# Veason-silverbullet/DIGAT

Measured on AMD Instinct MI355X. Metric: MIND dev impressions scored/sec (AUC match not run), higher is better.
Workload: dtype f32; 1 GPU; MIND-small default: --graph_encoder=DIGAT neighbors=3 hops=2 (N=10, U=67), d=400, graph_depth=3, fp32 dev inference; projection=auto -> fp16x3, N=10, U=67, d=400, graph_depth=3, news_num=65238, parallelism=dp1 (row shards, no data-path collective), ranks_in_process_group=1

## Files before the change

digat_amd/_lib.py:

```python
from __future__ import annotations

import ctypes as C
import os
from typing import Optional

import torch

_HERE = os.path.dirname(os.path.abspath(__file__))
LIB_PATH = os.environ.get("DIGAT_HIP_LIB") or os.path.join(_HERE, "lib", "libdigat_hip.so")
DIGAT_MAX_DEPTH = 16
DIGAT_MAX_NODES = 128
GEMM_BF16X6, GEMM_F16X3 = 0, 1
GEMM_F16F8C = 2
PARAMS_GEMM_F16X3 = 64
PARAMS_BD_TILED = 128
PARAMS_PQ_FP8 = 256
PARAMS_SIDE_STREAM_OFF, PARAMS_SIDE_STREAM_ON = 512, 1024
PARAMS_NO_LIVE_ROWS = 2048
PARAMS_PROJ_F16F8C = 4096

_f = C.c_void_p


class LayerParams(C.Structure):
    _fields_ = [(k, _f) for k in ("W", "bW", "F1", "F2", "F3", "b3", "a", "wsplit", "f3_wsplit")]


class MsaParams(C.Structure):
    _fields_ = ([(k, C.c_int32) for k in ("word_embedding_dim", "head_num", "head_dim", "attention_dim")]
                + [(k, C.c_void_p) for k in ("word_embedding", "W_Q", "b_Q", "W_K", "W_V", "b_V", "A1", "b1", "a2",
                                             "qkv_wsplit", "a1_wsplit")])


class MhsaParams(C.Structure):
    _fields_ = ([(k, C.c_int32) for k in ("in_dim", "head_num", "head_dim", "attention_dim")]
                + [(k, C.c_void_p) for k in ("table", "W_Q", "b_Q", "W_K", "W_V", "b_V", "A1", "b1", "a2", "qkv_wsplit", "a1_wsplit")]
                + [("flags", C.c_int32), ("reserved", C.c_int32)])


MHSA_POOL_UNMASKED = 1


class CnnParams(C.Structure):
    _fields_ = ([(k, C.c_int32) for k in ("word_embedding_dim", "kernel_num", "taps", "attention_dim")]
                + [(k, C.c_void_p) for k in ("word_embedding", "W", "b", "A1", "b1", "a2", "w_split", "a1_wsplit")])


class SplitJob(C.Structure):
    _fields_ = [("w0", C.c_void_p), ("w1", C.c_void_p), ("w2", C.c_void_p), ("rows", C.c_int32), ("cols", C.c_int32), ("layout", C.c_int32),
                ("reserved", C.c_int32), ("image", C.c_void_p)]


class GatherJob(C.Structure):
    _fields_ = [("src", C.c_void_p), ("dst", C.c_void_p), ("row_bytes", C.c_int64), ("rows", C.c_int64),
                ("idx", C.c_void_p), ("idx2", C.c_void_p), ("inner", C.c_int64)]


class Params(C.Structure):
    _fields_ = ([("d", C.c_int32), ("depth", C.c_int32), ("category_num", C.c_int32), ("flags", C.c_int32)]
                + [(k, _f) for k in ("topic_node_embedding", "cand_K", "cand_Q", "cand_bQ",
                                     "news_graph_W", "news_graph_b", "user_news_K", "user_news_Q",
                                     "user_news_bQ", "featureAffine_W", "featureAffine_b",
                                     "userAtt_K", "userAtt_Q", "userAtt_bQ")]
                + [("news", LayerParams * DIGAT_MAX_DEPTH), ("user", LayerParams * DIGAT_MAX_DEPTH)]
                + [(k, _f) for k in ("cand_fold_W", "cand_fold_b", "user_news_fold_W", "user_news_fold_b",
                                     "userAtt_fold_W", "userAtt_fold_b", "featureAffine_wsplit", "cand_fold_wsplit", "gate_wsplit")]
                + [("ctx_wsplit", _f * (DIGAT_MAX_DEPTH + 1)), ("range_flag", _f), ("featureAffine_fsplit", _f)])


class DigatHipError(RuntimeError):
    pass


_lib: Optional[C.CDLL] = None

_SIGNATURES = {
    "digat_version": (C.c_int, []),
    "digat_error_string": (C.c_char_p, [C.c_int]),
    "digat_linear_f32": (C.c_int, [_f, C.c_int64, _f, _f, _f, C.c_int64, C.c_int, C.c_int, C.c_int, _f]),
    "digat_xattn_workspace_bytes": (C.c_size_t, [C.c_int] * 3),
    "digat_xattn_fwd": (C.c_int, [_f] * 12 + [C.c_int] * 3 + [_f, C.c_size_t, _f]),
    "digat_xattn_fwd_mode": (C.c_int, [_f] * 11 + [C.c_int] * 4 + [_f, C.c_size_t, _f]),
    "digat_xattn_fwd_lowprec": (C.c_int, [_f] * 11 + [C.c_int, _f] + [C.c_int] * 4 + [_f, C.c_size_t, _f]),
    "digat_xattn_pairwise_fwd": (C.c_int, [_f] * 8 + [C.c_int] * 3 + [_f]),
    "digat_news_ctx_workspace_bytes": (C.c_size_t, [C.c_int] * 3),
    "digat_news_ctx_fwd": (C.c_int, [_f] * 9 + [C.c_int] * 3 + [_f, C.c_size_t, _f]),
    "digat_user_ctx_workspace_bytes": (C.c_size_t, [C.c_int] * 5),
    "digat_user_ctx_fwd": (C.c_int, [_f] * 14 + [C.c_int] * 5 + [_f, C.c_size_t, _f]),
    "digat_user_ctx_grouped_workspace_bytes": (C.c_size_t, [C.c_int] * 6),
    "digat_user_ctx_fwd_grouped": (C.c_int, [_f] * 15 + [C.c_int] * 6 + [_f, C.c_size_t, _f]),
    "digat_user_nodes_build": (C.c_int, [_f] * 4 + [C.c_long, C.c_long] + [C.c_int] * 3 + [_f]),
    "digat_topic_pool_fwd": (C.c_int, [_f] * 4 + [C.c_int] * 5 + [_f]),
    "digat_encoder_workspace_bytes": (C.c_size_t, [C.c_int] * 6),
    "digat_encoder_fwd": (C.c_int, [C.POINTER(Params)] + [_f] * 10 + [C.c_int] * 3 + [_f, C.c_size_t, _f]),
    "digat_row_logits": (C.c_int, [_f] * 3 + [C.c_int] * 2 + [_f]),
    "digat_profile_pause": (C.c_int, [C.c_int]),
    "digat_set_train_precision": (C.c_int, [C.c_int]),
    "digat_gather_tables": (C.c_int, [C.POINTER(GatherJob), C.c_int, _f]),
    "digat_user_graph_build": (C.c_int, [_f, _f, C.c_long, C.c_int, C.c_int, _f, _f, _f, _f]),
    "digat_negative_sample": (C.c_int, [_f, _f, _f, C.c_long, C.c_int, C.c_uint32, C.c_uint32, _f, _f]),
    "digat_train_batch_ids": (C.c_int, [_f, C.c_long, _f, _f, C.c_long, C.c_int, _f, C.c_long, C.c_int, _f, C.c_long, C.c_int, _f, _f, _f, _f, _f]),
    "digat_profile_live_row_fraction": (C.c_double, []),
    "digat_rank_metrics": (C.c_int, [_f] * 3 + [C.c_int] + [_f] * 4),
    "digat_format_rank_file": (C.c_int64, [_f, _f, C.c_int64, _f, C.c_int64]),
    "digat_topk_segments_workspace_bytes": (C.c_size_t, [C.c_int64, C.c_int64, C.c_int]),
    "digat_topk_segments": (C.c_int, [_f, _f, C.c_int64, C.c_int64, _f, _f, C.c_int, C.c_int, _f, _f, _f, _f, C.c_size_t, _f]),
    "digat_dot_topk_workspace_bytes": (C.c_size_t, [C.c_int64, C.c_int64, C.c_int]),
    "digat_dot_topk": (C.c_int, [_f, _f, _f, C.c_int64, C.c_int64, C.c_int64, C.c_int, _f, C.c_int, C.c_int, _f, _f, _f, _f, C.c_size_t, _f]),
    "digat_dot_scores": (C.c_int, [_f, _f, _f, C.c_int64, C.c_int64, C.c_int64, C.c_int, _f, _f]),
    "digat_mmr_select_workspace_bytes": (C.c_size_t, [C.c_int64, C.c_int, C.c_int]),
    "digat_mmr_select": (C.c_int, [_f, _f, _f, C.c_int64, C.c_int, _f, C.c_int64, C.c_int, _f, C.c_int, C.c_float, C.c_float, C.c_int, _f, _f, _f,
                                   _f, C.c_size_t, _f]),
    "digat_gat_workspace_bytes": (C.c_size_t, [C.c_int] * 3),
    "digat_gat_fwd": (C.c_int, [_f] * 7 + [C.c_int] * 3 + [_f, C.c_size_t, _f]),
    "digat_gat_train_save_bytes": (C.c_size_t, [C.c_int] * 3),
    "digat_gat_train_workspace_bytes": (C.c_size_t, [C.c_int] * 3),
    "digat_gat_fwd_train": (C.c_int, [_f] * 7 + [C.c_float, C.c_uint32] + [C.c_int] * 3 + [_f, C.c_size_t, _f, C.c_size_t, _f]),
    "digat_gat_bwd": (C.c_int, [_f] * 7 + [C.c_float, _f, C.c_size_t] + [_f] * 5 + [C.c_int] * 3 + [_f, C.c_size_t, _f]),
    "digat_sag_cos_topk_workspace_bytes": (C.c_size_t, [C.c_int64, C.c_int64, C.c_int]),
    "digat_sag_cos_topk": (C.c_int, [_f, _f, C.c_int64, _f, _f, C.c_int64, C.c_int, C.c_int, _f, _f, _f, C.c_size_t, _f]),
    "digat_sag_similar_lists_workspace_bytes": (C.c_size_t, [C.c_int64, C.c_int64, C.c_int]),
    "digat_sag_similar_lists": (C.c_int, [_f, _f, C.c_int64, _f, _f, C.c_int64, C.c_int, C.c_int] + [_f] * 7 + [C.c_int64, _f, C.c_size_t, _f]),
    "digat_sag_news_graph": (C.c_int, [_f, _f, _f, C.c_int64, C.c_int, C.c_int, C.c_int, C.c_float] + [_f] * 5),
    "digat_msa_split_bytes": (C.c_size_t, [C.c_int] * 3),
    "digat_split_msa_weights": (C.c_int, [_f] * 3 + [C.c_int] * 2 + [_f, _f]),
    "digat_msa_workspace_bytes": (C.c_size_t, [C.c_int] * 6),
    "digat_msa_fwd": (C.c_int, [C.POINTER(MsaParams), _f, _f, _f, C.c_int, C.c_int, _f, C.c_size_t, _f]),
    "digat_msa_train_save_bytes": (C.c_size_t, [C.c_int] * 6),
    "digat_msa_train_workspace_bytes": (C.c_size_t, [C.c_int] * 6),
    "digat_msa_fwd_train": (C.c_int, [C.POINTER(MsaParams), _f, _f, _f, C.c_float, C.c_uint32, C.c_int, C.c_int, _f, C.c_size_t, _f,
                                      C.c_size_t, _f]),
    "digat_msa_bwd": (C.c_int, [C.POINTER(MsaParams), _f, _f, _f, C.c_float, _f, C.c_size_t, _f, C.c_int64] + [_f] * 8
                      + [C.c_int, C.c_int, _f, C.c_size_t, _f]),
    "digat_msa_row_grad_ld": (C.c_int64, [C.c_int] * 3),
    "digat_mhsa_workspace_bytes": (C.c_size_t, [C.c_int] * 6),
    "digat_mhsa_fwd": (C.c_int, [C.POINTER(MhsaParams), _f, _f, _f, C.c_int, C.c_int, _f, C.c_size_t, _f]),
    "digat_mhsa_train_save_bytes": (C.c_size_t, [C.c_int] * 6),
    "digat_mhsa_train_workspace_bytes": (C.c_size_t, [C.c_int] * 6),
    "digat_mhsa_fwd_train": (C.c_int, [C.POINTER(MhsaParams), _f, _f, _f, C.c_float, C.c_float, C.c_uint32, C.c_int, C.c_int, _f, C.c_size_t, _f,
                                       C.c_size_t, _f]),
    "digat_mhsa_bwd": (C.c_int, [C.POINTER(MhsaParams), _f, _f, _f, C.c_float, C.c_float, C.c_uint32, _f, C.c_size_t, _f, C.c_int64] + [_f] * 8
                       + [C.c_int, C.c_int, _f, C.c_size_t, _f]),
    "digat_mhsa_attention_fwd": (C.c_int, [_f, _f, _f, C.c_float, C.c_uint32] + [C.c_int] * 4 + [_f]),
    "digat_mhsa_attention_bwd": (C.c_int, [_f, _f, _f, _f, C.c_float, C.c_uint32] + [C.c_int] * 4 + [_f]),
    "digat_cnn_split_bytes": (C.c_size_t, [C.c_int] * 3),
    "digat_split_cnn_weights": (C.c_int, [_f] + [C.c_int] * 3 + [_f, _f]),
    "digat_cnn_merge_group3": (C.c_int, [_f] * 6 + [C.c_int] * 2 + [_f] * 3),
    "digat_cnn_workspace_bytes": (C.c_size_t, [C.c_int] * 6),
    "digat_cnn_fwd": (C.c_int, [C.POINTER(CnnParams), _f, _f, _f, C.c_int, C.c_int, _f, C.c_size_t, _f]),
    "digat_cnn_train_save_bytes": (C.c_size_t, [C.c_int] * 6),
    "digat_cnn_train_workspace_bytes": (C.c_size_t, [C.c_int] * 6),
    "digat_cnn_fwd_train": (C.c_int, [C.POINTER(CnnParams), _f, _f, _f, C.c_float, C.c_uint32, C.c_int, C.c_int, _f, C.c_size_t, _f,
                                      C.c_size_t, _f]),
    "digat_cnn_bwd": (C.c_int, [C.POINTER(CnnParams), _f, _f, _f, C.c_float, C.c_uint32, _f, C.c_size_t, _f, C.c_int64] + [_f] * 5
                      + [C.c_int, C.c_int, _f, C.c_size_t, _f]),
    "digat_embedding_bwd_workspace_bytes": (C.c_size_t, [C.c_int64, C.c_int]),
    "digat_embedding_bwd": (C.c_int, [_f, C.c_int64, _f, _f, C.c_int64, C.c_int, _f, _f, C.c_size_t, _f]),
    "digat_embedding_bwd_unsorted_workspace_bytes": (C.c_size_t, [C.c_int64, C.c_int, C.c_int64]),
    "digat_embedding_bwd_unsorted": (C.c_int, [_f, _f, C.c_int64, C.c_int64, _f, _f, C.c_int64, C.c_int64, C.c_int, C.c_int64, _f, _f, C.c_size_t,
                                               _f]),
    "digat_encoder_grouped_workspace_bytes": (C.c_size_t, [C.c_int] * 6),
    "digat_encoder_fwd_grouped": (C.c_int, [C.POINTER(Params)] + [_f] * 11 + [C.c_int] * 4 + [_f, C.c_size_t, _f]),
    "digat_encoder_fwd_grouped_cached": (C.c_int, [C.POINTER(Params)] + [_f] * 14 + [C.c_int64] + [_f] * 2 + [C.c_int] * 4 + [_f, C.c_size_t, _f]),
    "digat_news_context_queries": (C.c_int, [C.POINTER(Params), _f, _f, C.c_int, _f]),
    "digat_user_project0": (C.c_int, [C.POINTER(Params), _f, _f, C.c_int, _f]),
    "digat_news_project0": (C.c_int, [C.POINTER(Params), _f, _f, C.c_int, C.c_int, _f]),
    "digat_split_weights_bytes": (C.c_size_t, [C.c_int, C.c_int]),
    "digat_split_weights_bytes_format": (C.c_size_t, [C.c_int, C.c_int, C.c_int]),
    "digat_forget_split_image": (C.c_int, [_f]),
    "digat_split_proj_weights": (C.c_int, [_f, _f, _f, C.c_int, _f, C.c_int, _f]),
    "digat_split_weights": (C.c_int, [_f, C.c_int, C.c_int, _f, C.c_int, _f]),
    "digat_linear_f32x3": (C.c_int, [_f, C.c_int64, _f, _f, _f, C.c_int64, C.c_int, C.c_int, C.c_int, _f, C.c_int, _f]),
    "digat_fold_workspace_bytes": (C.c_size_t, [C.c_int]),
    "digat_fold_attention": (C.c_int, [_f] * 5 + [C.c_int, _f, C.c_size_t, _f]),
    "digat_linear_bwd_input": (C.c_int, [_f, C.c_int64, _f, _f, C.c_int64, C.c_int, C.c_int, C.c_int, C.c_int, _f]),
    "digat_linear_bwd_input_x3": (C.c_int, [_f, C.c_int64, _f, _f, C.c_int64, C.c_int, C.c_int, C.c_int, C.c_int, _f, _f]),
    "digat_linear_bwd_weight_workspace": (C.c_size_t, [C.c_int] * 3),
    "digat_linear_bwd_weight": (C.c_int, [_f, C.c_int64, _f, C.c_int64, _f, _f, C.c_int, C.c_int, C.c_int, C.c_int, _f,
                                          C.c_size_t, _f]),
    "digat_colsum": (C.c_int, [_f, C.c_int64, _f, C.c_int, C.c_int, C.c_int, _f]),
    "digat_dropout_fwd": (C.c_int, [_f, _f, _f, C.c_int64, C.c_float, C.c_uint32, _f]),
    "digat_dropout_bwd": (C.c_int, [_f, _f, _f, C.c_int64, C.c_float, _f]),
    "digat_gate_fwd": (C.c_int, [_f, _f, C.c_int64, _f, _f, C.c_int, C.c_int, _f]),
    "digat_gate_bwd": (C.c_int, [_f, _f, _f, C.c_int64, _f, _f, _f, _f, C.c_int, C.c_int, _f]),
    "digat_relu_res_fwd": (C.c_int, [_f, _f, _f, C.c_int64, _f]),
    "digat_relu_mask": (C.c_int, [_f, _f, _f, C.c_int64, _f]),
    "digat_attn_pool_fwd": (C.c_int, [_f, C.c_int64, _f, _f, _f, _f, C.c_int, C.c_int, C.c_int, _f]),
    "digat_attn_pool_bwd": (C.c_int, [_f, C.c_int64, _f, _f, _f, _f, _f, C.c_int64, _f, C.c_int, C.c_int, C.c_int,
                                      C.c_int, _f]),
    "digat_topic_pool_fwd_train": (C.c_int, [_f] * 5 + [C.c_int] * 5 + [_f]),
    "digat_topic_pool_bwd": (C.c_int, [_f] * 7 + [C.c_int] * 5 + [_f]),
    "digat_xattn_project": (C.c_int, [_f] * 9 + [C.c_int] * 3 + [_f]),
    "digat_xattn_project_x3": (C.c_int, [_f] * 9 + [C.c_int] * 3 + [_f, _f]),
    "digat_xattn_pairwise_fwd_train": (C.c_int, [_f] * 11 + [C.c_float, C.c_uint32, C.c_int, C.c_int, C.c_int, _f]),
    "digat_xattn_pairwise_bwd_workspace": (C.c_size_t, [C.c_int] * 3),
    "digat_xattn_pairwise_bwd": (C.c_int, [_f] * 11 + [C.c_float] + [_f] * 4 + [C.c_int] * 4 + [_f, C.c_size_t, _f]),
    "digat_sum_nodes": (C.c_int, [_f, _f, C.c_int, C.c_int, C.c_int, _f]),
    "digat_xattn_train_save_bytes": (C.c_size_t, [C.c_int] * 3),
    "digat_xattn_train_workspace_bytes": (C.c_size_t, [C.c_int] * 3),
    "digat_xattn_fwd_train": (C.c_int, [_f] * 11 + [C.c_float, C.c_uint32, C.c_float, C.c_uint32] + [C.c_int] * 3 + [_f, C.c_size_t, _f, C.c_size_t, _f, C.c_int,
                                        _f]),
    "digat_xattn_bwd": (C.c_int, [_f] * 10 + [C.c_float, C.c_float, _f, C.c_size_t] + [_f] * 9 + [C.c_int] * 3 + [_f, C.c_size_t, _f, C.c_int, _f]),
    "digat_opt_chunk": (C.c_int, []),
    "digat_clip_adam_step": (C.c_int, [_f, _f, _f, C.c_int, _f] + [C.c_float] * 5 + [C.c_int, _f]),
    "digat_row_logits_bwd": (C.c_int, [_f] * 5 + [C.c_int, C.c_int, _f]),
    "digat_click_loss": (C.c_int, [_f, C.c_int, C.c_int, _f, _f, _f]),
    "digat_split_job_bytes": (C.c_size_t, [C.c_int] * 4),
    "digat_split_jobs": (C.c_int, [C.POINTER(SplitJob), C.c_int, _f]),
    "digat_news_ctx_train_save_bytes": (C.c_size_t, [C.c_int] * 3),
    "digat_news_ctx_train_workspace_bytes": (C.c_size_t, [C.c_int] * 3),
    "digat_news_ctx_fwd_train": (C.c_int, [_f] * 8 + [C.c_float, C.c_uint32] + [C.c_int] * 3 + [_f, C.c_size_t, _f, C.c_size_t, _f, _f]),
    "digat_news_ctx_bwd": (C.c_int, [_f] * 6 + [C.c_float, _f, C.c_size_t] + [_f] * 6 + [C.c_int] * 4 + [_f, C.c_size_t, _f]),
    "digat_user_ctx_train_save_bytes": (C.c_size_t, [C.c_int] * 5),
    "digat_user_ctx_train_workspace_bytes": (C.c_size_t, [C.c_int] * 5),
    "digat_user_ctx_fwd_train": (C.c_int, [_f] * 13 + [C.c_float, C.c_uint32] + [C.c_int] * 5 + [_f, C.c_size_t, _f, C.c_size_t, _f, _f, _f]),
    "digat_user_ctx_bwd": (C.c_int, [_f] * 10 + [C.c_float, _f, C.c_size_t] + [_f] * 10 + [C.c_int] * 6 + [_f, C.c_size_t, _f, _f]),
    "digat_profile_start": (C.c_int, [C.c_int]),
    "digat_profile_stop": (C.c_int, [C.POINTER(C.c_double), C.POINTER(C.c_double), C.POINTER(C.c_int)]),
    "digat_profile_set_kinds": (C.c_int, [C.c_uint]),
    "digat_profile_gemm_bytes": (C.c_int, [C.POINTER(C.c_double)]),
    "digat_profile_marker": (C.c_int, [C.c_int, _f]),
    "digat_encoder_shared_workspace_bytes": (C.c_size_t, [C.c_int] * 6),
    "digat_encoder_fwd_shared": (C.c_int, [C.POINTER(Params)] + [_f] * 10 + [C.c_int] * 3 + [_f, C.c_size_t, _f]),
    "digat_user_row_runs": (C.c_int, [_f] * 4 + [C.c_int] * 5 + [_f] * 4 + [C.c_size_t, _f]),
    "digat_profile_xattn_parts": (C.c_int, [C.POINTER(C.c_double), C.POINTER(C.c_double), C.POINTER(C.c_int)]),
    "digat_split_ctx_fused_bytes": (C.c_size_t, [C.c_int]),
    "digat_split_ctx_fused_weights": (C.c_int, [_f, C.c_int, _f, _f]),
}
KERNEL_KINDS = ("proj", "linear", "xattn", "pool", "topic", "glue", "agg")
XATTN_PARTS = ("twin", "l0", "news", "other")
EXPORTED = tuple(_SIGNATURES)
ABI_VERSION = 4


def lib() -> C.CDLL:
    global _lib
    if _lib is None:
        if not os.path.exists(LIB_PATH):
            raise DigatHipError(
                f"{LIB_PATH} is missing: the HIP extension has not been built "
                "(run `python -m digat_amd.build` or __graft_entry__.build()). There is no CPU fallback.")
        handle = C.CDLL(LIB_PATH)
        handle.digat_version.restype, handle.digat_version.argtypes = C.c_int, []
        got = handle.digat_version()
        if got != ABI_VERSION:
            raise DigatHipError(f"{LIB_PATH} reports ABI version {got}, this loader's signature table is for version {ABI_VERSION}: "
                                "rebuild it from this tree (python -m digat_amd.build)")
        for name, (res, args) in _SIGNATURES.items():
            fn = getattr(handle, name)
            fn.restype, fn.argtypes = res, args
        _lib = handle
    return _lib


EXT_PATH = os.path.join(_HERE, "lib", "digat_torch_ext.so")
USE_TORCH_EXT = os.environ.get("DIGAT_TORCH_EXT", "1") != "0"
_ext = None


def ext():
    global _ext
    if not USE_TORCH_EXT or os.environ.get("DIGAT_HIP_LIB"):
        return None
    if _ext is None:
        if not os.path.exists(EXT_PATH):
            _ext = False
        else:
            import importlib.util
            lib()
            spec = importlib.util.spec_from_file_location("digat_torch_ext", EXT_PATH)
            mod = importlib.util.module_from_spec(spec)
            spec.loader.exec_module(mod)
            if mod.abi_version() != lib().digat_version():
                raise DigatHipError("digat_torch_ext.so and libdigat_hip.so disagree about the ABI version: rebuild (python -m digat_amd.build)")
            _ext = mod
    return _ext or None


def binding():
    X = ext()
    if X is not None:
        return X
    from . import _ctypes_binding
    return _ctypes_binding


def check(code: int, what: str) -> None:
    if code != 0:
        msg = lib().digat_error_string(code).decode()
        raise DigatHipError(f"{what} failed: [{code}] {msg}")


def addressof(struct) -> int:
    return C.addressof(struct)


def ptr(t: Optional[torch.Tensor]) -> Optional[int]:
    return None if t is None else t.data_ptr()


def stream_ptr() -> int:
    return torch.cuda.current_stream().cuda_stream


def require_device(*tensors: torch.Tensor) -> torch.device:
    dev = tensors[0].device
    if dev.type != "cuda":
        raise DigatHipError("digat_amd runs on the GPU only (got a %s tensor); there is no CPU path" % dev.type)
    for t in tensors:
        if t.device != dev:
            raise DigatHipError("all tensors must live on the same device")
    return dev


def f32(t: torch.Tensor) -> torch.Tensor:
    if t.dtype != torch.float32:
        raise DigatHipError(f"expected float32, got {t.dtype}")
    return t.contiguous()


def as_bytes(t: torch.Tensor) -> torch.Tensor:
    if t.dtype == torch.bool:
        return t.contiguous().view(torch.uint8)
    if t.dtype == torch.uint8:
        return t.contiguous()
# ... 44 lines not shown
```

digat_amd/csrc/digat_encoder.inc:

```
static size_t max_sz(size_t a, size_t b) { return a > b ? a : b; }

struct FoldCtxWs { float *T, *T2, *glob; };
struct EncoderWs {
    float *Xu[2], *Xn[2];
    char* xws; size_t xws_bytes;
    XattnWs xu;
    char* cws; size_t cws_bytes;
    FoldCtxWs fc;
    float *kq_t, *kq_u, *r_user[2], *r_news;
    char* xws_news; size_t xws_news_bytes;
    XattnWs xn;
    int *cnt, *off, *idx, *cnt2, *off2, *idx2, *entries, *flag, *hlast;
    uint8_t *flags1, *flags2;
    int *cnt_n, *off_n, *idx_n; uint8_t* flags_n;
    int *l0_gs, *l0_off; uint8_t* l0_lead; int* l0_idx;
    unsigned* tw_word; int* tw_list; uint8_t* tw_flags; int *tw_cnt, *tw_off;
    int *gl_off, *gl_idx;
    int* idx32;
    uint8_t *Au, *cm; int64_t* ci;
    uint8_t *fg, *tfg; unsigned* twg; uint8_t* bfg; int *cg, *eg, *hg, *bcg, *tcg;
    uint8_t *same, *is_leader, *lead; int* leader_of;
};
static bool encoder_carve(Arena& a, int B, int N, int H, int C, int d, int variant, EncoderWs& e) {
    const int U = H + C, C1 = C + 1, nmax = N > U ? N : U;
    const size_t b = (size_t)B, bd = b * d, bu = b * U;
    e = EncoderWs();
    for (float*& x : e.Xu) x = a.take<float>(bu * d);
    for (float*& x : e.Xn) x = a.take<float>(b * N * d);
    Arena xa = a.sub(digat_xattn_workspace_bytes(B, nmax, d));
    e.xws = xa.base; e.xws_bytes = xa.cap;
    e.xu = xattn_carve(xa, B, U, d);
    Arena ca = a.sub(max_sz(digat_news_ctx_workspace_bytes(B, N, d), digat_user_ctx_workspace_bytes(B, U, H, C1, d)));
    e.cws = ca.base; e.cws_bytes = ca.cap;
    e.fc = FoldCtxWs{ca.take<float>(b * C1 * d), ca.take<float>(b * C1 * d), ca.take<float>(bd)};
    e.kq_t = a.take<float>(bd); e.kq_u = a.take<float>(bd);
    e.r_user[0] = a.take<float>(bd); e.r_news = a.take<float>(bd); e.r_user[1] = a.take<float>(bd);
    Arena na = a.sub(digat_xattn_workspace_bytes(B, N, d));
    e.xws_news = na.base; e.xws_news_bytes = na.cap;
    e.xn = xattn_carve(na, B, N, d);
    e.cnt = a.take<int>(b); e.off = a.take<int>(b + 1); e.idx = a.take<int>(bu);
    e.cnt2 = a.take<int>(b); e.off2 = a.take<int>(b + 1); e.idx2 = a.take<int>(b * C1);
    e.entries = a.take<int>(b); e.flag = a.take<int>(64); e.hlast = a.take<int>(b);
    e.flags1 = a.take<uint8_t>(bu); e.flags2 = a.take<uint8_t>(b * C1);
    e.cnt_n = a.take<int>(b); e.off_n = a.take<int>(b + 1); e.idx_n = a.take<int>(b * N); e.flags_n = a.take<uint8_t>(b * N);
    e.l0_gs = a.take<int>(b + 64); e.l0_off = a.take<int>(b + 64); e.l0_lead = a.take<uint8_t>(b); e.l0_idx = a.take<int>(bu);
    e.tw_word = a.take<unsigned>(bu); e.tw_list = a.take<int>(bu); e.tw_flags = a.take<uint8_t>(bu);
    e.tw_cnt = a.take<int>(b + 64); e.tw_off = a.take<int>(b + 64);
    e.gl_off = a.take<int>(b + 64); e.gl_idx = a.take<int>(bu);
    e.idx32 = a.take<int>(b);
    if (variant == ENC_GROUPED) {
        const size_t g = b / 4 + 1;
        e.Au = a.take<uint8_t>(bu * U); e.cm = a.take<uint8_t>(b * C1); e.ci = a.take<int64_t>(b * H);
        e.fg = a.take<uint8_t>(g * U); e.tfg = a.take<uint8_t>(g * U); e.twg = a.take<unsigned>(g * U); e.bfg = a.take<uint8_t>(g * C1);
        for (int** x : {&e.cg, &e.eg, &e.hg, &e.bcg, &e.tcg}) *x = a.take<int>(g);
    } else if (variant == ENC_SHARED) {
        e.same = a.take<uint8_t>(b); e.is_leader = a.take<uint8_t>(b); e.lead = a.take<uint8_t>(b); e.leader_of = a.take<int>(b);
    }
    return a.ok && xa.ok && ca.ok && na.ok;
}
static size_t encoder_ws_bytes(int B, int N, int H, int C, int d, int variant) { Arena a; EncoderWs e; encoder_carve(a, B, N, H, C, d, variant, e); return a.used; }

struct EncoderCall {
    const digat_params* p;
    const float* Xn_in; const uint8_t *An, *Mn;
    const float* ue;
    const uint8_t *Au, *cat_mask; const int64_t* cat_idx;
    const float* c_n0; float *out_news, *out_user;
    int B, N, H;
    void* workspace; size_t workspace_bytes; hipStream_t st;
    int variant;
    const int* row_group; int G;
    const uint8_t *Au_g, *cm_g; const int64_t* ci_g;
    const float *news_hpq0, *hist_hpq0, *topic_hpq0, *ctxq0; const int64_t* news_index; int64_t news_rows;
    const uint8_t *run_leader, *run_lead;
    EncoderPlan plan;
    EncoderWs ws;
};
struct SideStream { hipStream_t s; hipEvent_t fork, join, early; int ok; };
constexpr int SPARSE_PER_NODE = 20;
static SideStream* side_stream(hipStream_t caller) {
    struct Entry { int dev; hipStream_t caller; SideStream side; int state; };
    static Entry tab[64];
    static int used = 0;
    static std::mutex mu;
    int dev = 0;
    if (hipGetDevice(&dev) != hipSuccess) return nullptr;
    std::lock_guard<std::mutex> lock(mu);
    for (int i = 0; i < used; ++i)
        if (tab[i].dev == dev && tab[i].caller == caller) return tab[i].state == 1 ? &tab[i].side : nullptr;
    if (used == 64) return nullptr;
    Entry& e = tab[used++];
    e.dev = dev; e.caller = caller;
    SideStream& x = e.side;
    const bool ok = hipStreamCreateWithFlags(&x.s, hipStreamNonBlocking) == hipSuccess &&
                    hipEventCreateWithFlags(&x.fork, hipEventDisableTiming) == hipSuccess &&
                    hipEventCreateWithFlags(&x.join, hipEventDisableTiming) == hipSuccess &&
                    hipEventCreateWithFlags(&x.early, hipEventDisableTiming) == hipSuccess;
    e.state = ok ? 1 : -1;
    return ok ? &x : nullptr;
}

static int grid_blocks(long total4, int cap) {
    const int blocks = (int)((total4 + 255) / 256);
    return blocks > cap ? cap : blocks;
}

static GemmArgs ctx_queries_args(const digat_params* p, const float* c_n, int M, int next_layer, float* kq_topic, float* kq_user, float* k3) {
    const GemmFormats f = gemm_formats(p);
    const int d = p->d;
    GemmArgs g = gemm_plain(c_n, d, p->user_news_fold_W, p->user_news_fold_b, kq_topic, d, M, d, d, 0);
    g.w[1] = p->userAtt_fold_W; g.bias[1] = p->userAtt_fold_b; g.y[1] = kq_user;
    g.nsegs = 2;
    if (next_layer < p->depth) {
        g.w[2] = p->user[next_layer].F3; g.bias[2] = p->user[next_layer].b3; g.y[2] = k3;
        g.nsegs = 3;
    }
    g.wsplit = (const unsigned short*)p->ctx_wsplit[next_layer]; g.format = f.fmt; g.range_flag = f.range_flag;
    g.m_dispatch = bd_dispatch(p->flags);
    return g;
}

static GemmArgs layer_proj3_args(const digat_params* p, const digat_layer_params& l, const float* X, int M, float* h, float* P, float* Q) {
    const GemmFormats f = gemm_formats(p);
    return proj3_args(X, M, p->d, l.W, l.bW, l.F1, l.F2, h, P, Q, l.wsplit, (p->flags & DIGAT_PROJ_PQ_X3) ? 1 : 0, f.lfmt, f.range_flag);
}

struct LiveArrays { uint8_t *flags, *tflags, *bflags; unsigned* twin; int *cnt, *entries, *hlast, *bcnt, *tcnt; };
struct LiveFlagsJob { const uint8_t *Au, *cat_mask; const int64_t* cat_idx; int rows; const uint8_t* rowmask; LiveArrays out; bool expand; };

struct LiveLists {
    const int *rowidx, *nrows;
    const int *bucket_idx, *nbuckets;
    const int* hist_last;
    uint8_t* flags;
    TwinLists tw;
};

struct FoldedPass {
    const EncoderCall& c; const EncoderPlan& pl;
    const float* const Xg0;
    SideStream* const side;
    const digat_params* const p; const EncoderWs& w; const hipStream_t st;
    const int B, N, H, G, d, C, L, U, C1;
    const GemmFormats f;
    float *const c_n, *const c_u; const float* const c_n_src;
    LiveLists pend{}, live{};
    const int* sparse_flag = nullptr;
    const int *news_rowidx = nullptr, *news_nrows = nullptr; const uint8_t* news_flags = nullptr;

    FoldedPass(const EncoderCall& call, const float* Xg0_, SideStream* side_)
        : c(call), pl(call.plan), Xg0(Xg0_), side(side_), p(call.p), w(call.ws), st(call.st), B(call.B), N(call.N), H(call.H), G(call.G),
          d(call.p->d), C(call.p->category_num), L(call.p->depth), U(call.H + call.p->category_num), C1(call.p->category_num + 1),
          f(gemm_formats(call.p)), c_n(call.out_news), c_u(call.out_user), c_n_src(call.plan.c_n0_in_place ? call.c_n0 : call.out_news) {}

    int context_queries(int next_layer, hipStream_t sq) const {
        return launch_gemm(ctx_queries_args(p, next_layer == 0 ? c_n_src : c_n, B, next_layer, w.kq_t, w.kq_u, w.r_user[next_layer & 1]), sq);
    }

    int user_context(const float* Xu_cur, const float* addend, hipStream_t sq, const int* xgroup, bool lists,
                     const float* kq_topic = nullptr, const float* kq_user = nullptr) const {
        if (!kq_topic) { kq_topic = w.kq_t; kq_user = w.kq_u; }
        const uint8_t* flags = lists ? live.flags : nullptr;
        const int* hist_last = flags ? live.hist_last : nullptr;
        if (pl.user_ctx_fused) {
            const CtxFusedArgs fa{Xu_cur, (long)U * d, xgroup, flags, U, hist_last, kq_topic, kq_user, c.cat_idx, c.cat_mask, addend, c_u,
                                  (const uint4*)p->featureAffine_fsplit, p->featureAffine_b, f.range_flag, B, H, C1, d, sqrtf((float)d)};
            return launch_user_ctx_fused(fa, sq);
        }
        float *T = w.fc.T, *T2 = w.fc.T2;
        int e = launch_topic(Xu_cur, (long)U * d, kq_topic, c.cat_idx, T, B, H, C1, d, sq, xgroup, flags, U, hist_last);
        if (e) return e;
        GemmArgs g = gemm_plain(T, d, p->featureAffine_W, p->featureAffine_b, T2, d, B * C1, d, d, 0);
        g.epi = EPI_RELU_RES; g.e0 = T; g.lde0 = d;
        g.wsplit = (const unsigned short*)p->featureAffine_wsplit;
        g.format = f.fmt; g.range_flag = f.range_flag;
        if (live.bucket_idx && gemm_takes_row_list(g)) { g.rowidx = live.bucket_idx; g.nrows_dev = live.nbuckets; }
        e = launch_gemm(g, sq);
        if (e) return e;
        return launch_pool(T2, (long)C1 * d, kq_user, c.cat_mask, addend, c_u, B, C1, d, sq);
    }

    int news_context(const float* Xn_cur, hipStream_t sq, bool first) const {
        const long ldx = (long)N * d;
        float *kq = w.kq_t, *glob = w.fc.glob;
        GemmArgs gq = gemm_plain(Xn_cur, ldx, p->cand_fold_W, p->cand_fold_b, kq, d, B, d, d, 0);
        gq.wsplit = (const unsigned short*)p->cand_fold_wsplit; gq.format = f.fmt; gq.range_flag = f.range_flag;
        gq.m_dispatch = pl.bd_disp;
        int e = launch_gemm(gq, sq);
        if (e) return e;
        e = launch_pool(Xn_cur, ldx, kq, c.Mn, nullptr, glob, B, N, d, sq);
        if (e) return e;
        GemmArgs g = gemm_plain(Xn_cur, ldx, p->news_graph_W, p->news_graph_b, c_n, d, B, d, 2 * d, 0);
        g.k0 = d; g.a1 = glob; g.lda1 = d;
        g.epi = EPI_GATE; g.e0 = Xn_cur; g.lde0 = ldx; g.e1 = glob; g.lde1 = d; g.e2 = first ? c_n_src : c_n; g.lde2 = d;
        g.wsplit = (const unsigned short*)p->gate_wsplit; g.format = f.fmt; g.range_flag = f.range_flag;
        g.m_dispatch = 1;
        return launch_gemm(g, sq);
    }

    int live_flags(const LiveFlagsJob& j, const LiveArrays& rows, hipStream_t sq) const {
        const bool want_entries = pl.sparse_mode == DIGAT_XATTN_AUTO, twins = pl.twins;
        const LiveArrays& o = j.out;
        hipLaunchKernelGGL(user_live_flags_kernel, dim3((j.rows + 3) / 4), dim3(256), (size_t)4 * ((U * U + 63) & ~63), sq, j.Au, j.cat_mask, j.cat_idx,
                           j.rows, U, H, C1, o.flags, o.cnt, want_entries ? o.entries : (int*)nullptr, o.hlast, o.bflags, o.bcnt,
                           twins ? o.twin : (unsigned*)nullptr, twins ? o.tflags : (uint8_t*)nullptr, twins ? o.tcnt : (int*)nullptr, j.rowmask);
        DIGAT_CHECK_LAUNCH();
        if (!j.expand) return DIGAT_OK;
        LiveExpand le;
        le.flags_g = o.flags; le.twin_g = twins ? o.twin : nullptr; le.tflags_g = o.tflags; le.bflags_g = o.bflags;
        le.cnt_g = o.cnt; le.entries_g = o.entries; le.hlast_g = o.hlast; le.bcnt_g = o.bcnt; le.tcnt_g = o.tcnt;
        le.flags = rows.flags; le.twin = twins ? rows.twin : nullptr; le.tflags = rows.tflags; le.bflags = rows.bflags;
        le.cnt = rows.cnt; le.entries = want_entries ? rows.entries : nullptr; le.hlast = rows.hlast; le.bcnt = rows.bcnt;
        le.tcnt = twins ? rows.tcnt : nullptr;
        hipLaunchKernelGGL(live_expand_kernel, dim3((B + 3) / 4), dim3(256), 0, sq, le, c.row_group, B, U, C1);
        DIGAT_CHECK_LAUNCH();
        return DIGAT_OK;
    }

    int adjacency_pass(hipStream_t sq) {
        LiveArrays rows;
        rows.flags = w.flags1; rows.tflags = w.tw_flags; rows.bflags = w.flags2; rows.twin = w.tw_word;
        rows.cnt = w.cnt; rows.entries = w.entries; rows.hlast = w.hlast; rows.bcnt = w.cnt2; rows.tcnt = w.tw_cnt;
        const uint8_t* const l0_lead = pl.shared ? c.run_lead : w.l0_lead;
        ProfScope prof(DIGAT_KERNEL_GLUE, (double)B * ((double)U * U + 2.0 * C1 + H * 8.0) + (double)B * (U + C1) * 6, sq);
        if (pl.l0_chunked && !pl.shared) {
            hipLaunchKernelGGL(sparse_l0_chunks_kernel, dim3(1), dim3(1024), 0, sq, c.row_group, B, G, SPARSE_L0_ROWS, w.l0_gs, w.l0_lead);
            DIGAT_CHECK_LAUNCH();
        }
        LiveFlagsJob j{c.Au, c.cat_mask, c.cat_idx, B, nullptr, rows, false};
        if (pl.shared) {
            j.rowmask = c.run_leader; j.expand = true;
        } else if (c.variant == ENC_GROUPED) {
            j.Au = c.Au_g; j.cat_mask = c.cm_g; j.cat_idx = c.ci_g; j.rows = G; j.expand = true;
            LiveArrays& o = j.out;
            o.flags = w.fg; o.tflags = w.tfg; o.bflags = w.bfg; o.twin = w.twg;
            o.cnt = w.cg; o.entries = w.eg; o.hlast = w.hg; o.bcnt = w.bcg; o.tcnt = w.tcg;
        }
        const int rc = live_flags(j, rows, sq);
        if (rc) return rc;
        if (pl.sparse_mode == DIGAT_XATTN_AUTO) {
            hipLaunchKernelGGL(sparse_decide_kernel, dim3(1), dim3(1024), 0, sq, (const int*)w.entries, B, U, SPARSE_PER_NODE, w.flag);
            DIGAT_CHECK_LAUNCH();
            sparse_flag = w.flag;
        }
        ScanPair sp{{w.cnt, w.cnt2}, {w.off, w.off2}, {nullptr, nullptr}};
        ListPair lp{{w.flags1, w.flags2}, {w.off, w.off2}, {U, C1, U, U, U, U}, {w.idx, w.idx2}, {nullptr, nullptr}};
        int jobs = 2;
        if (pl.l0_chunked) {
            sp.cnt[jobs] = w.cnt; sp.off[jobs] = w.l0_off; sp.rowmask[jobs] = l0_lead;
            lp.flags[jobs] = w.flags1; lp.off[jobs] = w.l0_off; lp.out[jobs] = w.l0_idx; lp.rowmask[jobs] = l0_lead;
            ++jobs;
        }
        if (pl.twins) {
            sp.cnt[jobs] = w.tw_cnt; sp.off[jobs] = w.tw_off;
            lp.flags[jobs] = w.tw_flags; lp.off[jobs] = w.tw_off; lp.out[jobs] = w.tw_list;
            lp.width[jobs] = U;
            ++jobs;
        }
        if (pl.shared) {
            sp.cnt[jobs] = w.cnt; sp.off[jobs] = w.gl_off; sp.rowmask[jobs] = c.run_leader;
            lp.flags[jobs] = w.flags1; lp.off[jobs] = w.gl_off; lp.out[jobs] = w.gl_idx; lp.rowmask[jobs] = c.run_leader;
            lp.width[jobs] = U;
            ++jobs;
        }
        hipLaunchKernelGGL(exclusive_scan2_kernel, dim3(jobs), dim3(1024), 0, sq, sp, B);
        DIGAT_CHECK_LAUNCH();
        hipLaunchKernelGGL(live_list2_kernel, dim3((B + 3) / 4, jobs), dim3(256), 0, sq, lp, B);
        DIGAT_CHECK_LAUNCH();
        pend = LiveLists{w.idx, w.off + B, w.idx2, w.off2 + B, w.hlast, w.flags1, {nullptr, nullptr, nullptr}};
        if (pl.twins) pend.tw = TwinLists{w.tw_word, w.tw_list, w.tw_off + B};
        return DIGAT_OK;
    }
    void publish() { live = pend; }

    int news_projection(int layer, const float* Xn_cur, hipStream_t sq) const {
        GemmArgs gp = layer_proj3_args(p, p->news[layer], Xn_cur, B * N, w.xn.h, w.xn.P, w.xn.Q);
        gp.m_dispatch = 1 << 30;
        if (news_rowidx && gemm_takes_row_list(gp)) { gp.rowidx = news_rowidx; gp.nrows_dev = news_nrows; }
        return launch_gemm(gp, sq, DIGAT_KERNEL_PROJ);
    }

    int group_projection(hipStream_t sq) const {
        const digat_layer_params& lu = p->user[0];
        if (pl.shared) {
            GemmArgs gs = layer_proj3_args(p, lu, w.Xu[0], B * U, w.xu.h, w.xu.P, w.xu.Q);
            gs.m_dispatch = B * U;
            if (pl.want_live && gemm_takes_row_list(gs)) { gs.rowidx = w.gl_idx; gs.nrows_dev = w.gl_off + B; }
            return launch_gemm(gs, sq, DIGAT_KERNEL_PROJ);
        }
        const size_t ndg = (size_t)G * U * d;
        float* Xg = pl.xu0_grouped ? const_cast<float*>(Xg0) : w.Xu[1];
        float* h0 = w.xu.h;
        float* P0 = h0 + ndg;
        float* Q0 = w.xu.Q;
        const int blocks = grid_blocks((long)ndg / 4, 2048);
        if (!pl.xu0_grouped) {
            hipLaunchKernelGGL(build_user_nodes_kernel, dim3(blocks), dim3(256), 0, sq, (const float4*)c.ue,
                               (const float4*)p->topic_node_embedding, (float4*)Xg, (long)G, H, C, d / 4, (const int*)nullptr);
            DIGAT_CHECK_LAUNCH();
        }
        if (pl.group_tables) {
            float* dst[3] = {h0, P0, Q0};
            UserNodes3 un3;
            for (int t = 0; t < 3; ++t) {
                un3.hist[t] = (const float4*)(c.hist_hpq0 + (size_t)t * G * H * d);
                un3.topic[t] = (const float4*)(c.topic_hpq0 + (size_t)t * C * d);
                un3.dst[t] = (float4*)dst[t];
            }
            hipLaunchKernelGGL(build_user_nodes3_kernel, dim3(blocks, 3), dim3(256), 0, sq, un3, (long)G, H, C, d / 4);
            DIGAT_CHECK_LAUNCH();
            return DIGAT_OK;
        }
        GemmArgs gg = layer_proj3_args(p, lu, Xg, G * U, h0, P0, Q0);
        gg.m_dispatch = B * U;
        return launch_gemm(gg, sq, DIGAT_KERNEL_PROJ);
    }

    int user_layer0_grouped(const float* r_user, bool projected) const {
        const digat_layer_params& lu = p->user[0];
        const size_t ndg = pl.shared ? (size_t)B * U * d : (size_t)G * U * d;
        float* h0 = w.xu.h;
        float* P0 = h0 + ndg;
        float* Q0 = w.xu.Q;
        int rc = projected ? DIGAT_OK : group_projection(st);
        if (rc) return rc;
        if (pl.l0_sparse) {
            const bool l0_live = pl.want_live && live.flags;
            SparseArgs sg{P0, Q0, h0, pl.xu0_grouped ? Xg0 : w.Xu[0], lu.a, c.Au, w.Xu[1], r_user, c.row_group, l0_live ? live.flags : nullptr,
// ... 354 lines not shown
```

digat_amd/csrc/digat_encoder_plan.h:

```cpp
#pragma once
#include <stddef.h>
#include <stdint.h>
#include "../../include/digat_hip.h"

enum { ENC_PLAIN, ENC_GROUPED, ENC_SHARED };

static inline bool eq8_row_fits_wave(int d) { return d / 4 <= 256; }
static inline bool eq8_multi_centre_fits(int d, int n) { return d / 4 <= 128 && n <= 128; }
static inline bool eq8_sparse_graph(int n) { return n > 16; }
static inline bool eq8_small_graph(int n) { return n <= 16; }

struct GemmFormats { int fmt, lfmt; unsigned* range_flag; };
static inline GemmFormats gemm_formats(int flags, void* range_flag) {
    const int fmt = (flags & DIGAT_PARAMS_GEMM_F16X3) ? 1 : 0;
    return GemmFormats{fmt, (flags & DIGAT_PARAMS_PROJ_F16F8C) ? DIGAT_GEMM_F16F8C : fmt, fmt ? (unsigned*)range_flag : nullptr};
}
static inline GemmFormats gemm_formats(const digat_params* p) { return gemm_formats(p->flags, p->range_flag); }
static inline int bd_dispatch(int flags) { return (flags & DIGAT_PARAMS_BD_TILED) ? (1 << 30) : 1; }

struct EncoderPlanIn {
    int flags, B, N, H, C, d, L, G, variant;
    bool folded;
    bool c_n0, news_hpq0, hist_hpq0, topic_hpq0, ctxq0, news_index; int64_t news_rows;
    bool fsplit;
    bool ctx_fused_fits;
};

struct EncoderPlan {
    int status;
    int status_after_carve;
    bool folded;
    bool shared;
    bool by_group;
    bool xu0_grouped;
    bool xu0_shared;
    bool c_n0_in_place;
    bool ctxq0;
    int sparse_mode;
    bool want_live, want_scan;
    bool l0_chunked, twins;
    bool l0_sparse, l0_dense;
    bool group_tables;
    int pq_x3, pq_mode;
    int fmt, lfmt, bd_disp;
    bool news_early;
    bool news_lists;
    int news_sparse_mode;
    bool news_cached0, news_indexed0;
    bool user_ctx_fused;
    int side_mode;
    bool side_wanted;
};

static inline EncoderPlan encoder_plan(const EncoderPlanIn& in) {
    EncoderPlan pl = {};
    const int flags = in.flags, B = in.B, N = in.N, H = in.H, C = in.C, d = in.d, L = in.L, U = H + C;
    const bool grouped = in.variant == ENC_GROUPED, folded = in.folded;
    pl.status = pl.status_after_carve = DIGAT_OK;
    pl.folded = folded;
    if (in.hist_hpq0 != in.topic_hpq0) { pl.status = DIGAT_ERR_ARG; return pl; }
    if (in.ctxq0 && !in.c_n0) { pl.status = DIGAT_ERR_ARG; return pl; }
    if (grouped && in.G <= 0) { pl.status = DIGAT_ERR_ARG; return pl; }
    if (B < 0 || N <= 0 || H < 0) { pl.status = DIGAT_ERR_ARG; return pl; }
    if (grouped && !folded) { pl.status = DIGAT_ERR_ARG; return pl; }
    if (d <= 0 || d % 4 || L < 0 || L > DIGAT_MAX_DEPTH || N > DIGAT_MAX_NODES || U > DIGAT_MAX_NODES || C < 0) { pl.status = DIGAT_ERR_SHAPE; return pl; }
    if (grouped && (size_t)4 * in.G > (size_t)B) { pl.status = DIGAT_ERR_SHAPE; return pl; }
    if (in.news_index && !(in.c_n0 && in.news_hpq0 && L > 0 && eq8_row_fits_wave(d) && in.news_rows > 0 && in.news_rows <= 0x7fffffffLL &&
                           (eq8_small_graph(N) || ((flags & DIGAT_NEWS_XATTN_SPARSE) && N <= DIGAT_MAX_NODES)) && folded))
        pl.status_after_carve = DIGAT_ERR_ARG;

    pl.shared = in.variant == ENC_SHARED && folded && L > 0 && (flags & 3) == DIGAT_XATTN_SPARSE && !(flags & DIGAT_PARAMS_NO_LIVE_ROWS) &&
                eq8_multi_centre_fits(d, U) && eq8_sparse_graph(U);
    pl.by_group = grouped || pl.shared;
    pl.xu0_grouped = grouped && folded && L > 0 && (flags & 3) == DIGAT_XATTN_SPARSE && eq8_row_fits_wave(d) && eq8_sparse_graph(U) && 3 * (long)in.G <= B;
    pl.c_n0_in_place = in.c_n0 && folded && L > 0;
    pl.ctxq0 = folded && in.ctxq0 && in.c_n0;
    const GemmFormats f = gemm_formats(flags, nullptr);
    pl.fmt = f.fmt; pl.lfmt = f.lfmt; pl.bd_disp = bd_dispatch(flags);
    pl.pq_x3 = (flags & DIGAT_PROJ_PQ_X3) ? 1 : 0;
    pl.pq_mode = ((flags & DIGAT_PQ_BF16) ? 1 : 0) | ((flags & DIGAT_PQ_X1) ? 2 : 0) | ((flags & DIGAT_PQ_FP8) ? 4 : 0);
    pl.sparse_mode = flags & 3;
    if (pl.sparse_mode == 3 || (pl.sparse_mode == DIGAT_XATTN_AUTO && L == 0)) pl.sparse_mode = DIGAT_XATTN_DENSE;
    pl.xu0_shared = pl.shared && pl.sparse_mode == DIGAT_XATTN_SPARSE;
    pl.want_live = L > 0 && !(flags & DIGAT_PARAMS_NO_LIVE_ROWS);
    pl.want_scan = pl.want_live || pl.sparse_mode == DIGAT_XATTN_AUTO;
    pl.l0_chunked = pl.by_group && (pl.xu0_grouped || pl.shared) && pl.want_live && pl.sparse_mode == DIGAT_XATTN_SPARSE && eq8_multi_centre_fits(d, U);
    pl.twins = pl.want_live && pl.sparse_mode == DIGAT_XATTN_SPARSE && eq8_multi_centre_fits(d, U) && L > 1;
    const bool group_l0 = folded && L > 0 && pl.by_group;
    pl.l0_sparse = group_l0 && pl.sparse_mode != DIGAT_XATTN_DENSE && eq8_row_fits_wave(d);
    pl.l0_dense = group_l0 && !(pl.sparse_mode == DIGAT_XATTN_SPARSE && eq8_row_fits_wave(d));
    pl.group_tables = group_l0 && !pl.shared && in.hist_hpq0 && in.topic_hpq0 && (long)B * U >= 2048;
    pl.news_early = L > 0 && eq8_small_graph(N) && eq8_row_fits_wave(d);
    const bool news_lists_on = L > 0 && eq8_row_fits_wave(d) && !(flags & DIGAT_PARAMS_NO_LIVE_ROWS);
    pl.news_lists = news_lists_on && ((!pl.news_early && (flags & DIGAT_NEWS_XATTN_SPARSE) && eq8_sparse_graph(N)) || (pl.news_early && L > 1 && B >= 2048));
    pl.news_sparse_mode = (flags & DIGAT_NEWS_XATTN_SPARSE) ? DIGAT_XATTN_SPARSE : DIGAT_XATTN_DENSE;
    pl.news_cached0 = folded && L > 0 && in.news_hpq0;
    pl.news_indexed0 = pl.news_cached0 && in.news_index;
    pl.user_ctx_fused = in.fsplit && pl.fmt == 1 && in.ctx_fused_fits;
    pl.side_mode = (flags & DIGAT_PARAMS_SIDE_STREAM_OFF) ? 0 : ((flags & DIGAT_PARAMS_SIDE_STREAM_ON) ? 1 : 2);
    pl.side_wanted = folded && !(pl.side_mode == 0 || (pl.side_mode == 2 && B >= 2048));
    return pl;
}
```

digat_amd/csrc/digat_gemm.inc:

```

#include "digat_gemm_plan.h"

template <int BM, int BN, int WAVES_M, int WAVES_N, int PF, int TAG>
__global__ void __launch_bounds__(256) gemm_f32_kernel(const GemmArgs g) {
    constexpr int BK4 = 8;
    constexpr int MT = BM / WAVES_M / 16;
    constexpr int NT = BN / WAVES_N / 16;
    static_assert(WAVES_M * WAVES_N == 4, "4 waves per workgroup");
    static_assert(BM % (WAVES_M * 16) == 0 && BN % (WAVES_N * 16) == 0, "wave tile");
    static_assert(BM % 8 == 0 && BN % 8 == 0, "xor swizzle needs 8-row groups");
    constexpr int A_PER_T = (BM * BK4 + 255) / 256;
    constexpr int B_PER_T = (BN * BK4 + 255) / 256;
    __shared__ float4 As[BK4 * BM];
    __shared__ float4 Bs[BK4 * BN];

    const int total = g.mtiles * g.ntiles;
    const int chunk = (total + 7) >> 3;
    const int tile = (int)(blockIdx.x & 7) * chunk + (int)(blockIdx.x >> 3);
    if (tile >= total) return;
    const int mtile = tile / g.ntiles, ntile = tile - mtile * g.ntiles;

    const int tid = threadIdx.x, lane = tid & 63, wave = tid >> 6;
    const int wm = wave / WAVES_N, wn = wave % WAVES_N;
    const int m0 = mtile * BM, n0 = ntile * BN;
// ... 164 lines not shown
}

typedef __bf16 bf16x8 __attribute__((ext_vector_type(8)));

struct Split3f { float a, b, c; };
__device__ __forceinline__ Split3f split3f(float v) {
    Split3f o;
    o.a = __builtin_bit_cast(float, __builtin_bit_cast(unsigned, v) & 0xffff0000u);
    const float r1 = v - o.a;
    o.b = __builtin_bit_cast(float, __builtin_bit_cast(unsigned, r1) & 0xffff0000u);
    o.c = r1 - o.b;
    return o;
}
__device__ __forceinline__ unsigned pack_bf16_rne(float lo, float hi) {
    unsigned a = __builtin_bit_cast(unsigned, lo), b = __builtin_bit_cast(unsigned, hi);
    a += 0x7fffu + ((a >> 16) & 1u);
    b += 0x7fffu + ((b >> 16) & 1u);
    return (a >> 16) | (b & 0xffff0000u);
}
__device__ __forceinline__ unsigned pack_hi16(float lo, float hi) {
    return __builtin_amdgcn_perm(__builtin_bit_cast(unsigned, hi), __builtin_bit_cast(unsigned, lo), 0x07060302u);
}
constexpr float F16_WEIGHT_SCALE = 1024.f;
constexpr float F16_ACT_SCALE = 16.f;
typedef _Float16 half8 __attribute__((ext_vector_type(8)));
typedef __fp16 fp16x2 __attribute__((ext_vector_type(2)));
__device__ __forceinline__ unsigned pack_half_rtz(float lo, float hi) { return __builtin_bit_cast(unsigned, __builtin_amdgcn_cvt_pkrtz(lo, hi)); }
__device__ __forceinline__ unsigned half_bits_rtz(float v) { return pack_half_rtz(v, 0.f) & 0xffffu; }
__device__ __forceinline__ float half_bits_to_float(unsigned bits) {
    const fp16x2 h = __builtin_bit_cast(fp16x2, bits);
    return (float)h[0];
}
struct Split3 { unsigned short a, b, c; };
__device__ __forceinline__ Split3 split3(float v) {
    const Split3f f = split3f(v);
    Split3 o;
    o.a = (unsigned short)(__builtin_bit_cast(unsigned, f.a) >> 16);
    o.b = (unsigned short)(__builtin_bit_cast(unsigned, f.b) >> 16);
    o.c = (unsigned short)(__builtin_bit_cast(unsigned, f.c) >> 16);
    return o;
}

constexpr int WS_SLOTS = 960;

__device__ __forceinline__ void split_weights_tiled_body(const float* w0, const float* w1, const float* w2,
                                                         int nseg, int nsegs, int K, unsigned short* out, int transposed, int planes) {
    const int KT = (K + 31) >> 5, Kp = KT * 32;
    const int Ntot = nseg * nsegs;
    const int strips = (Ntot + 79) / 80;
    const long total = (long)strips * 80 * Kp;
    for (long i = (long)blockIdx.x * 256 + threadIdx.x; i < total; i += (long)gridDim.x * 256) {
        const int n = (int)(i / Kp), k = (int)(i - (long)n * Kp);
        float v = 0.f;
        if (n < Ntot && k < K) {
            const int seg = n / nseg;
            const float* w = seg == 0 ? w0 : (seg == 1 ? w1 : w2);
            if (transposed == 2) {
                const int kseg = K / 3, ks = k / kseg;
                const float* wk = ks == 0 ? w0 : (ks == 1 ? w1 : w2);
                v = wk[(long)(k - ks * kseg) * nseg + n];
            } else
            v = transposed ? w[(long)k * nseg + n] : w[(long)(n - seg * nseg) * K + k];
        }
        const int strip = n / 80, r = n - strip * 80, kt = k >> 5, kq = (k >> 3) & 3, e = k & 7;
        const long base = ((long)strip * KT + kt) * (planes * 320) * 8;
        if (planes == 3) {
            const Split3 sp = split3(v);
            out[base + ((0 * 4 + kq) * 80 + r) * 8 + e] = sp.a;
            out[base + ((1 * 4 + kq) * 80 + r) * 8 + e] = sp.b;
            out[base + ((2 * 4 + kq) * 80 + r) * 8 + e] = sp.c;
        } else {
            const float vs = v * F16_WEIGHT_SCALE;
            const _Float16 h = (_Float16)vs;
            const _Float16 l = (_Float16)(vs - (float)h);
            const unsigned hi = __builtin_bit_cast(unsigned short, h), lo = __builtin_bit_cast(unsigned short, l);
            out[base + ((0 * 4 + kq) * 80 + r) * 8 + e] = (unsigned short)hi;
            out[base + ((1 * 4 + kq) * 80 + r) * 8 + e] = (unsigned short)lo;
        }
    }
}
__global__ void __launch_bounds__(256) split_weights_tiled_kernel(const float* w0, const float* w1, const float* w2,
                                                                  int nseg, int nsegs, int K, unsigned short* out, int transposed, int planes) {
    split_weights_tiled_body(w0, w1, w2, nseg, nsegs, K, out, transposed, planes);
}
constexpr int SPLIT_MAX_JOBS = 24;
struct SplitJobDev { const float *w0, *w1, *w2; unsigned short* out; int nseg, nsegs, K, transposed; };
struct SplitJobsDev { SplitJobDev j[SPLIT_MAX_JOBS]; };
__device__ __forceinline__ void split_weights_slots_body(const float* w0, const float* w1, const float* w2, int nseg, int nsegs, int K,
                                                         unsigned short* out, int transposed) {
    const int KT = (K + 31) >> 5;
    const int Ntot = nseg * nsegs;
    const int strips = (Ntot + 79) / 80;
    const int k8s = KT * 4;
    const long total = (long)strips * 80 * k8s;
    for (long i = (long)blockIdx.x * 256 + threadIdx.x; i < total; i += (long)gridDim.x * 256) {
        const int n = transposed ? (int)(i % (strips * 80)) : (int)(i / k8s);
        const int k8 = transposed ? (int)(i / (strips * 80)) : (int)(i - (long)n * k8s);
        const int k0 = k8 * 8;
        float v[8];
#pragma unroll
        for (int e = 0; e < 8; ++e) v[e] = 0.f;
        if (n < Ntot) {
            if (!transposed) {
                const int seg = n / nseg;
                const float* row = (seg == 0 ? w0 : (seg == 1 ? w1 : w2)) + (long)(n - seg * nseg) * K;
                if (k0 + 8 <= K && ((uintptr_t)(row + k0) & 15) == 0) {
                    const float4 a = *reinterpret_cast<const float4*>(row + k0), b = *reinterpret_cast<const float4*>(row + k0 + 4);
                    v[0] = a.x; v[1] = a.y; v[2] = a.z; v[3] = a.w; v[4] = b.x; v[5] = b.y; v[6] = b.z; v[7] = b.w;
                } else {
#pragma unroll
                    for (int e = 0; e < 8; ++e) if (k0 + e < K) v[e] = row[k0 + e];
                }
            } else if (transposed == 2) {
                const int kseg = K / 3;
#pragma unroll
                for (int e = 0; e < 8; ++e) {
                    const int k = k0 + e;
                    if (k < K) {
                        const int ks = k / kseg;
                        v[e] = (ks == 0 ? w0 : (ks == 1 ? w1 : w2))[(long)(k - ks * kseg) * nseg + n];
                    }
                }
            } else {
#pragma unroll
                for (int e = 0; e < 8; ++e) if (k0 + e < K) v[e] = w0[(long)(k0 + e) * nseg + n];
            }
        }
        const int strip = n / 80, r = n - strip * 80, kt = k8 >> 2, kq = k8 & 3;
        const long base = ((long)strip * KT + kt) * (3 * 320) * 8;
        unsigned pa[4], pb[4], pc[4];
#pragma unroll
        for (int h = 0; h < 4; ++h) {
            const Split3 s0 = split3(v[2 * h]), s1 = split3(v[2 * h + 1]);
            pa[h] = (unsigned)s0.a | ((unsigned)s1.a << 16);
            pb[h] = (unsigned)s0.b | ((unsigned)s1.b << 16);
            pc[h] = (unsigned)s0.c | ((unsigned)s1.c << 16);
        }
        *reinterpret_cast<uint4*>(out + base + ((0 * 4 + kq) * 80 + r) * 8) = make_uint4(pa[0], pa[1], pa[2], pa[3]);
        *reinterpret_cast<uint4*>(out + base + ((1 * 4 + kq) * 80 + r) * 8) = make_uint4(pb[0], pb[1], pb[2], pb[3]);
        *reinterpret_cast<uint4*>(out + base + ((2 * 4 + kq) * 80 + r) * 8) = make_uint4(pc[0], pc[1], pc[2], pc[3]);
    }
}
__global__ void __launch_bounds__(256) split_weights_jobs_kernel(const SplitJobsDev a) {
    const SplitJobDev& j = a.j[blockIdx.y];
    split_weights_slots_body(j.w0, j.w1, j.w2, j.nseg, j.nsegs, j.K, j.out, j.transposed);
}

#ifdef DIGAT_GEMM_TIMERS
__device__ unsigned long long g_gemm_timers[8];
#define GT_NOW() __builtin_amdgcn_s_memtime()
#else
#define GT_NOW() 0ull
#endif
template <int NSUB, bool F16, int MT, bool FULL>
__global__ void __launch_bounds__(256, MT == 1 ? 3 : 2) gemm_bf16x6s_kernel(const GemmArgs g) {
    static_assert(MT == 1 || MT == 2, "wave tiles of 16 or 32 rows");
    constexpr int NT = 5;
    constexpr int WROWS = 16 * MT, TROWS = 4 * WROWS;
    constexpr int APW = 2 * MT;
    constexpr int RING = 3;
    constexpr int ABUF = NSUB == 1 ? 2 : 1;
    constexpr int PL = F16 ? 2 : 3;
    constexpr int WS_SLOTS = PL * 320;
    constexpr int PIECES = WS_SLOTS / 64;
    constexpr int IMG_I = (PIECES + 3) / 4;
    __shared__ uint4 Bs[RING][WS_SLOTS];
    __shared__ uint4 As[ABUF][TROWS * 8];

    const int Mv = g.nrows_dev ? __builtin_amdgcn_readfirstlane(*g.nrows_dev) : g.M;
    if (g.exec_rows && blockIdx.x == 0 && threadIdx.x == 0) atomicAdd(g.exec_rows, (unsigned long long)Mv);
    const int total = ((Mv + TROWS - 1) / TROWS) * g.ntiles;
    const int chunk = (total + 7) >> 3;
    if ((int)(blockIdx.x >> 3) >= chunk) return;
    const int tile = (int)(blockIdx.x & 7) * chunk + (int)(blockIdx.x >> 3);
    if (tile >= total) return;
    const int mtile = tile / g.ntiles, ntile = tile - mtile * g.ntiles;

    const int tid = threadIdx.x, lane = tid & 63, wm = tid >> 6;
    const int kg = lane >> 4, lr = lane & 15;
    const int m0 = mtile * TROWS;
    const int strip0 = ntile * NSUB;
#ifdef DIGAT_GEMM_TIMERS
    const unsigned long long gt_enter = GT_NOW();
    unsigned long long gt_wait = 0, gt_bar = 0, gt_body = 0, gt_steps = 0, gt_last = 0;
#endif
    const int KT = (g.K + 31) >> 5;
    const int nsteps = KT * NSUB;
    const unsigned ldsB = (unsigned)(uintptr_t)(__attribute__((address_space(3))) unsigned char*)&Bs[0][0];
    const unsigned ldsA = (unsigned)(uintptr_t)(__attribute__((address_space(3))) unsigned char*)&As[0][0];
    const char* const wimg = reinterpret_cast<const char*>(g.wsplit);
    const unsigned wlane = (unsigned)lane * 16u;
    const int wu = __builtin_amdgcn_readfirstlane(wm);

    auto issue_b = [&](int step) {
        const int kt = step / NSUB, s = step - kt * NSUB;
        const int buf = step % RING;
        const char* src = wimg + ((long)(strip0 + s) * KT + kt) * (WS_SLOTS * 16);
#pragma unroll
        for (int k = 0; k < IMG_I; ++k) {
            int q = wu + 4 * k;
            q = q < PIECES ? q : PIECES - 1;
            lds_dma16_s(src + q * 1024, wlane, ldsB + (unsigned)((buf * WS_SLOTS + q * 64) * 16));
        }
    };
    const long arow0 = g.rowidx ? 0 : (long)(m0 < Mv ? m0 : Mv - 1);
    const char* const abase = reinterpret_cast<const char*>(g.a0 + arow0 * g.lda0);
    unsigned aoff[APW];
    int ac4[APW];
#pragma unroll
    for (int k = 0; k < APW; ++k) {
        const int sl = (wm + 4 * k) * 64 + lane;
        const int r = sl >> 3, c4 = (sl & 7) ^ ((r >> 1) & 7);
        int gm = m0 + r;
        gm = gm < Mv ? gm : Mv - 1;
        if (g.rowidx) gm = g.rowidx[gm];
        aoff[k] = (unsigned)((((long)gm - arow0) * g.lda0 + c4 * 4) * 4);
        ac4[k] = c4 * 4;
    }
    auto issue_a_piece = [&](int kt, int abuf, int k) {
        unsigned vo = aoff[k];
        long sk = (long)kt * 128;
        if (kt * 32 + 32 > g.K) { vo += kt * 32 + ac4[k] < g.K ? (unsigned)kt * 128u : 0u; sk = 0; }
        lds_dma16_s(abase + sk, vo, ldsA + (unsigned)((abuf * (TROWS * 8) + (wu + 4 * k) * 64) * 16));
    };
    auto issue_a = [&](int kt, int abuf) {
#pragma unroll
        for (int k = 0; k < APW; ++k) issue_a_piece(kt, abuf, k);
    };
    auto split_half = [&](const float4& v, unsigned (&o)[3][2]) {
        const Split3f s0 = split3f(v.x), s1 = split3f(v.y), s2 = split3f(v.z), s3 = split3f(v.w);
        o[0][0] = pack_hi16(s0.a, s1.a); o[0][1] = pack_hi16(s2.a, s3.a);
        o[1][0] = pack_hi16(s0.b, s1.b); o[1][1] = pack_hi16(s2.b, s3.b);
        o[2][0] = pack_hi16(s0.c, s1.c); o[2][1] = pack_hi16(s2.c, s3.c);
    };
    float amax = 0.f;
    auto split_mt = [&](int mt, int abuf, bf16x8 (&dst)[3][MT]) {
        const int r = wm * WROWS + mt * 16 + lr;
        const int sw = (r >> 1) & 7;
        const float4 v0 = __builtin_bit_cast(float4, As[abuf][r * 8 + ((kg * 2) ^ sw)]);
        const float4 v1 = __builtin_bit_cast(float4, As[abuf][r * 8 + ((kg * 2 + 1) ^ sw)]);
        if constexpr (F16) {
            constexpr float xs = F16_ACT_SCALE;
            const float raw[8] = {v0.x, v0.y, v0.z, v0.w, v1.x, v1.y, v1.z, v1.w};
            const float v[8] = {v0.x * xs, v0.y * xs, v0.z * xs, v0.w * xs, v1.x * xs, v1.y * xs, v1.z * xs, v1.w * xs};
            amax = fmaxf(fmaxf(amax, fabsf(v[0])), fabsf(v[1])); amax = fmaxf(fmaxf(amax, fabsf(v[2])), fabsf(v[3]));
            amax = fmaxf(fmaxf(amax, fabsf(v[4])), fabsf(v[5])); amax = fmaxf(fmaxf(amax, fabsf(v[6])), fabsf(v[7]));
            unsigned hi[4], lo[4];
#pragma unroll
            for (int e = 0; e < 4; ++e) {
                hi[e] = pack_half_rtz(v[2 * e], v[2 * e + 1]);
                const fp16x2 h = __builtin_bit_cast(fp16x2, hi[e]);
                const _Float16 l0 = (_Float16)__builtin_fmaf(raw[2 * e], xs, -(float)h[0]), l1 = (_Float16)__builtin_fmaf(raw[2 * e + 1], xs, -(float)h[1]);
                lo[e] = (unsigned)__builtin_bit_cast(unsigned short, l0) | ((unsigned)__builtin_bit_cast(unsigned short, l1) << 16);
            }
            dst[0][mt] = __builtin_bit_cast(bf16x8, make_uint4(hi[0], hi[1], hi[2], hi[3]));
            dst[1][mt] = __builtin_bit_cast(bf16x8, make_uint4(lo[0], lo[1], lo[2], lo[3]));
        } else {
            unsigned lo[3][2], hi[3][2];
            split_half(v0, lo);
            split_half(v1, hi);
#pragma unroll
            for (int p = 0; p < 3; ++p) dst[p][mt] = __builtin_bit_cast(bf16x8, make_uint4(lo[p][0], lo[p][1], hi[p][0], hi[p][1]));
        }
    };
    auto mma = [&](const bf16x8 w, const bf16x8 a, const v4f c) -> v4f {
        if constexpr (F16) return __builtin_amdgcn_mfma_f32_16x16x32_f16(__builtin_bit_cast(half8, w), __builtin_bit_cast(half8, a), c, 0, 0, 0);
        else return __builtin_amdgcn_mfma_f32_16x16x32_bf16(w, a, c, 0, 0, 0);
    };

    int lite[NSUB];
#pragma unroll
    for (int s = 0; s < NSUB; ++s) {
        const int seg = ((strip0 + s) * 80) / g.nseg;
        lite[s] = FULL ? 0 : __builtin_amdgcn_readfirstlane(((g.x1_segs >> seg) & 1) ? 2 : ((g.x3_segs >> seg) & 1));
    }
    v4f acc[NSUB][MT][NT];
#pragma unroll
    for (int s = 0; s < NSUB; ++s)
#pragma unroll
        for (int mt = 0; mt < MT; ++mt)
#pragma unroll
            for (int nt = 0; nt < NT; ++nt) acc[s][mt][nt] = (v4f){0.f, 0.f, 0.f, 0.f};

    bf16x8 af[3][MT], afn[3][MT];
    if constexpr (NSUB == 1) {
#pragma unroll
        for (int j = 0; j < ABUF; ++j) if (j < KT) issue_a(j, j);
#pragma unroll
        for (int j = 0; j < RING - 1; ++j) if (j < nsteps) issue_b(j);
    } else {
        issue_a(0, 0);
        issue_b(0);
        if (nsteps > 1) issue_b(1);
    }
    asm volatile("s_waitcnt vmcnt(0)" ::: "memory");
    __builtin_amdgcn_s_barrier();
#pragma unroll
    for (int mt = 0; mt < MT; ++mt) split_mt(mt, 0, af);

    for (int kt = 0; kt < KT; ++kt) {
        const bool more = kt + 1 < KT;
#pragma unroll
        for (int s = 0; s < NSUB; ++s) {
            const int step = kt * NSUB + s;
            const int buf = step % RING;
#ifdef DIGAT_GEMM_TIMERS
            const unsigned long long gt0 = GT_NOW();
            if (step > 0) gt_body += gt0 - gt_last;
#endif
            if constexpr (NSUB == 1) {
                constexpr int L = (RING - 1 < ABUF - 1 ? RING - 1 : ABUF - 1) - 1;
                constexpr int KEEP = (APW + IMG_I) * (L < 0 ? 0 : L) + ((ABUF - 1 < RING - 1) ? IMG_I : 0);
                static_assert(KEEP <= 63, "vmcnt is six bits");
                if (kt + (RING - 1 > ABUF ? RING - 1 : ABUF) < KT) wait_vmcnt_imm<KEEP>();
                else asm volatile("s_waitcnt vmcnt(0)" ::: "memory");
            } else if (step + 1 < nsteps) {
                if constexpr (IMG_I == 4) asm volatile("s_waitcnt vmcnt(4)" ::: "memory");
                else asm volatile("s_waitcnt vmcnt(3)" ::: "memory");
            } else asm volatile("s_waitcnt vmcnt(0)" ::: "memory");
#ifdef DIGAT_GEMM_TIMERS
            const unsigned long long gt1 = GT_NOW();
#endif
            __builtin_amdgcn_s_barrier();
#ifdef DIGAT_GEMM_TIMERS
            gt_last = GT_NOW();
            gt_wait += gt1 - gt0; gt_bar += gt_last - gt1; ++gt_steps;
#endif
            if (NSUB == 1) {
                if (kt + ABUF < KT) issue_a(kt + ABUF, kt % ABUF);
                if (step + RING - 1 < nsteps) issue_b(step + RING - 1);
            } else {
                if (s == 0 && more) issue_a(kt + 1, 0);
                if (step + 2 < nsteps) issue_b(step + 2);
            }
            const uint4* Bi = Bs[buf];
            const int lslot = kg * 80 + lr;
            bf16x8 bq[2][3];
#pragma unroll
            for (int p = 0; p < PL; ++p) bq[0][p] = __builtin_bit_cast(bf16x8, Bi[p * 320 + lslot]);
#pragma unroll
            for (int nt = 0; nt < NT; ++nt) {
                if (nt + 1 < NT) {
#pragma unroll
                    for (int p = 0; p < PL; ++p) bq[(nt + 1) & 1][p] = __builtin_bit_cast(bf16x8, Bi[p * 320 + lslot + (nt + 1) * 16]);
                }
                const bf16x8 b1 = bq[nt & 1][0], b2 = bq[nt & 1][1], b3 = bq[nt & 1][PL - 1];
                v4f c[MT];
#pragma unroll
                for (int mt = 0; mt < MT; ++mt) c[mt] = acc[s][mt][nt];
                if (!F16 && (FULL || !lite[s])) {
#pragma unroll
                    for (int mt = 0; mt < MT; ++mt) c[mt] = mma(b1, af[2][mt], c[mt]);
#pragma unroll
                    for (int mt = 0; mt < MT; ++mt) c[mt] = mma(b2, af[1][mt], c[mt]);
#pragma unroll
                    for (int mt = 0; mt < MT; ++mt) c[mt] = mma(b3, af[0][mt], c[mt]);
                }
                if (FULL || lite[s] < 2) {
#pragma unroll
                    for (int mt = 0; mt < MT; ++mt) c[mt] = mma(b1, af[1][mt], c[mt]);
#pragma unroll
                    for (int mt = 0; mt < MT; ++mt) c[mt] = mma(b2, af[0][mt], c[mt]);
                }
#pragma unroll
                for (int mt = 0; mt < MT; ++mt) c[mt] = mma(b1, af[0][mt], c[mt]);
#pragma unroll
                for (int mt = 0; mt < MT; ++mt) acc[s][mt][nt] = c[mt];
                if (NSUB > 1) {
                    if (s == 1 && nt == 0) split_mt(0, 0, afn);
                    if constexpr (MT > 1) { if (s == 1 && nt == 2) split_mt(1, 0, afn); }
                } else {
                    if (nt == 0) split_mt(0, (kt + 1) % ABUF, afn);
                    if constexpr (MT > 1) { if (nt == 2) split_mt(1, (kt + 1) % ABUF, afn); }
                }
            }
            if (NSUB == 1 || s == 1) {
#pragma unroll
                for (int i = 0; i < 56; ++i) {
                    __builtin_amdgcn_sched_group_barrier(0x008, 1, 0);
                    __builtin_amdgcn_sched_group_barrier(0x002, 2, 0);
                }
            }
        }
        if (more) {
#pragma unroll
            for (int p = 0; p < 3; ++p)
#pragma unroll
                for (int mt = 0; mt < MT; ++mt) af[p][mt] = afn[p][mt];
        }
    }

#ifdef DIGAT_GEMM_TIMERS
    const unsigned long long gt_loop_end = GT_NOW();
    gt_body += gt_loop_end - gt_last;
#endif
    if constexpr (F16) {
        if (g.range_flag && __builtin_amdgcn_ballot_w64(!(amax < 65504.f)) != 0 && lane == 0) atomicOr(g.range_flag, 1u);
    }
    int gmv[MT];
    bool rok[MT];
    {
        const int* const ri = (g.rowidx && !g.gather_only) ? g.rowidx : nullptr;
#pragma unroll
        for (int mt = 0; mt < MT; ++mt) {
            const int gv = m0 + wm * WROWS + mt * 16 + lr;
            rok[mt] = gv < Mv;
            const int gvc = rok[mt] ? gv : Mv - 1;
            gmv[mt] = ri ? ri[gvc] : gvc;
        }
    }
    const bool has_e0 = g.epi == EPI_RELU_RES || g.epi == EPI_ADD_E0;
#pragma unroll
    for (int s = 0; s < NSUB; ++s) {
        const int ncol0 = (strip0 + s) * 80;
        const int seg = ncol0 / g.nseg;
        const int nbase = ncol0 - seg * g.nseg + kg * 4;
        const float* const bp = g.bias[seg];
        const bool radd_here = g.radd && seg == g.radd_seg;
        const bool y16 = (g.bf16_segs >> seg) & 1;
        const bool y8 = (g.fp8_segs >> seg) & 1;
        float4 bv[NT];
        if (bp) {
#pragma unroll
            for (int nt = 0; nt < NT; ++nt) bv[nt] = *reinterpret_cast<const float4*>(bp + nbase + nt * 16);
        }
#pragma unroll
        for (int mt = 0; mt < MT; ++mt) {
            const int gm = gmv[mt];
            float* const yrow = g.y[seg] + (long)gm * g.ldy;
            float4 rv[NT], ev[NT];
            if (radd_here) {
                const float* rrow = g.radd + (long)(gm / g.rows_per_b) * g.nseg + nbase;
#pragma unroll
                for (int nt = 0; nt < NT; ++nt) rv[nt] = *reinterpret_cast<const float4*>(rrow + nt * 16);
            }
            if (y8) {
                float4 vv[NT];
                float amx = 0.f;
#pragma unroll
                for (int nt = 0; nt < NT; ++nt) {
                    const v4f a = acc[s][mt][nt];
                    float4 v = make_float4(a[0], a[1], a[2], a[3]);
                    if constexpr (F16) {
                        constexpr float u = 1.f / (F16_WEIGHT_SCALE * F16_ACT_SCALE);
                        v = make_float4(v.x * u, v.y * u, v.z * u, v.w * u);
                    }
                    if (bp) v = f4_add(v, bv[nt]);
                    if (radd_here) v = f4_add(rv[nt], v);
                    vv[nt] = v;
                    amx = fmaxf(fmaxf(amx, fmaxf(fabsf(v.x), fabsf(v.y))), fmaxf(fabsf(v.z), fabsf(v.w)));
                }
                amx = fmaxf(amx, __shfl_xor(amx, 16, 64));
                amx = fmaxf(amx, __shfl_xor(amx, 32, 64));
                const float scale = amx > 0.f ? amx * (1.f / 448.f) : 1.f;
                const float inv = 1.f / scale;
                unsigned char* const row8 = reinterpret_cast<unsigned char*>(g.y[seg]) + (long)gm * g.ldy8;
                if (rok[mt]) {
#pragma unroll
                    for (int nt = 0; nt < NT; ++nt) {
                        int w = 0;
                        w = __builtin_amdgcn_cvt_pk_fp8_f32(vv[nt].x * inv, vv[nt].y * inv, w, false);
                        w = __builtin_amdgcn_cvt_pk_fp8_f32(vv[nt].z * inv, vv[nt].w * inv, w, true);
                        *reinterpret_cast<int*>(row8 + nbase + nt * 16) = w;
                    }
                    if (kg == 0) *reinterpret_cast<float*>(row8 + g.nseg + 4 * ((ncol0 - seg * g.nseg) / 80)) = scale;
                }
                continue;
            }
            if (has_e0) {
                const float* erow = g.e0 + (long)gm * g.lde0 + nbase;
#pragma unroll
                for (int nt = 0; nt < NT; ++nt) ev[nt] = *reinterpret_cast<const float4*>(erow + nt * 16);
            } else if (g.epi == EPI_ACCUM) {
#pragma unroll
                for (int nt = 0; nt < NT; ++nt) ev[nt] = *reinterpret_cast<const float4*>(yrow + nbase + nt * 16);
            }
#pragma unroll
            for (int nt = 0; nt < NT; ++nt) {
                const int nn = nbase + nt * 16;
                const v4f a = acc[s][mt][nt];
                float4 v = make_float4(a[0], a[1], a[2], a[3]);
                if constexpr (F16) {
                    constexpr float u = 1.f / (F16_WEIGHT_SCALE * F16_ACT_SCALE);
                    v = make_float4(v.x * u, v.y * u, v.z * u, v.w * u);
                }
                if (bp) v = f4_add(v, bv[nt]);
                if (radd_here) v = f4_add(rv[nt], v);
                if (y16) {
                    if (rok[mt])
                        *reinterpret_cast<uint2*>(reinterpret_cast<unsigned short*>(g.y[seg]) + (long)gm * g.ldy + nn) =
                            make_uint2(pack_bf16_rne(v.x, v.y), pack_bf16_rne(v.z, v.w));
                    continue;
                }
                if (g.epi == EPI_RELU_RES) {
                    const float4 x = ev[nt];
                    v = make_float4(fmaxf(v.x, 0.f) + x.x, fmaxf(v.y, 0.f) + x.y, fmaxf(v.z, 0.f) + x.z, fmaxf(v.w, 0.f) + x.w);
                }
                if (g.epi == EPI_ACCUM || g.epi == EPI_ADD_E0) v = f4_add(ev[nt], v);
                if constexpr (!F16) {
                    if (g.dmask && rok[mt] && (g.dmask_cols == 0 || nn < g.dmask_cols)) {
                        const unsigned mk = *reinterpret_cast<const unsigned*>(g.dmask + (long)gm * g.lddm + nn);
                        v = make_float4((mk & 0xffu) ? v.x * g.dscale : 0.f, (mk & 0xff00u) ? v.y * g.dscale : 0.f,
                                        (mk & 0xff0000u) ? v.z * g.dscale : 0.f, (mk & 0xff000000u) ? v.w * g.dscale : 0.f);
                    }
                }
                if (rok[mt]) *reinterpret_cast<float4*>(yrow + nn) = v;
            }
        }
    }
#ifdef DIGAT_GEMM_TIMERS
    if (lane == 0 && (blockIdx.x & 15) < 8) {
        const unsigned long long gt_end = GT_NOW();
        atomicAdd(&g_gemm_timers[0], gt_wait); atomicAdd(&g_gemm_timers[1], gt_bar); atomicAdd(&g_gemm_timers[2], gt_body);
        atomicAdd(&g_gemm_timers[3], gt_steps); atomicAdd(&g_gemm_timers[5], gt_end - gt_loop_end);
        atomicAdd(&g_gemm_timers[6], 1ull); atomicAdd(&g_gemm_timers[7], gt_end - gt_enter);
    }
#endif
}

template <int MT, bool KTAIL, bool TW = false>
__global__ void __launch_bounds__(256) gemm_skinny_kernel(const GemmArgs g) {
    __shared__ float red[4][MT * 20][64];
    const int tile = blockIdx.x;
    const int mtile = tile / g.ntiles, ntile = tile - mtile * g.ntiles;
    const int tid = threadIdx.x, lane = tid & 63, wave = tid >> 6;
    const int lr = lane & 15, lq = lane >> 4;
    const int m0 = mtile * (MT * 16), n0 = ntile * 80;
    const int seg = n0 / g.nseg;
    const int nbase = n0 - seg * g.nseg;
    const float* const wseg = g.w[seg];
    const int nkb = (g.K + 15) >> 4;

    const float* arow[MT][2];
    bool aok[MT];
#pragma unroll
    for (int mt = 0; mt < MT; ++mt) {
        const int gm = m0 + mt * 16 + lr;
        aok[mt] = gm < g.M;
        arow[mt][0] = g.a0 + (long)(aok[mt] ? gm : 0) * g.lda0;
        arow[mt][1] = g.a1 ? g.a1 + (long)(aok[mt] ? gm : 0) * g.lda1 : arow[mt][0];
    }
    const float* brow[5];
    bool bok[5];
#pragma unroll
    for (int nt = 0; nt < 5; ++nt) {
        const int nn = nbase + nt * 16 + lr;
        bok[nt] = nn < g.nseg;
        brow[nt] = TW ? wseg + (bok[nt] ? nn : 0) : wseg + (long)(bok[nt] ? nn : 0) * g.K;
    }
    auto load_block = [&](int kb, float4* a, float4* b) {
        const int k = kb * 16 + 4 * lq;
        const int kc = (KTAIL && k >= g.K) ? g.K - 4 : k;
        const float mk = (KTAIL && k >= g.K) ? 0.f : 1.f;
#pragma unroll
        for (int mt = 0; mt < MT; ++mt) {
            const float* p = kc < g.k0 ? arow[mt][0] + kc : arow[mt][1] + (kc - g.k0);
            const float4 v = *reinterpret_cast<const float4*>(p);
            a[mt] = KTAIL ? make_float4(v.x * mk, v.y * mk, v.z * mk, v.w * mk) : v;
        }
#pragma unroll
        for (int nt = 0; nt < 5; ++nt) {
            float4 v;
            if constexpr (TW) {
                const float* c = brow[nt] + (long)kc * g.nseg;
                v = make_float4(c[0], c[g.nseg], c[2 * (long)g.nseg], c[3 * (long)g.nseg]);
            } else {
// ... 418 lines not shown
        const int w = (kg == 0 || kg == 3) ? mine : other;
        const int sh = kg < 2 ? 0 : 8;
        xsc = ((w >> sh) & 0xff) | (((w >> (16 + sh)) & 0xff) << 8);
    };

    v4f acc[NSUB][NT];
#pragma unroll
    for (int s = 0; s < NSUB; ++s)
#pragma unroll
        for (int nt = 0; nt < NT; ++nt) acc[s][nt] = (v4f){0.f, 0.f, 0.f, 0.f};

    load_x(0);
    issue_b(0);
    for (int kt = 0; kt < KT; ++kt) {
        const int krel = g.K - kt * 128;
        const int nks = krel >= 32 ? 4 : (krel + 7) >> 3;
#pragma unroll
        for (int s = 0; s < NSUB; ++s) {
            const int step = kt * NSUB + s;
            asm volatile("s_waitcnt vmcnt(0)" ::: "memory");
            __builtin_amdgcn_s_barrier();
            if (s == 0) split_x();
            if (step + 1 < nsteps) issue_b(step + 1);
            if (s == NSUB - 1 && kt + 1 < KT) load_x(kt + 1);
            const uint4* Bi = Bs[step & 1];
            const int lslot = kg * 80 + lr;
            const uint2 sch = *reinterpret_cast<const uint2*>(reinterpret_cast<const unsigned char*>(Bi) + 40960 + ((0 * 4 + kg) * 16 + lr) * 8);
            const uint2 scl = *reinterpret_cast<const uint2*>(reinterpret_cast<const unsigned char*>(Bi) + 40960 + ((1 * 4 + kg) * 16 + lr) * 8);
#pragma unroll
            for (int nt = 0; nt < NT; ++nt) {
                const int sl = lslot + nt * 16;
                const uint4 q1a = Bi[1280 + sl], q1b = Bi[1280 + 320 + sl];
                const uint4 q2a = Bi[1920 + sl], q2b = Bi[1920 + 320 + sl];
                const v8i wq1 = (v8i){(int)q1a.x, (int)q1a.y, (int)q1a.z, (int)q1a.w, (int)q1b.x, (int)q1b.y, (int)q1b.z, (int)q1b.w};
                const v8i wq2 = (v8i){(int)q2a.x, (int)q2a.y, (int)q2a.z, (int)q2a.w, (int)q2b.x, (int)q2b.y, (int)q2b.z, (int)q2b.w};
                const int sh = (int)(nt < 4 ? sch.x : sch.y), sl8 = (int)(nt < 4 ? scl.x : scl.y);
                v4f c = acc[s][nt];
                c = f8c_mma<0>(nt & 3, wq2, xq1, c, sl8, xsc);
                c = f8c_mma<1>(nt & 3, wq1, xq2, c, sh, xsc);
#pragma unroll
                for (int ks = 0; ks < 4; ++ks) {
                    if (ks < nks) {
                        const bf16x8 wh = __builtin_bit_cast(bf16x8, Bi[ks * 320 + sl]);
                        c = __builtin_amdgcn_mfma_f32_16x16x32_f16(__builtin_bit_cast(half8, wh), __builtin_bit_cast(half8, xh[ks]), c, 0, 0, 0);
                    }
                }
                acc[s][nt] = c;
            }
        }
    }

    if (g.range_flag && __builtin_amdgcn_ballot_w64(!(amax < 65504.f)) != 0 && lane == 0) atomicOr(g.range_flag, 1u);
    const int gv = m0 + wm * 16 + lr;
    const bool rok = gv < Mv;
    const int gvc = rok ? gv : Mv - 1;
    const int gm = (g.rowidx && !g.gather_only) ? g.rowidx[gvc] : gvc;
    const bool has_e0 = g.epi == EPI_RELU_RES || g.epi == EPI_ADD_E0;
    constexpr float u = 1.f / (F16_WEIGHT_SCALE * F16_ACT_SCALE);
#pragma unroll
    for (int s = 0; s < NSUB; ++s) {
        const int ncol0 = (strip0 + s) * 80;
        const int seg = ncol0 / g.nseg;
        const int nbase = ncol0 - seg * g.nseg + kg * 4;
        const float* const bp = g.bias[seg];
        const bool radd_here = g.radd && seg == g.radd_seg;
        float* const yrow = g.y[seg] + (long)gm * g.ldy;
        float4 bv[NT], rv[NT], ev[NT];
        if (bp) {
#pragma unroll
            for (int nt = 0; nt < NT; ++nt) bv[nt] = *reinterpret_cast<const float4*>(bp + nbase + nt * 16);
        }
        if (radd_here) {
            const float* rrow = g.radd + (long)(gm / g.rows_per_b) * g.nseg + nbase;
#pragma unroll
            for (int nt = 0; nt < NT; ++nt) rv[nt] = *reinterpret_cast<const float4*>(rrow + nt * 16);
        }
        if (has_e0) {
            const float* erow = g.e0 + (long)gm * g.lde0 + nbase;
#pragma unroll
            for (int nt = 0; nt < NT; ++nt) ev[nt] = *reinterpret_cast<const float4*>(erow + nt * 16);
        } else if (g.epi == EPI_ACCUM) {
#pragma unroll
            for (int nt = 0; nt < NT; ++nt) ev[nt] = *reinterpret_cast<const float4*>(yrow + nbase + nt * 16);
        }
#pragma unroll
        for (int nt = 0; nt < NT; ++nt) {
            const v4f a = acc[s][nt];
            float4 v = make_float4(a[0] * u, a[1] * u, a[2] * u, a[3] * u);
            if (bp) v = f4_add(v, bv[nt]);
            if (radd_here) v = f4_add(rv[nt], v);
            if (g.epi == EPI_RELU_RES) {
                const float4 x = ev[nt];
                v = make_float4(fmaxf(v.x, 0.f) + x.x, fmaxf(v.y, 0.f) + x.y, fmaxf(v.z, 0.f) + x.z, fmaxf(v.w, 0.f) + x.w);
            }
            if (g.epi == EPI_ACCUM || g.epi == EPI_ADD_E0) v = f4_add(ev[nt], v);
            if (rok) *reinterpret_cast<float4*>(yrow + nbase + nt * 16) = v;
        }
    }
}

static std::mutex g_wsplit_mu;
static std::unordered_map<const void*, int> g_wsplit_format;
static void wsplit_note(const void* image, int format) {
    std::lock_guard<std::mutex> lock(g_wsplit_mu);
    g_wsplit_format[image] = format;
}
static int wsplit_forget(const void* image) {
    std::lock_guard<std::mutex> lock(g_wsplit_mu);
    return g_wsplit_format.erase(image) ? 1 : 0;
}
static int wsplit_format_of(const void* image) {
    std::lock_guard<std::mutex> lock(g_wsplit_mu);
    const auto it = g_wsplit_format.find(image);
    return it == g_wsplit_format.end() ? -1 : it->second;
}
static double gemm_row_bytes(const GemmArgs& g) {
    double out = 0.0;
    for (int sgm = 0; sgm < g.nsegs; ++sgm)
        out += ((g.fp8_segs >> sgm) & 1) ? (double)g.nseg + 4.0 * (g.nseg / 80) : (((g.bf16_segs >> sgm) & 1) ? 2.0 * g.nseg : 4.0 * g.nseg);
    double in = 4.0 * g.K;
    if (g.epi == EPI_RELU_RES || g.epi == EPI_ADD_E0 || g.epi == EPI_ACCUM) in += 4.0 * g.nseg;
    if (g.epi == EPI_GATE) in += 4.0 * g.nseg * (g.e2 ? 3 : 2);
    if (g.radd) in += 4.0 * g.nseg / (g.rows_per_b > 0 ? g.rows_per_b : 1);
    return in + out;
}

static int launch_gemm(GemmArgs g, hipStream_t st, int kind = DIGAT_KERNEL_LINEAR) {
    if (g.M <= 0) return DIGAT_OK;
    const GemmPlan p = gemm_plan(g, kind);
    if (p.status) return p.status;
    if (p.kernel == GEMM_PER_SEGMENT) {
        for (int sgm = 0; sgm < g.nsegs; ++sgm) {
            GemmArgs one = g;
            one.w[0] = g.w[sgm]; one.bias[0] = g.bias[sgm]; one.y[0] = g.y[sgm]; one.nsegs = 1;
            if (sgm == g.radd_seg) one.radd_seg = 0; else one.radd = nullptr;
            const int rc = launch_gemm(one, st, kind);
            if (rc) return rc;
        }
        return DIGAT_OK;
    }
    if (p.image_format >= 0) {
        const int made_as = wsplit_format_of(g.wsplit);
        if (made_as >= 0 && made_as != p.image_format) return DIGAT_ERR_ARG;
    }
    const int Ntot = g.nseg * g.nsegs;
    const bool listed = g.rowidx != nullptr && !g.gather_only;
    if (listed && g_prof.enabled) {
        g.exec_rows = g_prof.rows_dev + kind;
        g_prof.flops_per_row[kind] = 2.0 * (double)Ntot * g.K; g_prof.rows_nominal[kind] += g.M;
        g_prof.bytes_per_row[kind] = gemm_row_bytes(g);
    }
    ProfScope prof(kind, listed ? 0.0 : 2.0 * g.M * (double)Ntot * g.K, st, listed ? 0.0 : (double)g.M * gemm_row_bytes(g));
    g.mtiles = p.mtiles; g.ntiles = p.ntiles;
    switch (p.kernel) {
#define DIGAT_GEMM_LAUNCH(id, ...) case GEMM_##id: hipLaunchKernelGGL((__VA_ARGS__), dim3(p.grid), dim3(p.block), 0, st, g); break;
        DIGAT_GEMM_KERNELS(DIGAT_GEMM_LAUNCH)
#undef DIGAT_GEMM_LAUNCH
        default: return DIGAT_ERR_ARG;
    }
    DIGAT_CHECK_LAUNCH();
    return DIGAT_OK;
}

static GemmArgs gemm_plain(const float* x, long ldx, const float* w, const float* b, float* y, long ldy,
                           int M, int N, int K, int transW) {
    GemmArgs g;
    memset(&g, 0, sizeof(g));
    g.a0 = x; g.lda0 = ldx; g.k0 = K; g.a1 = nullptr; g.lda1 = 0;
    g.w[0] = w; g.bias[0] = b; g.y[0] = y; g.ldy = ldy;
    g.nseg = N; g.nsegs = 1; g.M = M; g.K = K; g.transW = transW; g.epi = EPI_NONE;
    return g;
}
```

digat_amd/csrc/digat_gemm_plan.h:

```cpp
#pragma once
#include <stdint.h>
#include "../../include/digat_hip.h"

enum { EPI_NONE = 0, EPI_RELU_RES = 1, EPI_GATE = 2, EPI_ACCUM = 3,
       EPI_ADD_E0 = 4 };

struct GemmArgs {
    const float* a0; long lda0; int k0;
    const float* a1; long lda1;
    const float* w[3]; const float* bias[3]; float* y[3]; long ldy;
    int nseg, nsegs, M, K, transW;
    int epi;
    const float* e0; long lde0; const float* e1; long lde1; const float* e2; long lde2;
    int mtiles, ntiles;
    const unsigned short* wsplit;
    const float* radd; int radd_seg, rows_per_b;
    unsigned long long* exec_rows;
    const int* rowidx; const int* nrows_dev;
    int gather_only;
    int m_dispatch;
    int x3_segs;
    int x1_segs;
    int bf16_segs;
    int fp8_segs; long ldy8;
    int format;
    unsigned* range_flag;
    const uint8_t* dmask; long lddm; float dscale;
    int dmask_cols;
};

#define DIGAT_GEMM_KERNELS(X)                                        \
    X(F16F8C_3, gemm_f16f8c_kernel<3>)                               \
    X(F16F8C_1, gemm_f16f8c_kernel<1>)                               \
    X(SKINNY_TW_2, gemm_skinny_kernel<2, false, true>)               \
    X(SKINNY_TW_1, gemm_skinny_kernel<1, false, true>)               \
    X(SKINNY_SPLIT_F16_2, gemm_skinny_split_kernel<2, true>)         \
    X(SKINNY_SPLIT_F16_1, gemm_skinny_split_kernel<1, true>)         \
    X(SKINNY_SPLIT_BF16_2, gemm_skinny_split_kernel<2, false>)       \
    X(SKINNY_SPLIT_BF16_1, gemm_skinny_split_kernel<1, false>)       \
    X(SKINNY_2_KTAIL, gemm_skinny_kernel<2, true, false>)            \
    X(SKINNY_2, gemm_skinny_kernel<2, false, false>)                 \
    X(SKINNY_1_KTAIL, gemm_skinny_kernel<1, true, false>)            \
    X(SKINNY_1, gemm_skinny_kernel<1, false, false>)                 \
    X(STRIP_3_F16_64, gemm_bf16x6s_kernel<3, true, 1, false>)        \
    X(STRIP_1_F16_64, gemm_bf16x6s_kernel<1, true, 1, false>)        \
    X(STRIP_3_BF16_64, gemm_bf16x6s_kernel<3, false, 1, false>)      \
    X(STRIP_1_BF16_64, gemm_bf16x6s_kernel<1, false, 1, false>)      \
    X(STRIP_3_F16_FULL, gemm_bf16x6s_kernel<3, true, 2, true>)       \
    X(STRIP_3_F16, gemm_bf16x6s_kernel<3, true, 2, false>)           \
    X(STRIP_3_BF16, gemm_bf16x6s_kernel<3, false, 2, false>)         \
    X(STRIP_1_F16, gemm_bf16x6s_kernel<1, true, 2, false>)           \
    X(STRIP_1_BF16, gemm_bf16x6s_kernel<1, false, 2, false>)         \
    X(F32_128_PROJ, gemm_f32_kernel<128, 80, 4, 1, 1, 1>)            \
    X(F32_128, gemm_f32_kernel<128, 80, 4, 1, 1, 0>)                 \
    X(F32_64, gemm_f32_kernel<64, 80, 4, 1, 2, 0>)                   \
    X(F32_32, gemm_f32_kernel<32, 64, 1, 4, 2, 0>)

enum GemmKernel {
    GEMM_NONE,
    GEMM_PER_SEGMENT,
#define DIGAT_GEMM_ENUM(id, ...) GEMM_##id,
    DIGAT_GEMM_KERNELS(DIGAT_GEMM_ENUM)
#undef DIGAT_GEMM_ENUM
};

static inline const char* gemm_kernel_name(int kernel) {
#define DIGAT_GEMM_NAME(id, ...) if (kernel == GEMM_##id) return #__VA_ARGS__;
    DIGAT_GEMM_KERNELS(DIGAT_GEMM_NAME)
#undef DIGAT_GEMM_NAME
    return kernel == GEMM_PER_SEGMENT ? "per segment" : "none";
}

struct GemmPlan {
    int status;
    int kernel;
    int mtiles, ntiles;
    unsigned grid, block;
    int image_format;
};

static inline bool gemm_kernel_takes_row_list(int kernel) {
    return kernel == GEMM_F16F8C_3 || kernel == GEMM_F16F8C_1 || (kernel >= GEMM_STRIP_3_F16_64 && kernel <= GEMM_STRIP_1_BF16);
}

static inline GemmPlan gemm_plan(const GemmArgs& g, int kind = DIGAT_KERNEL_LINEAR) {
    GemmPlan p = {DIGAT_OK, GEMM_NONE, 0, 0, 0, 256, -1};
    const int Ntot = g.nseg * g.nsegs;
    const int Md = g.m_dispatch > 0 ? g.m_dispatch : g.M;
    const auto tiles = [&](int kernel, int mtiles, int ntiles, bool round8) {
        p.kernel = kernel; p.mtiles = mtiles; p.ntiles = ntiles;
        p.grid = round8 ? (unsigned)(((mtiles * ntiles + 7) / 8) * 8) : (unsigned)(mtiles * ntiles);
        if (g.rowidx && !gemm_kernel_takes_row_list(kernel)) p.status = DIGAT_ERR_ARG;
        return p;
    };

    if (g.format == DIGAT_GEMM_F16F8C && g.wsplit) {
        const bool ok = g.nseg % 80 == 0 && g.K % 4 == 0 && g.k0 == g.K && !g.a1 && !g.transW && g.lda0 % 4 == 0 &&
                        ((uintptr_t)g.a0 & 15) == 0 && g.ldy % 4 == 0 && g.lde0 % 4 == 0 &&
                        (g.epi == EPI_NONE || g.epi == EPI_RELU_RES || g.epi == EPI_ACCUM || g.epi == EPI_ADD_E0) &&
                        !g.x1_segs && !g.x3_segs && !g.bf16_segs && !g.fp8_segs && !g.dmask;
        if (!ok) { p.status = DIGAT_ERR_ARG; return p; }
        const int strips = Ntot / 80;
        p.image_format = DIGAT_GEMM_F16F8C;
        p.block = 512;
        return strips % 3 == 0 ? tiles(GEMM_F16F8C_3, (g.M + 127) / 128, strips / 3, true)
                               : tiles(GEMM_F16F8C_1, (g.M + 127) / 128, strips, true);
    }
    if (Md < 2048 && g.nseg % 80 == 0 && g.transW && g.nsegs == 1 && g.K % 16 == 0 && g.k0 == g.K && !g.radd && !g.a1) {
        const int ntiles = Ntot / 80;
        if (((g.M + 31) / 32) * ntiles >= 480 || g.K >= 800) return tiles(GEMM_SKINNY_TW_2, (g.M + 31) / 32, ntiles, false);
        return tiles(GEMM_SKINNY_TW_1, (g.M + 15) / 16, ntiles, false);
    }
    if (Md < 2048 && g.wsplit && g.nseg % 80 == 0 && !g.transW && g.K % 8 == 0 && g.k0 % 8 == 0 && !g.radd && !g.rowidx &&
        g.ldy % 4 == 0 && g.lda0 % 4 == 0 && (!g.a1 || g.lda1 % 4 == 0) && g.lde0 % 4 == 0 && g.lde1 % 4 == 0 && g.lde2 % 4 == 0 &&
        (g.epi == EPI_NONE || g.epi == EPI_RELU_RES || g.epi == EPI_GATE || g.epi == EPI_ACCUM)) {
        if (g.format != DIGAT_GEMM_BF16X6 && g.format != DIGAT_GEMM_F16X3) p.status = DIGAT_ERR_ARG;
        p.image_format = g.format;
        const int ntiles = Ntot / 80;
        const bool mt2 = ((g.M + 31) / 32) * ntiles >= 320;
        const bool f16 = g.format == DIGAT_GEMM_F16X3;
        return tiles(mt2 ? (f16 ? GEMM_SKINNY_SPLIT_F16_2 : GEMM_SKINNY_SPLIT_BF16_2) : (f16 ? GEMM_SKINNY_SPLIT_F16_1 : GEMM_SKINNY_SPLIT_BF16_1),
                     mt2 ? (g.M + 31) / 32 : (g.M + 15) / 16, ntiles, false);
    }
    if (Md < 2048 && g.nseg % 80 == 0 && !g.transW && g.K % 4 == 0 && g.k0 % 16 == 0 && !g.radd) {
        const int ntiles = Ntot / 80;
        const bool ktail = (g.K & 15) != 0;
        if (((g.M + 31) / 32) * ntiles >= 480 || g.K >= 800)
            return tiles(ktail ? GEMM_SKINNY_2_KTAIL : GEMM_SKINNY_2, (g.M + 31) / 32, ntiles, false);
        return tiles(ktail ? GEMM_SKINNY_1_KTAIL : GEMM_SKINNY_1, (g.M + 15) / 16, ntiles, false);
    }
    const int cfg = Md >= 2048 ? 0 : ((g.nsegs > 1 && g.nseg % 80 == 0) ? 1 : 2);
    const int bn = cfg == 2 ? 64 : 80;
    if (g.nsegs > 1 && g.nseg % bn != 0) return tiles(GEMM_PER_SEGMENT, 0, 0, false);
    if (g.wsplit && cfg == 0 && g.nseg % 80 == 0 && g.K % 4 == 0 && g.K >= 32 && g.ldy % 4 == 0 && g.lde0 % 4 == 0 &&
        (g.epi == EPI_NONE || g.epi == EPI_RELU_RES || g.epi == EPI_ACCUM || g.epi == EPI_ADD_E0) && g.k0 == g.K && !g.transW) {
        if (g.format != DIGAT_GEMM_BF16X6 && g.format != DIGAT_GEMM_F16X3) p.status = DIGAT_ERR_ARG;
        else if (g.rowidx && (unsigned long long)g.M * (unsigned long long)g.lda0 * 4ull >= (1ull << 32)) p.status = DIGAT_ERR_SHAPE;
        p.image_format = g.format;
        const bool f16 = g.format == DIGAT_GEMM_F16X3;
        const int strips = Ntot / 80;
        const bool three = strips % 3 == 0;
        const int ntiles = three ? strips / 3 : strips;
        if (((g.M + 127) / 128) * ntiles < 400 && (f16 || !g.rowidx)) {
            const int k = f16 ? (three ? GEMM_STRIP_3_F16_64 : GEMM_STRIP_1_F16_64) : (three ? GEMM_STRIP_3_BF16_64 : GEMM_STRIP_1_BF16_64);
            return tiles(k, (g.M + 63) / 64, ntiles, true);
        }
        const int k = three ? (f16 ? (!g.x1_segs && !g.x3_segs ? GEMM_STRIP_3_F16_FULL : GEMM_STRIP_3_F16) : GEMM_STRIP_3_BF16)
                            : (f16 ? GEMM_STRIP_1_F16 : GEMM_STRIP_1_BF16);
        return tiles(k, (g.M + 127) / 128, ntiles, true);
    }
    const int bm = cfg == 0 ? 128 : (cfg == 1 ? 64 : 32);
    const int k = cfg == 0 ? (kind == DIGAT_KERNEL_PROJ ? GEMM_F32_128_PROJ : GEMM_F32_128) : (cfg == 1 ? GEMM_F32_64 : GEMM_F32_32);
    return tiles(k, (g.M + bm - 1) / bm, (Ntot + bn - 1) / bn, true);
}

static inline bool gemm_takes_row_list(const GemmArgs& g) { return gemm_kernel_takes_row_list(gemm_plan(g).kernel); }
```

digat_amd/csrc/digat_kernels.hip:

```cpp
#include <hip/hip_runtime.h>
#include <stdint.h>
#include <string.h>
#include <stdlib.h>
#include <atomic>
#include <initializer_list>
#include <mutex>
#include <unordered_map>
#include <utility>

#include "../../include/digat_hip.h"
#include "digat_encoder_plan.h"

typedef float v4f __attribute__((ext_vector_type(4)));

#define DIGAT_CHECK_LAUNCH()                                   \
    do {                                                       \
        if (hipGetLastError() != hipSuccess) return DIGAT_ERR_LAUNCH; \
    } while (0)

static inline size_t align_up(size_t v, size_t a) { return (v + a - 1) / a * a; }
struct Arena {
    char* base; size_t cap, used; bool ok;
    Arena() : base(nullptr), cap(SIZE_MAX), used(0), ok(true) {}
    Arena(void* p, size_t n) : base((char*)p), cap(n), used(0), ok(p != nullptr) {}
// ... 313 lines not shown
static thread_local const void* tl_premade_image = nullptr;
struct PremadeImage {
    const void* prev;
    explicit PremadeImage(const void* image) : prev(tl_premade_image) { tl_premade_image = image; }
    ~PremadeImage() { tl_premade_image = prev; }
};
static int launch_split(const float* w0, const float* w1, const float* w2, int nseg, int nsegs, int K, void* wsplit, hipStream_t st,
                        int transposed = 0, int format = 0) {
    if (format != 0 && format != 1 && format != DIGAT_GEMM_F16F8C) return DIGAT_ERR_ARG;
    if (wsplit && wsplit == tl_premade_image) return format == 0 ? DIGAT_OK : DIGAT_ERR_ARG;
    if (format == DIGAT_GEMM_F16F8C) {
        if (transposed) return DIGAT_ERR_ARG;
        const long total = (long)((nseg * nsegs + 79) / 80) * ((K + 127) / 128) * 320;
        int blocks = (int)((total + 255) / 256);
        if (blocks > 2048) blocks = 2048;
        wsplit_note(wsplit, format);
        hipLaunchKernelGGL(split_weights_f8c_kernel, dim3(blocks), dim3(256), 0, st, w0, w1, w2, nseg, nsegs, K, (unsigned char*)wsplit);
        DIGAT_CHECK_LAUNCH();
        return DIGAT_OK;
    }
    const long total = (long)nseg * nsegs * K;
    int blocks = (int)((total + 255) / 256);
    if (blocks > 2048) blocks = 2048;
    wsplit_note(wsplit, format);
    hipLaunchKernelGGL(split_weights_tiled_kernel, dim3(blocks), dim3(256), 0, st, w0, w1, w2, nseg, nsegs, K, (unsigned short*)wsplit, transposed,
                       format == 1 ? 2 : 3);
    DIGAT_CHECK_LAUNCH();
    return DIGAT_OK;
}

size_t digat_split_job_bytes(int rows, int cols, int layout, int matrices) {
    if (rows <= 0 || cols <= 0 || (matrices != 1 && matrices != 3)) return 0;
    if (layout == 0) return digat_split_weights_bytes(rows * matrices, cols);
    if (layout == 1) return matrices == 1 ? digat_split_weights_bytes(cols, rows) : digat_split_weights_bytes(cols, 3 * rows);
    return 0;
}
int digat_split_jobs(const digat_split_job* jobs, int njobs, void* stream) {
    if (!jobs || njobs < 0 || njobs > SPLIT_MAX_JOBS) return DIGAT_ERR_ARG;
    if (njobs == 0) return DIGAT_OK;
    SplitJobsDev all;
    memset(&all, 0, sizeof(all));
    long most = 0;
    for (int k = 0; k < njobs; ++k) {
        const digat_split_job& j = jobs[k];
        const bool three = j.w1 != nullptr || j.w2 != nullptr;
        if (!j.w0 || !j.image || j.rows <= 0 || j.cols <= 0 || (three && (!j.w1 || !j.w2)) || (j.layout != 0 && j.layout != 1)) return DIGAT_ERR_ARG;
        SplitJobDev& o = all.j[k];
        o.w0 = j.w0; o.w1 = three ? j.w1 : j.w0; o.w2 = three ? j.w2 : j.w0; o.out = (unsigned short*)j.image;
        if (j.layout == 0) { o.nseg = j.rows; o.nsegs = three ? 3 : 1; o.K = j.cols; o.transposed = 0; }
        else { o.nseg = j.cols; o.nsegs = 1; o.K = three ? 3 * j.rows : j.rows; o.transposed = three ? 2 : 1; }
        const long total = (long)((o.nseg * o.nsegs + 79) / 80) * 80 * ((o.K + 31) / 32) * 4;
        if (total > most) most = total;
        wsplit_note(j.image, 0);
    }
    long bx = (most + 255) / 256;
    if (bx > 2048) bx = 2048;
    hipLaunchKernelGGL(split_weights_jobs_kernel, dim3((unsigned)bx, (unsigned)njobs), dim3(256), 0, (hipStream_t)stream, all);
    DIGAT_CHECK_LAUNCH();
    return DIGAT_OK;
}

int digat_forget_split_image(const void* wsplit) { return wsplit && wsplit_forget(wsplit) ? DIGAT_OK : DIGAT_ERR_ARG; }

int digat_gather_tables(const digat_gather_job* jobs, int njobs, void* stream) {
    if (!jobs || njobs < 0 || njobs > GATHER_MAX_JOBS) return DIGAT_ERR_ARG;
    if (njobs == 0) return DIGAT_OK;
    GatherTableJobs all;
    memset(&all, 0, sizeof(all));
    long most = 0;
    for (int k = 0; k < njobs; ++k) {
        const digat_gather_job& j = jobs[k];
        if (j.rows < 0 || j.row_bytes <= 0 || (j.rows > 0 && (!j.src || !j.dst || !j.idx)) || (j.idx2 && j.inner <= 0)) return DIGAT_ERR_ARG;
        all.job[k] = j;
        if (!j.idx2) all.job[k].inner = 1;
        const long units = (j.row_bytes & 15) == 0 ? j.rows * (j.row_bytes >> 4) : j.rows * j.row_bytes;
        if (units > most) most = units;
    }
    if (most == 0) return DIGAT_OK;
    long bx = (most + 255) / 256;
    if (bx > 1024) bx = 1024;
    hipLaunchKernelGGL(gather_tables_kernel, dim3((unsigned)bx, (unsigned)njobs), dim3(256), 0, (hipStream_t)stream, all);
    DIGAT_CHECK_LAUNCH();
    return DIGAT_OK;
}

int digat_user_row_runs(const float* ue, const uint8_t* Au, const uint8_t* cat_mask, const int64_t* cat_idx, int B, int H, int U, int C1, int d,
                        int32_t* row_group, int64_t* leaders, int32_t* n_runs, void* workspace, size_t workspace_bytes, void* stream) {
    if (!ue || !Au || !cat_mask || !cat_idx || !row_group || !leaders || !n_runs || !workspace || B <= 0 || H < 0 || U <= 0 || C1 <= 0 || d <= 0)
        return DIGAT_ERR_ARG;
    if (d % 4 || ((long)H * d) % 4) return DIGAT_ERR_SHAPE;
    if (workspace_bytes < (size_t)B) return DIGAT_ERR_WORKSPACE;
    hipStream_t st = (hipStream_t)stream;
    uint8_t* same = (uint8_t*)workspace;
    ProfScope prof(DIGAT_KERNEL_GLUE, (double)B * ((double)H * d * 4 + (double)U * U + C1 + 8.0 * H), st);
    hipLaunchKernelGGL(user_rows_same_kernel, dim3(B), dim3(256), 0, st, (const uint4*)ue, Au, cat_mask, cat_idx, B, (long)H * d / 4, U * U, C1, H, same);
    DIGAT_CHECK_LAUNCH();
    hipLaunchKernelGGL(user_row_runs_kernel, dim3(1), dim3(1024), 0, st, (const uint8_t*)same, B, row_group, leaders, n_runs);
    DIGAT_CHECK_LAUNCH();
    return DIGAT_OK;
}

int digat_split_proj_weights(const float* W, const float* F1, const float* F2, int d, void* wsplit, int format, void* stream) {
    if (!W || !F1 || !F2 || !wsplit || d <= 0) return DIGAT_ERR_ARG;
    return launch_split(W, F1, F2, d, 3, d, wsplit, (hipStream_t)stream, 0, format);
}

size_t digat_split_ctx_fused_bytes(int d) { return d > 0 ? ctxfused_image_bytes(d) : 0; }
int digat_split_ctx_fused_weights(const float* W, int d, void* image, void* stream) {
    if (!W || !image || d <= 0) return DIGAT_ERR_ARG;
    if (d % 8) return DIGAT_ERR_SHAPE;
    const long total = (long)(ctxfused_image_bytes(d) / 16);
    hipLaunchKernelGGL(split_weights_ctxfused_kernel, dim3((unsigned)((total + 255) / 256)), dim3(256), 0, (hipStream_t)stream, W, d, (uint4*)image);
    DIGAT_CHECK_LAUNCH();
    return DIGAT_OK;
}

int digat_split_weights(const float* W, int N, int K, void* wsplit, int format, void* stream) {
    if (!W || !wsplit || N <= 0 || K <= 0) return DIGAT_ERR_ARG;
    return launch_split(W, W, W, N, 1, K, wsplit, (hipStream_t)stream, 0, format);
}

#ifdef DIGAT_CF_TIMERS
extern "C" int digat_debug_cf_timers(double* out16) {
    unsigned long long h[16];
    if (hipDeviceSynchronize() != hipSuccess || hipMemcpyFromSymbol(h, HIP_SYMBOL(g_cf_timers), sizeof(h)) != hipSuccess) return DIGAT_ERR_LAUNCH;
    for (int k = 0; k < 16; ++k) { out16[k] = (double)h[k]; h[k] = 0; }
    return hipMemcpyToSymbol(HIP_SYMBOL(g_cf_timers), h, sizeof(h)) == hipSuccess ? DIGAT_OK : DIGAT_ERR_LAUNCH;
}
#endif
#ifdef DIGAT_GEMM_TIMERS
int digat_debug_gemm_timers(double* out8) {
    unsigned long long h[8];
    if (hipDeviceSynchronize() != hipSuccess || hipMemcpyFromSymbol(h, HIP_SYMBOL(g_gemm_timers), sizeof(h)) != hipSuccess) return DIGAT_ERR_LAUNCH;
    for (int k = 0; k < 8; ++k) { out8[k] = (double)h[k]; h[k] = 0; }
    return hipMemcpyToSymbol(HIP_SYMBOL(g_gemm_timers), h, sizeof(h)) == hipSuccess ? DIGAT_OK : DIGAT_ERR_LAUNCH;
}
#endif

static std::atomic<int> g_train_bf16{0};
int digat_set_train_precision(int bf16) { return g_train_bf16.exchange(bf16 ? 1 : 0); }

int digat_linear_f32x3(const float* x, int64_t ldx, const float* w, const float* b, float* y, int64_t ldy,
                       int M, int N, int K, void* wsplit, int format, void* stream) {
    if (!x || !w || !y || !wsplit || M < 0 || N <= 0 || K <= 0) return DIGAT_ERR_ARG;
    if (K % 8 || ldx % 4 || N % 80) return DIGAT_ERR_SHAPE;
    const int rcs = launch_split(w, w, w, N, 1, K, wsplit, (hipStream_t)stream, 0, format);
    if (rcs) return rcs;
    GemmArgs g = gemm_plain(x, ldx, w, b, y, ldy, M, N, K, 0);
    g.wsplit = (const unsigned short*)wsplit; g.format = format;
    if (g_train_bf16 && format != DIGAT_GEMM_F16F8C) g.x1_segs = 7;
    return launch_gemm(g, (hipStream_t)stream, DIGAT_KERNEL_PROJ);
}

struct NewsCtxWs { float *qv, *kq, *glob; };
static NewsCtxWs news_ctx_carve(Arena& a, int B, int d) {
    const size_t bd = (size_t)B * d;
    return NewsCtxWs{a.take<float>(bd), a.take<float>(bd), a.take<float>(bd)};
}
size_t digat_news_ctx_workspace_bytes(int B, int N, int d) { (void)N; Arena a; news_ctx_carve(a, B, d); return a.used; }

int digat_news_ctx_fwd(const float* X, const uint8_t* mask, const float* Kc, const float* Qc, const float* bQc,
                       const float* Wg, const float* bg, const float* addend, float* out, int B, int N, int d,
                       void* workspace, size_t workspace_bytes, void* stream) {
    if (!X || !mask || !Kc || !Qc || !Wg || !out || !workspace || B < 0 || N <= 0 || d <= 0) return DIGAT_ERR_ARG;
    if (d % 4 || N > DIGAT_MAX_NODES) return DIGAT_ERR_SHAPE;
    Arena ar(workspace, workspace_bytes);
    const NewsCtxWs w = news_ctx_carve(ar, B, d);
    if (!ar.ok) return DIGAT_ERR_WORKSPACE;
    if (B == 0) return DIGAT_OK;
    hipStream_t st = (hipStream_t)stream;
    float *qv = w.qv, *kq = w.kq, *glob = w.glob;
    const long ldx = (long)N * d;
    int rc;
    rc = launch_gemm(gemm_plain(X, ldx, Qc, bQc, qv, d, B, d, d, 0), st);
    if (rc) return rc;
    rc = launch_gemm(gemm_plain(qv, d, Kc, nullptr, kq, d, B, d, d, 1), st);
    if (rc) return rc;
    rc = launch_pool(X, ldx, kq, mask, nullptr, glob, B, N, d, st);
    if (rc) return rc;
    GemmArgs g = gemm_plain(X, ldx, Wg, bg, out, d, B, d, 2 * d, 0);
    g.k0 = d; g.a1 = glob; g.lda1 = d;
    g.epi = EPI_GATE; g.e0 = X; g.lde0 = ldx; g.e1 = glob; g.lde1 = d; g.e2 = addend; g.lde2 = d;
    return launch_gemm(g, st);
}

struct UserCtxWs { float *qv, *kq, *T, *T2; };
static UserCtxWs user_ctx_carve(Arena& a, int B, int C1, int d) {
    const size_t bd = (size_t)B * d, bcd = (size_t)B * C1 * d;
    return UserCtxWs{a.take<float>(bd), a.take<float>(bd), a.take<float>(bcd), a.take<float>(bcd)};
}
size_t digat_user_ctx_workspace_bytes(int B, int U, int H, int C1, int d) { (void)U; (void)H; Arena a; user_ctx_carve(a, B, C1, d); return a.used; }

int digat_topic_pool_fwd(const float* Xu, const float* kq, const int64_t* cat_idx, float* out,
                         int B, int U, int H, int C1, int d, void* stream) {
    if (!Xu || !kq || !cat_idx || !out || B < 0 || H < 0 || U < H || C1 <= 0 || d <= 0) return DIGAT_ERR_ARG;
    return launch_topic(Xu, (long)U * d, kq, cat_idx, out, B, H, C1, d, (hipStream_t)stream);
}

static int user_ctx_run(const float* Xu, const uint8_t* cat_mask, const int64_t* cat_idx, const int* group, const float* c_n,
                        const float* Ku, const float* Qu, const float* bQu, const float* Fa, const float* bFa,
                        const float* Kua, const float* Qua, const float* bQua, const float* addend, float* out,
                        int B, int U, int H, int C1, int d, const UserCtxWs& w, hipStream_t st) {
    float *qv = w.qv, *kq = w.kq, *T = w.T, *T2 = w.T2;
    int rc;
    rc = launch_gemm(gemm_plain(c_n, d, Qu, bQu, qv, d, B, d, d, 0), st);
    if (rc) return rc;
    rc = launch_gemm(gemm_plain(qv, d, Ku, nullptr, kq, d, B, d, d, 1), st);
    if (rc) return rc;
    rc = launch_topic(Xu, (long)U * d, kq, cat_idx, T, B, H, C1, d, st, group);
    if (rc) return rc;
    GemmArgs g = gemm_plain(T, d, Fa, bFa, T2, d, B * C1, d, d, 0);
    g.epi = EPI_RELU_RES; g.e0 = T; g.lde0 = d;
    rc = launch_gemm(g, st);
    if (rc) return rc;
    rc = launch_gemm(gemm_plain(c_n, d, Qua, bQua, qv, d, B, d, d, 0), st);
    if (rc) return rc;
    rc = launch_gemm(gemm_plain(qv, d, Kua, nullptr, kq, d, B, d, d, 1), st);
    if (rc) return rc;
    return launch_pool(T2, (long)C1 * d, kq, cat_mask, addend, out, B, C1, d, st);
}

int digat_user_ctx_fwd(const float* Xu, const uint8_t* cat_mask, const int64_t* cat_idx, const float* c_n,
                       const float* Ku, const float* Qu, const float* bQu, const float* Fa, const float* bFa,
                       const float* Kua, const float* Qua, const float* bQua, const float* addend, float* out,
                       int B, int U, int H, int C1, int d, void* workspace, size_t workspace_bytes, void* stream) {
    if (!Xu || !cat_mask || !cat_idx || !c_n || !Ku || !Qu || !Fa || !Kua || !Qua || !out || !workspace)
        return DIGAT_ERR_ARG;
    if (B < 0 || H < 0 || U < H || C1 <= 0 || d <= 0) return DIGAT_ERR_ARG;
    if (d % 4 || C1 > DIGAT_MAX_NODES || H > TOPIC_MAX_H) return DIGAT_ERR_SHAPE;
    Arena ar(workspace, workspace_bytes);
    const UserCtxWs w = user_ctx_carve(ar, B, C1, d);
    if (!ar.ok) return DIGAT_ERR_WORKSPACE;
    if (B == 0) return DIGAT_OK;
    return user_ctx_run(Xu, cat_mask, cat_idx, nullptr, c_n, Ku, Qu, bQu, Fa, bFa, Kua, Qua, bQua, addend, out, B, U, H, C1, d, w,
                        (hipStream_t)stream);
}

__global__ void __launch_bounds__(256) transpose_kernel(const float* __restrict__ in, float* __restrict__ out, int d) {
    __shared__ float tile[32][33];
    const int bx = blockIdx.x * 32, by = blockIdx.y * 32;
    for (int r = threadIdx.y; r < 32; r += 8) {
        const int y = by + r, x = bx + threadIdx.x;
        if (y < d && x < d) tile[r][threadIdx.x] = in[(long)y * d + x];
    }
    __syncthreads();
    for (int r = threadIdx.y; r < 32; r += 8) {
        const int y = bx + r, x = by + threadIdx.x;
        if (y < d && x < d) out[(long)y * d + x] = tile[threadIdx.x][r];
    }
}

size_t digat_fold_workspace_bytes(int d) { return 2 * align_up((size_t)d * d * 4, 256); }

int digat_fold_attention(const float* K, const float* Q, const float* bQ, float* Wf, float* bf, int d,
                         void* workspace, size_t workspace_bytes, void* stream) {
    if (!K || !Q || !Wf || !bf || !workspace || d <= 0) return DIGAT_ERR_ARG;
    if (d % 4) return DIGAT_ERR_SHAPE;
    if (workspace_bytes < digat_fold_workspace_bytes(d)) return DIGAT_ERR_WORKSPACE;
    hipStream_t st = (hipStream_t)stream;
    float* Kt = (float*)workspace;
    float* Qt = (float*)((char*)workspace + align_up((size_t)d * d * 4, 256));
    const dim3 grid((d + 31) / 32, (d + 31) / 32), block(32, 8);
    hipLaunchKernelGGL(transpose_kernel, grid, block, 0, st, K, Kt, d);
    hipLaunchKernelGGL(transpose_kernel, grid, block, 0, st, Q, Qt, d);
    DIGAT_CHECK_LAUNCH();
    int rc = launch_gemm(gemm_plain(Kt, d, Qt, nullptr, Wf, d, d, d, d, 0), st);
    if (rc) return rc;
    if (bQ) return launch_gemm(gemm_plain(bQ, d, Kt, nullptr, bf, d, 1, d, d, 0), st);
    return hipMemsetAsync(bf, 0, (size_t)d * 4, st) == hipSuccess ? DIGAT_OK : DIGAT_ERR_LAUNCH;
}

#include "digat_encoder.inc"

static double g_prof_last_live_fraction = -1.0;
double digat_profile_live_row_fraction(void) { return g_prof_last_live_fraction; }
static double g_prof_last_gemm_bytes[DIGAT_KERNEL_KINDS] = {0.0};
static double g_prof_last_part_ms[XATTN_PARTS] = {0.0}, g_prof_last_part_bytes[XATTN_PARTS] = {0.0};
static int g_prof_last_part_launches[XATTN_PARTS] = {0};
int digat_profile_xattn_parts(double* ms, double* bytes, int* launches) {
    for (int p = 0; p < XATTN_PARTS; ++p) {
        if (ms) ms[p] = g_prof_last_part_ms[p];
        if (bytes) bytes[p] = g_prof_last_part_bytes[p];
        if (launches) launches[p] = g_prof_last_part_launches[p];
    }
    return DIGAT_OK;
}
int digat_profile_gemm_bytes(double* bytes_per_kind) {
    if (!bytes_per_kind) return DIGAT_ERR_ARG;
    for (int k = 0; k < DIGAT_KERNEL_KINDS; ++k) bytes_per_kind[k] = g_prof_last_gemm_bytes[k];
    return DIGAT_OK;
}

int digat_profile_pause(int paused) {
    if (!g_prof.ev) return DIGAT_ERR_ARG;
    g_prof.enabled = paused ? 0 : 1;
    return DIGAT_OK;
}

__global__ void digat_region_marker_kernel(int id, int* sink) { if (sink && id < 0) *sink = id; }
int digat_profile_marker(int id, void* stream) {
    hipLaunchKernelGGL(digat_region_marker_kernel, dim3(1), dim3(1), 0, (hipStream_t)stream, id, (int*)nullptr);
    DIGAT_CHECK_LAUNCH();
    return DIGAT_OK;
}

int digat_profile_set_kinds(unsigned mask) {
// ... 99 lines not shown
```

digat_amd/graphEncoders.py:

```python
from __future__ import annotations

import contextlib
import math
import threading

import torch
import torch.nn as nn

from . import _lib
from .layers import ScaledDotProductAttention

_TLS = threading.local()


def derive_user_graph(user_graph, user_category_mask, user_category_indices, category_num: int):
    if user_graph is not None:
        return user_graph, user_category_mask
    if user_category_mask is not None:
        raise ValueError("user_graph=None derives the category mask too: pass user_category_mask=None")
    from .util import user_graphs_from_indices
    return user_graphs_from_indices(user_category_indices, category_num)


class GraphEncoder(nn.Module):
    def __init__(self, config, news_embedding_dim: int):
        super().__init__()
        self.news_graph_size = config.news_graph_size
        self.user_graph_size = config.max_history_num + config.category_num
        self.max_history_num = config.max_history_num
        self.category_num = config.category_num + 1
        self.news_embedding_dim = news_embedding_dim
        self.graph_depth = config.graph_depth
        self.dropout_rate = float(config.dropout_rate)
        self.attention_scalar = math.sqrt(float(self.news_embedding_dim))
        self.topic_node_embedding = nn.Parameter(torch.zeros([config.category_num, self.news_embedding_dim]))

    def initialize(self):
        nn.init.zeros_(self.topic_node_embedding)

    def forward(self, news_graph_embeddings, news_graph, news_graph_mask, user_news_embedding, user_graph,
                user_category_mask, user_category_indices):
        raise Exception('Function forward must be implemented at sub-class')

    def inference(self, news_graph_embeddings, news_graph, news_graph_mask, user_news_embedding, user_graph,
                  user_category_mask, user_category_indices, news_graph_context):
        raise Exception('Function inference must be implemented at sub-class')


class DIGAT(GraphEncoder):
    def __init__(self, config, news_embedding_dim: int):
        super().__init__(config, news_embedding_dim)
        d, L = self.news_embedding_dim, self.graph_depth
        if d % 4 != 0:
            raise ValueError("digat_amd needs news_embedding_dim % 4 == 0 (float4 rows)")
        if L > _lib.DIGAT_MAX_DEPTH or max(self.news_graph_size, self.user_graph_size) > _lib.DIGAT_MAX_NODES:
            raise ValueError("graph_depth <= %d and graph sizes <= %d are supported"
                             % (_lib.DIGAT_MAX_DEPTH, _lib.DIGAT_MAX_NODES))
        self.candidate_attention = ScaledDotProductAttention(d, d, d)
        self.news_graph_W = nn.Linear(d * 2, d, bias=True)
        self.user_news_K = nn.Linear(d, d, bias=False)
        self.user_news_Q = nn.Linear(d, d, bias=True)
        self.featureAffine = nn.Linear(d, d, bias=True)
        self.userAttention = ScaledDotProductAttention(d, d, d)
        for g in ("news", "user"):
            setattr(self, f"{g}_graph_attention_W", nn.ModuleList([nn.Linear(d, d, bias=True) for _ in range(L)]))
            setattr(self, f"{g}_graph_attention_ffn1", nn.ModuleList([nn.Linear(d, d, bias=False) for _ in range(L)]))
            setattr(self, f"{g}_graph_attention_ffn2", nn.ModuleList([nn.Linear(d, d, bias=False) for _ in range(L)]))
            setattr(self, f"{g}_graph_attention_ffn3", nn.ModuleList([nn.Linear(d, d, bias=True) for _ in range(L)]))
            setattr(self, f"{g}_graph_attention_a", nn.ModuleList([nn.Linear(d, 1, bias=False) for _ in range(L)]))
        self._param_block = None
        self.projection_mode = "auto"
        self._resolved_pm = None
        self._range_flag = None
        self.range_fallback = False
        self.corpus_activation_max = None
        self.pass_rows = 4096
        self.user_xattn_mode = "auto"
        self.news_xattn_mode = "auto"
        self.corpus_xattn_hint = {}
        self.side_stream = "auto"
        self.live_rows = True
        self.fused_user_context = False

    def initialize(self):
        super().initialize()
        relu_gain = nn.init.calculate_gain('relu')
        leaky_gain = nn.init.calculate_gain('leaky_relu', 0.2)
        for g in ("news", "user"):
            for i in range(self.graph_depth):
                nn.init.xavier_uniform_(getattr(self, f"{g}_graph_attention_W")[i].weight)
                nn.init.zeros_(getattr(self, f"{g}_graph_attention_W")[i].bias)
                nn.init.xavier_uniform_(getattr(self, f"{g}_graph_attention_a")[i].weight, gain=leaky_gain)
                for f in ("ffn1", "ffn2", "ffn3"):
                    nn.init.xavier_uniform_(getattr(self, f"{g}_graph_attention_{f}")[i].weight, gain=relu_gain)
                nn.init.zeros_(getattr(self, f"{g}_graph_attention_ffn3")[i].bias)
        self.candidate_attention.initialize()
        nn.init.xavier_uniform_(self.news_graph_W.weight)
        nn.init.zeros_(self.news_graph_W.bias)
        nn.init.xavier_uniform_(self.user_news_K.weight)
        nn.init.xavier_uniform_(self.user_news_Q.weight)
        nn.init.zeros_(self.user_news_Q.bias)
        nn.init.xavier_uniform_(self.featureAffine.weight, gain=relu_gain)
        nn.init.zeros_(self.featureAffine.bias)
        self.userAttention.initialize()

    @contextlib.contextmanager
    def launch_options(self, side_stream=None, live_rows=None, shared_users=None):
        table = _TLS.__dict__.setdefault("opts", {})
        prev = table.get(id(self))
        cur = dict(prev or {})
        if side_stream is not None:
            if side_stream not in ("auto", "on", "off"):
                raise ValueError("side_stream must be 'auto', 'on' or 'off'")
            cur["side_stream"] = side_stream
        if live_rows is not None:
            cur["live_rows"] = bool(live_rows)
        if shared_users is not None:
            cur["detect_shared_users"] = bool(shared_users)
        table[id(self)] = cur
        try:
            yield self
        finally:
            if prev is None:
                table.pop(id(self), None)
            else:
                table[id(self)] = prev

    def _launch_option(self, name):
        return _TLS.__dict__.get("opts", {}).get(id(self), {}).get(name, getattr(self, name))

    def resolved_xattn_mode(self, g: str) -> str:
        mode = getattr(self, f"{g}_xattn_mode", "auto")
        return self.corpus_xattn_hint.get(g, "auto") if mode == "auto" else mode

    def _apply(self, fn, *args, **kwargs):
        self._param_block = None
        return super()._apply(fn, *args, **kwargs)

    def _params(self) -> "_lib.Params":
        pm = self.resolved_projection_mode()
        fmt = self.gemm_format()
        ptrs = tuple(p.data_ptr() for p in self.parameters())
        if self._param_block is not None and self._param_block[0] == ptrs and self._param_block[2] == self._fold_key():
            return self._call_block(self._param_block[1])
        for p in self.parameters():
            if p.device.type != "cuda" or p.dtype != torch.float32 or not p.is_contiguous():
                raise _lib.DigatHipError("DIGAT parameters must be contiguous float32 CUDA tensors "
                                         "(call model.cuda()); there is no CPU path")
        P = _lib.Params()
        P.d, P.depth, P.category_num = self.news_embedding_dim, self.graph_depth, self.category_num - 1
        P.flags = self._flags()
        P.topic_node_embedding = self.topic_node_embedding.data_ptr()
        P.cand_K = self.candidate_attention.K.weight.data_ptr()
        P.cand_Q = self.candidate_attention.Q.weight.data_ptr()
        P.cand_bQ = self.candidate_attention.Q.bias.data_ptr()
        P.news_graph_W = self.news_graph_W.weight.data_ptr()
        P.news_graph_b = self.news_graph_W.bias.data_ptr()
        P.user_news_K = self.user_news_K.weight.data_ptr()
        P.user_news_Q = self.user_news_Q.weight.data_ptr()
        P.user_news_bQ = self.user_news_Q.bias.data_ptr()
        P.featureAffine_W = self.featureAffine.weight.data_ptr()
        P.featureAffine_b = self.featureAffine.bias.data_ptr()
        P.userAtt_K = self.userAttention.K.weight.data_ptr()
        P.userAtt_Q = self.userAttention.Q.weight.data_ptr()
        P.userAtt_bQ = self.userAttention.Q.bias.data_ptr()
        for g, arr in (("news", P.news), ("user", P.user)):
            for i in range(self.graph_depth):
                lp = arr[i]
                W = getattr(self, f"{g}_graph_attention_W")[i]
                lp.W, lp.bW = W.weight.data_ptr(), W.bias.data_ptr()
                lp.F1 = getattr(self, f"{g}_graph_attention_ffn1")[i].weight.data_ptr()
                lp.F2 = getattr(self, f"{g}_graph_attention_ffn2")[i].weight.data_ptr()
                F3 = getattr(self, f"{g}_graph_attention_ffn3")[i]
                lp.F3, lp.b3 = F3.weight.data_ptr(), F3.bias.data_ptr()
                lp.a = getattr(self, f"{g}_graph_attention_a")[i].weight.data_ptr()
        P._splits = []
        if pm in ("bf16x6", "bf16x6-pq3", "pq-bf16", "pq-bf16-x1", "pq-fp8", "fp16x3", "fp16-fp8c") and self.news_embedding_dim % 80 == 0:
            L_ = _lib.lib()
            d = self.news_embedding_dim
            lfmt = _lib.GEMM_F16F8C if pm == "fp16-fp8c" else fmt
            nbytes = L_.digat_split_weights_bytes_format(3 * d, d, lfmt)
            for g, arr in (("news", P.news), ("user", P.user)):
                for i in range(self.graph_depth):
                    buf = _lib.split_buffer(nbytes, self.topic_node_embedding.device)
                    _lib.check(L_.digat_split_proj_weights(
                        getattr(self, f"{g}_graph_attention_W")[i].weight.data_ptr(),
                        getattr(self, f"{g}_graph_attention_ffn1")[i].weight.data_ptr(),
                        getattr(self, f"{g}_graph_attention_ffn2")[i].weight.data_ptr(), d, buf.data_ptr(), lfmt,
                        _lib.stream_ptr()), "digat_split_proj_weights")
                    arr[i].wsplit = buf.data_ptr()
                    P._splits.append(buf)
            buf = _lib.split_buffer(L_.digat_split_weights_bytes(d, d), self.topic_node_embedding.device)
            _lib.check(L_.digat_split_weights(self.featureAffine.weight.data_ptr(), d, d, buf.data_ptr(), fmt, _lib.stream_ptr()),
                       "digat_split_weights")
            P.featureAffine_wsplit = buf.data_ptr()
            P._splits.append(buf)
            if fmt == _lib.GEMM_F16X3:
                P.range_flag = self.range_flag().data_ptr()
        P._folds = None
        if not self.training:
            P._folds = self._fold_attention()
            (P.cand_fold_W, P.cand_fold_b, P.user_news_fold_W, P.user_news_fold_b,
             P.userAtt_fold_W, P.userAtt_fold_b) = (t.data_ptr() for t in P._folds)
            if P._splits:
                L_, d, dev = _lib.lib(), self.news_embedding_dim, self.topic_node_embedding.device

                def image(rows, K, fn, *args):
                    buf = _lib.split_buffer(L_.digat_split_weights_bytes(rows, K), dev)
                    _lib.check(fn(*args, buf.data_ptr(), fmt, _lib.stream_ptr()), "split")
                    P._splits.append(buf)
                    return buf.data_ptr()
                for i in range(self.graph_depth):
                    P.news[i].f3_wsplit = image(d, d, L_.digat_split_weights, self.news_graph_attention_ffn3[i].weight.data_ptr(), d, d)
                P.cand_fold_wsplit = image(d, d, L_.digat_split_weights, P.cand_fold_W, d, d)
                P.gate_wsplit = image(d, 2 * d, L_.digat_split_weights, self.news_graph_W.weight.data_ptr(), d, 2 * d)
                for l in range(self.graph_depth + 1):
                    third = self.user_graph_attention_ffn3[l].weight.data_ptr() if l < self.graph_depth else P.userAtt_fold_W
                    P.ctx_wsplit[l] = image(3 * d, d, L_.digat_split_proj_weights, P.user_news_fold_W, P.userAtt_fold_W, third, d)
                if fmt == _lib.GEMM_F16X3 and self.fused_user_context:
                    buf = _lib.split_buffer(L_.digat_split_ctx_fused_bytes(d), dev)
                    _lib.check(L_.digat_split_ctx_fused_weights(self.featureAffine.weight.data_ptr(), d, buf.data_ptr(), _lib.stream_ptr()),
                               "digat_split_ctx_fused_weights")
                    P._splits.append(buf)
                    P.featureAffine_fsplit = buf.data_ptr()
        self._param_block = (ptrs, P, self._fold_key())
        return self._call_block(P)

    def _call_block(self, P):
        Q = _lib.Params.from_buffer_copy(P)
        Q.flags = self._flags()
        return Q

    def resolved_projection_mode(self) -> str:
        return self._auto_base() if self.projection_mode == "auto" else self.projection_mode

    def gemm_format(self) -> int:
        pm = self.projection_mode
        if pm in ("fp16x3", "fp16-fp8c") or (pm in ("auto", "pq-bf16", "pq-fp8") and self._auto_base() == "fp16x3"):
            return _lib.GEMM_F16X3
        return _lib.GEMM_BF16X6

    def _auto_base(self) -> str:
        if self.news_embedding_dim % 80 != 0:
            return "bf16x6"
        ws = [m.weight for g in ("news", "user") for f in ("W", "ffn1", "ffn2") for m in getattr(self, f"{g}_graph_attention_{f}")]
        ws.append(self.featureAffine.weight)
        key = tuple((w.data_ptr(), w._version) for w in ws + [self.topic_node_embedding])
        key += (self.corpus_activation_max, self.range_fallback)
        if self._resolved_pm is None or self._resolved_pm[0] != key:
            amax = self.corpus_activation_max
            ok = amax is not None and not self.range_fallback
            if ok:
                wmax = float(torch.stack([w.detach().abs().max() for w in ws]).max())
                tmax = float(self.topic_node_embedding.detach().abs().max())
                ok = wmax < 32.0 and amax < 256.0 and tmax < 256.0
            self._resolved_pm = (key, "fp16x3" if ok else "bf16x6")
        return self._resolved_pm[1]

    def range_flag(self) -> torch.Tensor:
        dev = self.topic_node_embedding.device
        if self._range_flag is None or self._range_flag.device != dev:
            self._range_flag = torch.zeros(1, dtype=torch.int32, device=dev)
        return self._range_flag

    def range_overflowed(self, reset: bool = True) -> bool:
        if self._range_flag is None:
            return False
        hit = bool(int(self._range_flag.item()))
        if reset and hit:
            self._range_flag.zero_()
        return hit

    def _flags(self) -> int:
        pm = self.projection_mode
        return ({"auto": 0, "dense": 1, "sparse": 2}[self.resolved_xattn_mode("user")]
                | (4 if pm in ("bf16x6-pq3", "pq-bf16", "pq-fp8") else 0)
                | (8 if self.resolved_xattn_mode("news") == "sparse" else 0)
                | (16 if pm in ("pq-bf16", "pq-bf16-x1") else 0)
                | (32 if pm == "pq-bf16-x1" else 0)
                | (256 if pm == "pq-fp8" else 0)
                | (_lib.PARAMS_GEMM_F16X3 if self.gemm_format() == _lib.GEMM_F16X3 else 0)
                | (_lib.PARAMS_PROJ_F16F8C if pm == "fp16-fp8c" else 0)
                | (_lib.PARAMS_BD_TILED if self.pass_rows >= 2048 else 0)
                | {"auto": 0, "off": _lib.PARAMS_SIDE_STREAM_OFF, "on": _lib.PARAMS_SIDE_STREAM_ON}[self._launch_option("side_stream")]
                | (0 if self._launch_option("live_rows") else _lib.PARAMS_NO_LIVE_ROWS))

    def _fold_sources(self):
        ca, ua = self.candidate_attention, self.userAttention
        return ((ca.K.weight, ca.Q.weight, ca.Q.bias), (self.user_news_K.weight, self.user_news_Q.weight,
                                                        self.user_news_Q.bias), (ua.K.weight, ua.Q.weight, ua.Q.bias))

    def _fold_key(self):
        key = (self.training, self.resolved_projection_mode(), self.gemm_format()) + tuple(t._version for trio in self._fold_sources() for t in trio)
        for g in ("news", "user"):
            for f in ("W", "ffn1", "ffn2"):
                key += tuple(m.weight._version for m in getattr(self, f"{g}_graph_attention_{f}"))
        return key + (self.featureAffine.weight._version, bool(self.fused_user_context))

    def _fold_attention(self):
        L = _lib.lib()
        d = self.news_embedding_dim
        dev = self.topic_node_embedding.device
        nbytes = L.digat_fold_workspace_bytes(d)
        ws = _lib.workspace(nbytes, dev, "fold")
        out = []
        for K, Q, b in self._fold_sources():
            Wf = torch.empty((d, d), dtype=torch.float32, device=dev)
            bf = torch.empty((d,), dtype=torch.float32, device=dev)
            _lib.check(L.digat_fold_attention(K.data_ptr(), Q.data_ptr(), b.data_ptr(), Wf.data_ptr(), bf.data_ptr(), d,
                                              ws.data_ptr(), nbytes, _lib.stream_ptr()), "digat_fold_attention")
            out += [Wf, bf]
        return out

    def _eval_only(self, what: str):
        if self.training and self.dropout_rate > 0 and torch.is_grad_enabled():
            raise NotImplementedError(
                f"{what}: the HIP path implements eval-mode semantics (dropout = identity); "
                "call model.eval() / torch.no_grad(), or train through digat_amd.training")

    def compute_news_graph_context(self, news_graph_embeddings, news_graph_mask):
        X = _lib.f32(news_graph_embeddings)
        dev = _lib.require_device(X, news_graph_mask)
        B, N, d = X.shape
        mask = _lib.as_bytes(news_graph_mask)
        out = torch.empty((B, d), dtype=torch.float32, device=dev)
        if B == 0:
            return out
        L = _lib.lib()
        nbytes = L.digat_news_ctx_workspace_bytes(B, N, d)
        ws = _lib.workspace(nbytes, dev, "ctx")
        ca, g = self.candidate_attention, self.news_graph_W
        _lib.check(L.digat_news_ctx_fwd(X.data_ptr(), mask.data_ptr(), ca.K.weight.data_ptr(), ca.Q.weight.data_ptr(),
                                        ca.Q.bias.data_ptr(), g.weight.data_ptr(), g.bias.data_ptr(), None,
                                        out.data_ptr(), B, N, d, ws.data_ptr(), nbytes, _lib.stream_ptr()),
                   "digat_news_ctx_fwd")
        return out

    def compute_user_graph_context(self, user_graph_embeddings, user_category_mask, user_category_indices,
                                   news_graph_context):
        Xu = _lib.f32(user_graph_embeddings)
        c_n = _lib.f32(news_graph_context)
        dev = _lib.require_device(Xu, user_category_mask, user_category_indices, c_n)
        B, U, d = Xu.shape
        H, C1 = self.max_history_num, self.category_num
        mask = _lib.as_bytes(user_category_mask)
        idx = user_category_indices.to(torch.int64).contiguous()
        out = torch.empty((B, d), dtype=torch.float32, device=dev)
        if B == 0:
            return out
        L = _lib.lib()
        nbytes = L.digat_user_ctx_workspace_bytes(B, U, H, C1, d)
        ws = _lib.workspace(nbytes, dev, "ctx")
        ua = self.userAttention
        _lib.check(L.digat_user_ctx_fwd(Xu.data_ptr(), mask.data_ptr(), idx.data_ptr(), c_n.data_ptr(),
                                        self.user_news_K.weight.data_ptr(), self.user_news_Q.weight.data_ptr(),
                                        self.user_news_Q.bias.data_ptr(), self.featureAffine.weight.data_ptr(),
                                        self.featureAffine.bias.data_ptr(), ua.K.weight.data_ptr(),
                                        ua.Q.weight.data_ptr(), ua.Q.bias.data_ptr(), None, out.data_ptr(),
                                        B, U, H, C1, d, ws.data_ptr(), nbytes, _lib.stream_ptr()),
                   "digat_user_ctx_fwd")
        return out

    def _xattn(self, g: str, index: int, X, A, ctx, return_alpha: bool = False):
        X, ctx = _lib.f32(X), _lib.f32(ctx)
        dev = _lib.require_device(X, A, ctx)
        B, n, d = X.shape
        adj = _lib.as_bytes(A)
        out = torch.empty_like(X)
        alpha = torch.empty((B, n, n), dtype=torch.float32, device=dev) if return_alpha else None
        if B == 0:
            return (out, alpha) if return_alpha else out
        L = _lib.lib()
        nbytes = L.digat_xattn_workspace_bytes(B, n, d)
        ws = _lib.workspace(nbytes, dev, "xattn")
        W = getattr(self, f"{g}_graph_attention_W")[index]
        F3 = getattr(self, f"{g}_graph_attention_ffn3")[index]
        mode = self.resolved_xattn_mode(g)
        if mode == "sparse" and not return_alpha and n > 16 and d <= 1024:
            _lib.check(L.digat_xattn_fwd_mode(X.data_ptr(), adj.data_ptr(), ctx.data_ptr(), W.weight.data_ptr(), W.bias.data_ptr(),
                                              getattr(self, f"{g}_graph_attention_ffn1")[index].weight.data_ptr(),
                                              getattr(self, f"{g}_graph_attention_ffn2")[index].weight.data_ptr(),
                                              F3.weight.data_ptr(), F3.bias.data_ptr(),
                                              getattr(self, f"{g}_graph_attention_a")[index].weight.data_ptr(),
                                              out.data_ptr(), B, n, d, 2, ws.data_ptr(), nbytes, _lib.stream_ptr()),
                       "digat_xattn_fwd_mode")
            return out
        _lib.check(L.digat_xattn_fwd(X.data_ptr(), adj.data_ptr(), ctx.data_ptr(), W.weight.data_ptr(),
                                     W.bias.data_ptr(),
                                     getattr(self, f"{g}_graph_attention_ffn1")[index].weight.data_ptr(),
                                     getattr(self, f"{g}_graph_attention_ffn2")[index].weight.data_ptr(),
                                     F3.weight.data_ptr(), F3.bias.data_ptr(),
                                     getattr(self, f"{g}_graph_attention_a")[index].weight.data_ptr(),
                                     out.data_ptr(), _lib.ptr(alpha), B, n, d, ws.data_ptr(), nbytes,
                                     _lib.stream_ptr()), "digat_xattn_fwd")
        return (out, alpha) if return_alpha else out

    def compute_news_graph_embeddings(self, index, news_graph_embeddings, news_graph, user_graph_context):
        self._eval_only("compute_news_graph_embeddings")
        return self._xattn("news", index, news_graph_embeddings, news_graph, user_graph_context)

    def compute_user_graph_embeddings(self, index, user_graph_embeddings, user_graph, news_graph_context):
        self._eval_only("compute_user_graph_embeddings")
        return self._xattn("user", index, user_graph_embeddings, user_graph, news_graph_context)

    def _encode(self, news_graph_embeddings, news_graph, news_graph_mask, user_news_embedding, user_graph,
                user_category_mask, user_category_indices, news_graph_context, shared: bool = False):
        Xn, ue = _lib.f32(news_graph_embeddings), _lib.f32(user_news_embedding)
        dev = _lib.require_device(Xn, news_graph, news_graph_mask, ue, user_graph, user_category_mask,
                                  user_category_indices)
        B, N, d = Xn.shape
        H, C = self.max_history_num, self.category_num - 1
        if ue.shape != (B, H, d) or user_graph.shape[1] != H + C or N != self.news_graph_size:
            raise _lib.DigatHipError("input shapes do not match the encoder's configuration")
        An, Mn = _lib.as_bytes(news_graph), _lib.as_bytes(news_graph_mask)
        Au, cm = _lib.as_bytes(user_graph), _lib.as_bytes(user_category_mask)
        ci = user_category_indices.to(torch.int64).contiguous()
        c0 = None if news_graph_context is None else _lib.f32(news_graph_context)
        out_n = torch.empty((B, d), dtype=torch.float32, device=dev)
        out_u = torch.empty((B, d), dtype=torch.float32, device=dev)
        if B == 0:
            return out_n, out_u
        L = _lib.lib()
        nbytes = (L.digat_encoder_shared_workspace_bytes if shared else L.digat_encoder_workspace_bytes)(B, N, H, C, d, self.graph_depth)
        ws = _lib.workspace(nbytes, dev, "encoder")
        P = self._params()
        _lib.binding().encoder_fwd(_lib.addressof(P), bool(shared), Xn, An, Mn, ue, Au, cm, ci, c0, out_n, out_u, ws)
        return out_n, out_u

    def project_news_layer0(self, news_graph_embeddings):
        X = _lib.f32(news_graph_embeddings)
        dev = _lib.require_device(X)
        M, N, d = X.shape
        out = torch.empty((3, M, N, d), dtype=torch.float32, device=dev)
        if M:
            _lib.check(_lib.lib().digat_news_project0(self._params(), X.data_ptr(), out.data_ptr(), M, N, _lib.stream_ptr()),
                       "digat_news_project0")
        return out

# ... 514 lines not shown
```

include/digat_hip.h:

```cpp
#ifndef DIGAT_HIP_H
#define DIGAT_HIP_H

#include <stddef.h>
#include <stdint.h>

#ifdef __cplusplus
extern "C" {
#endif

#define DIGAT_ABI_VERSION 4
#define DIGAT_MAX_NODES 128
#define DIGAT_MAX_DEPTH 16

enum {
    DIGAT_OK = 0,
    DIGAT_ERR_ARG = 1,
    DIGAT_ERR_SHAPE = 2,
    DIGAT_ERR_WORKSPACE = 3,
    DIGAT_ERR_LAUNCH = 4
};

int digat_version(void);
const char* digat_error_string(int code);

int digat_linear_f32(const float* x, int64_t ldx, const float* w, const float* b, float* y, int64_t ldy,
                     int M, int N, int K, void* stream);

size_t digat_split_weights_bytes(int rows, int K);
int digat_forget_split_image(const void* wsplit);
int digat_split_proj_weights(const float* W, const float* F1, const float* F2, int d, void* wsplit, int format, void* stream);
int digat_split_weights(const float* W, int N, int K, void* wsplit, int format, void* stream);
int digat_linear_f32x3(const float* x, int64_t ldx, const float* w, const float* b, float* y, int64_t ldy,
                       int M, int N, int K, void* wsplit, int format, void* stream);

size_t digat_xattn_workspace_bytes(int B, int n, int d);
int digat_xattn_fwd(const float* X, const uint8_t* A, const float* ctx,
                    const float* W, const float* bW, const float* F1, const float* F2,
                    const float* F3, const float* b3, const float* a,
                    float* out, float* alpha_out, int B, int n, int d,
                    void* workspace, size_t workspace_bytes, void* stream);
int digat_xattn_fwd_mode(const float* X, const uint8_t* A, const float* ctx,
                         const float* W, const float* bW, const float* F1, const float* F2,
                         const float* F3, const float* b3, const float* a,
                         float* out, int B, int n, int d, int mode,
                         void* workspace, size_t workspace_bytes, void* stream);

int digat_xattn_fwd_lowprec(const float* X, const uint8_t* A, const float* ctx,
                            const float* W, const float* bW, const float* F1, const float* F2,
                            const float* F3, const float* b3, const float* a, const void* wsplit, int format,
                            float* out, int B, int n, int d, int pq,
                            void* workspace, size_t workspace_bytes, void* stream);

int digat_xattn_pairwise_fwd(const float* Pr, const float* Q, const float* h, const float* X,
                             const float* a, const uint8_t* A,
                             float* out, float* alpha, int B, int n, int d, void* stream);

size_t digat_news_ctx_workspace_bytes(int B, int N, int d);
int digat_news_ctx_fwd(const float* X, const uint8_t* mask,
                       const float* Kc, const float* Qc, const float* bQc,
                       const float* Wg, const float* bg,
                       const float* addend, float* out, int B, int N, int d,
                       void* workspace, size_t workspace_bytes, void* stream);

size_t digat_user_ctx_workspace_bytes(int B, int U, int H, int C1, int d);
int digat_user_ctx_fwd(const float* Xu, const uint8_t* cat_mask, const int64_t* cat_idx, const float* c_n,
                       const float* Ku, const float* Qu, const float* bQu,
                       const float* Fa, const float* bFa,
                       const float* Kua, const float* Qua, const float* bQua,
                       const float* addend, float* out, int B, int U, int H, int C1, int d,
                       void* workspace, size_t workspace_bytes, void* stream);

size_t digat_user_ctx_grouped_workspace_bytes(int B, int G, int U, int H, int C1, int d);
int digat_user_ctx_fwd_grouped(const float* Xu, const uint8_t* cat_mask, const int64_t* cat_idx, const int32_t* row_group,
                               const float* c_n,
                               const float* Ku, const float* Qu, const float* bQu,
                               const float* Fa, const float* bFa,
                               const float* Kua, const float* Qua, const float* bQua,
                               const float* addend, float* out, int B, int G, int U, int H, int C1, int d,
                               void* workspace, size_t workspace_bytes, void* stream);

int digat_user_nodes_build(const float* ue, const float* topic, const int32_t* row_group, float* Xu, long rows, long G, int H,
                           int C, int d, void* stream);

int digat_topic_pool_fwd(const float* Xu, const float* kq, const int64_t* cat_idx, float* out,
                         int B, int U, int H, int C1, int d, void* stream);

enum { DIGAT_XATTN_AUTO = 0, DIGAT_XATTN_DENSE = 1, DIGAT_XATTN_SPARSE = 2 };
enum { DIGAT_PROJ_PQ_X3 = 4 };
enum { DIGAT_NEWS_XATTN_SPARSE = 8 };
enum { DIGAT_PQ_BF16 = 16, DIGAT_PQ_X1 = 32 };
enum { DIGAT_PQ_FP8 = 256 };
enum { DIGAT_PARAMS_GEMM_F16X3 = 64 };
enum { DIGAT_PARAMS_BD_TILED = 128 };

typedef struct digat_layer_params {
    const float *W, *bW;
    const float *F1;
    const float *F2;
    const float *F3, *b3;
    const float *a;
    const void  *wsplit;
    const void  *f3_wsplit;
} digat_layer_params;

typedef struct digat_params {
    int32_t d;
    int32_t depth;
    int32_t category_num;
    int32_t flags;
    const float *topic_node_embedding;
    const float *cand_K, *cand_Q, *cand_bQ;
    const float *news_graph_W, *news_graph_b;
    const float *user_news_K, *user_news_Q, *user_news_bQ;
    const float *featureAffine_W, *featureAffine_b;
    const float *userAtt_K, *userAtt_Q, *userAtt_bQ;
    digat_layer_params news[DIGAT_MAX_DEPTH];
    digat_layer_params user[DIGAT_MAX_DEPTH];
    const float *cand_fold_W, *cand_fold_b;
    const float *user_news_fold_W, *user_news_fold_b;
    const float *userAtt_fold_W, *userAtt_fold_b;
    const void  *featureAffine_wsplit;
    const void  *cand_fold_wsplit, *gate_wsplit;
    const void  *ctx_wsplit[DIGAT_MAX_DEPTH + 1];
    uint32_t    *range_flag;
    const void  *featureAffine_fsplit;
} digat_params;

size_t digat_split_ctx_fused_bytes(int d);
int digat_split_ctx_fused_weights(const float* W, int d, void* image, void* stream);

size_t digat_fold_workspace_bytes(int d);
int digat_fold_attention(const float* K, const float* Q, const float* bQ, float* Wf, float* bf, int d,
                         void* workspace, size_t workspace_bytes, void* stream);

size_t digat_encoder_workspace_bytes(int B, int N, int H, int C, int d, int depth);
int digat_encoder_fwd(const digat_params* params,
                      const float* news_graph_embeddings, const uint8_t* news_graph,
                      const uint8_t* news_graph_mask, const float* user_news_embedding,
                      const uint8_t* user_graph, const uint8_t* user_category_mask,
                      const int64_t* user_category_indices, const float* news_graph_context,
                      float* out_news_context, float* out_user_context,
                      int B, int N, int H,
                      void* workspace, size_t workspace_bytes, void* stream);

enum { DIGAT_PARAMS_SIDE_STREAM_OFF = 512, DIGAT_PARAMS_SIDE_STREAM_ON = 1024, DIGAT_PARAMS_NO_LIVE_ROWS = 2048 };
enum { DIGAT_PARAMS_PROJ_F16F8C = 4096 };

size_t digat_encoder_grouped_workspace_bytes(int B, int N, int H, int C, int d, int depth);
int digat_encoder_fwd_grouped(const digat_params* params,
                              const float* news_graph_embeddings, const uint8_t* news_graph,
                              const uint8_t* news_graph_mask, const float* user_news_embedding_groups,
                              const uint8_t* user_graph_groups, const uint8_t* user_category_mask_groups,
                              const int64_t* user_category_indices_groups, const int32_t* row_group,
                              const float* news_graph_context, float* out_news_context, float* out_user_context,
                              int B, int G, int N, int H, void* workspace, size_t workspace_bytes, void* stream);

int digat_news_project0(const digat_params* params, const float* Xn, float* hpq, int M, int N, void* stream);
int digat_user_project0(const digat_params* params, const float* X, float* hpq, int M, void* stream);
int digat_news_context_queries(const digat_params* params, const float* c_n, float* out, int M, void* stream);
int digat_encoder_fwd_grouped_cached(const digat_params* params,
                                     const float* news_graph_embeddings, const uint8_t* news_graph, const uint8_t* news_graph_mask,
                                     const float* user_news_embedding_g, const uint8_t* user_graph_g,
                                     const uint8_t* user_category_mask_g, const int64_t* user_category_indices_g,
                                     const int32_t* row_group, const float* news_graph_context, const float* news_hpq0,
                                     const float* hist_hpq0, const float* topic_hpq0, const float* ctxq0,
                                     const int64_t* news_index, int64_t news_rows,
                                     float* out_news, float* out_user, int B, int G, int N, int H,
                                     void* workspace, size_t workspace_bytes, void* stream);

int digat_row_logits(const float* news_ctx, const float* user_ctx, float* logits, int B, int d, void* stream);

int digat_linear_bwd_input(const float* dy, int64_t lddy, const float* w, float* dx, int64_t lddx,
                           int M, int N, int K, int accumulate, void* stream);
int digat_linear_bwd_input_x3(const float* dy, int64_t lddy, const float* w, float* dx, int64_t lddx,
                              int M, int N, int K, int accumulate, void* wsplit, void* stream);
size_t digat_linear_bwd_weight_workspace(int M, int No, int Ni);
int digat_linear_bwd_weight(const float* dy, int64_t lddy, const float* x, int64_t ldx, float* dW, float* db,
                            int M, int No, int Ni, int accumulate, void* workspace, size_t workspace_bytes,
                            void* stream);
int digat_colsum(const float* x, int64_t ldx, float* out, int M, int N, int accumulate, void* stream);
int digat_dropout_fwd(const float* x, float* y, uint8_t* mask, int64_t n, float p, uint32_t seed, void* stream);
int digat_dropout_bwd(const float* dy, const uint8_t* mask, float* dx, int64_t n, float p, void* stream);
int digat_gate_fwd(const float* z, const float* l, int64_t ldl, const float* g, float* out, int B, int d, void* stream);
int digat_gate_bwd(const float* dout, const float* z, const float* l, int64_t ldl, const float* g,
                   float* dz, float* dl, float* dg, int B, int d, void* stream);
int digat_relu_res_fwd(const float* y, const float* t, float* out, int64_t n, void* stream);
int digat_relu_mask(const float* dout, const float* y, float* dy, int64_t n, void* stream);
int digat_attn_pool_fwd(const float* feat, int64_t ld_b, const float* kq, const uint8_t* mask, float* out,
                        float* alpha_out, int B, int n, int d, void* stream);
int digat_attn_pool_bwd(const float* feat, int64_t ld_b, const float* kq, const uint8_t* mask, const float* alpha,
                        const float* dout, float* dfeat, int64_t ldd_b, float* dkq, int B, int n, int d,
                        int accumulate_dfeat, void* stream);
int digat_topic_pool_fwd_train(const float* Xu, const float* kq, const int64_t* cat_idx, float* out, float* alpha_out,
                               int B, int U, int H, int C1, int d, void* stream);
int digat_topic_pool_bwd(const float* Xu, const float* kq, const int64_t* cat_idx, const float* alpha, const float* dT,
                         float* dXu, float* dkq, int B, int U, int H, int C1, int d, void* stream);
int digat_xattn_project(const float* X, const float* r, const float* W, const float* bW, const float* F1,
                        const float* F2, float* h, float* Pr, float* Q, int B, int n, int d, void* stream);
int digat_xattn_project_x3(const float* X, const float* r, const float* W, const float* bW, const float* F1, const float* F2,
                           float* h, float* Pr, float* Q, int B, int n, int d, void* wsplit, void* stream);
int digat_xattn_pairwise_fwd_train(const float* Pr, const float* Q, const float* h, const float* X, const float* a,
                                   const uint8_t* A, float* out, float* alpha, float* s_pre, float* alpha_drop,
                                   uint8_t* amask, float p, uint32_t seed, int B, int n, int d, void* stream);
size_t digat_xattn_pairwise_bwd_workspace(int B, int n, int d);
int digat_xattn_pairwise_bwd(const float* dOut, const float* out, const float* Xres, const float* Pr, const float* Q,
                             const float* h, const float* a, const uint8_t* A, const float* alpha, const float* s_pre,
                             const uint8_t* amask, float p, float* dPr, float* dQ, float* dh, float* da,
                             int accumulate_da, int B, int n, int d, void* workspace, size_t workspace_bytes,
                             void* stream);
int digat_sum_nodes(const float* dP, float* dr, int B, int n, int d, void* stream);

int digat_set_train_precision(int bf16);

enum { DIGAT_GEMM_BF16X6 = 0, DIGAT_GEMM_F16X3 = 1 };
enum { DIGAT_GEMM_F16F8C = 2 };
size_t digat_split_weights_bytes_format(int rows, int K, int format);

int digat_row_logits_bwd(const float* dlogits, const float* news_ctx, const float* user_ctx, float* dnews, float* duser, int B, int d,
                         void* stream);
int digat_click_loss(const float* logits, int B, int K, float* loss, float* dlogits, void* stream);

typedef struct digat_opt_tensor { float* p; const float* g; float* m; float* v; int64_t n; float weight_decay; int32_t pad; } digat_opt_tensor;
int digat_opt_chunk(void);
int digat_clip_adam_step(const void* tensors, const int32_t* chunk_tensor, const int64_t* chunk_off, int nchunks, float* scratch, float max_norm,
                         float lr, float beta1, float beta2, float eps, int step, void* stream);

typedef struct digat_split_job {
    const float *w0, *w1, *w2;
    int32_t rows, cols, layout, reserved;
    void* image;
} digat_split_job;
size_t digat_split_job_bytes(int rows, int cols, int layout, int matrices);
int digat_split_jobs(const digat_split_job* jobs, int njobs, void* stream);

size_t digat_xattn_train_save_bytes(int B, int n, int d);
size_t digat_xattn_train_workspace_bytes(int B, int n, int d);
enum { DIGAT_TRAIN_XATTN_AUTO = 0, DIGAT_TRAIN_XATTN_SPARSE = 1, DIGAT_TRAIN_XATTN_DENSE = 2 };
int digat_xattn_fwd_train(const float* X, const uint8_t* A, const float* ctx, const float* W, const float* bW, const float* F1,
                          const float* F2, const float* F3, const float* b3, const float* a, float* out, float p_alpha,
                          uint32_t seed, float p_in, uint32_t seed_in, int B, int n, int d, void* save, size_t save_bytes, void* workspace,
                          size_t workspace_bytes, const void* proj_image, int xattn_mode, void* stream);
int digat_xattn_bwd(const float* dOut, const float* out, const float* X, const uint8_t* A, const float* ctx, const float* W,
                    const float* F1, const float* F2, const float* F3, const float* a, float p_alpha, float p_in, const void* save,
                    size_t save_bytes, float* dX, float* dctx, float* dW, float* dbW, float* dF1, float* dF2, float* dF3,
                    float* db3, float* da, int B, int n, int d, void* workspace, size_t workspace_bytes, const void* bwd_image,
                    int xattn_mode, void* stream);
size_t digat_news_ctx_train_save_bytes(int B, int N, int d);
size_t digat_news_ctx_train_workspace_bytes(int B, int N, int d);
int digat_news_ctx_fwd_train(const float* X, const uint8_t* mask, const float* Kc, const float* Qc, const float* bQc,
                             const float* Wg, const float* bg, float* out, float p_gate, uint32_t seed, int B, int N, int d,
                             void* save, size_t save_bytes, void* workspace, size_t workspace_bytes,
                             const float* prev , void* stream);
int digat_news_ctx_bwd(const float* dout, const float* X, const uint8_t* mask, const float* Kc, const float* Qc, const float* Wg,
                       float p_gate, const void* save, size_t save_bytes, float* dX, float* dKc, float* dQc, float* dbQc,
                       float* dWg, float* dbg, int B, int N, int d, int accumulate_params, void* workspace, size_t workspace_bytes,
                       void* stream);
size_t digat_user_ctx_train_save_bytes(int B, int U, int H, int C1, int d);
size_t digat_user_ctx_train_workspace_bytes(int B, int U, int H, int C1, int d);
int digat_user_ctx_fwd_train(const float* Xu, const uint8_t* cat_mask, const int64_t* cat_idx, const float* c_n, const float* Ku,
                             const float* Qu, const float* bQu, const float* Fa, const float* bFa, const float* Kua,
                             const float* Qua, const float* bQua, float* out, float p_topic, uint32_t seed, int B, int U, int H,
                             int C1, int d, void* save, size_t save_bytes, void* workspace, size_t workspace_bytes,
                             const void* fa_image ,
                             const float* prev , void* stream);
int digat_user_ctx_bwd(const float* dout, const float* Xu, const uint8_t* cat_mask, const int64_t* cat_idx, const float* c_n,
                       const float* Ku, const float* Qu, const float* Fa, const float* Kua, const float* Qua, float p_topic,
                       const void* save, size_t save_bytes, float* dXu, float* dc_n, float* dKu, float* dQu, float* dbQu,
                       float* dFa, float* dbFa, float* dKua, float* dQua, float* dbQua, int B, int U, int H, int C1, int d,
                       int accumulate_params ,
                       void* workspace, size_t workspace_bytes, const void* fa_bwd_image , void* stream);

int digat_rank_metrics(const float* scores, const uint8_t* labels, const int64_t* impression_start, int num_impressions,
                       int32_t* ranks, double* per_impression, double* mean4, void* stream);

int64_t digat_format_rank_file(const int64_t* ranks, const int64_t* starts, int64_t impressions, char* out, int64_t cap);

#define DIGAT_TOPK_CHUNK 16384
size_t digat_topk_segments_workspace_bytes(int64_t rows, int64_t segments, int k);
int digat_topk_segments(const float* scores, const int64_t* seg_start, int64_t rows, int64_t segments, const int64_t* ids,
                        const int64_t* skip, int skip_len, int k, float* out_scores, int64_t* out_ids, int32_t* out_count,
                        void* workspace, size_t workspace_bytes, void* stream);

#define DIGAT_DOT_TOPK_CHUNK 2048
#define DIGAT_DOT_TOPK_USERS 64
#define DIGAT_DOT_TOPK_SUB 64
size_t digat_dot_topk_workspace_bytes(int64_t users, int64_t pool, int k);
int digat_dot_topk(const float* users, const float* news, const int64_t* pool, int64_t G, int64_t N, int64_t P, int d, const int64_t* skip,
                   int skip_len, int k, float* out_scores, int64_t* out_ids, int32_t* out_count, void* workspace, size_t workspace_bytes,
                   void* stream);
int digat_dot_scores(const float* users, const float* news, const int64_t* pool, int64_t G, int64_t N, int64_t P, int d, float* out,
                     void* stream);

size_t digat_mmr_select_workspace_bytes(int64_t users, int m, int k);
int digat_mmr_select(const int64_t* ids, const float* scores, const int32_t* count, int64_t G, int M, const float* vectors, int64_t N, int d,
                     const int32_t* category, int max_per_category, float lam, float mu, int k, int64_t* out_ids, float* out_scores,
                     int32_t* out_count, void* workspace, size_t workspace_bytes, void* stream);

size_t digat_gat_workspace_bytes(int B, int n, int d);
int digat_gat_fwd(const float* X, const uint8_t* A, const float* W, const float* bW, const float* a1, const float* a2,
// ... 154 lines not shown
```

Measured before the change: 38310 impressions/s.

## Add ragged three-strip GEMM tiles for strip counts not divisible by three

Adds a ragged variant of the strip GEMM kernel that uses three-strip tiles with a shorter final tile when the strip count is not a multiple of three, so A-tile loads are reused across more output columns. For d=400 there are five 80-column strips, which previously ran as single-strip tiles. Full tiles are scheduled before the short tail tiles by default (long-first), with a row-major option and an off switch. The featureAffine GEMM in the encoder enables it by default. It also adds a new standalone linear-rows entry point. The cost is extra kernel instantiations and runtime branching on the strip count inside the K loop.

```diff
diff --git a/digat_amd/_lib.py b/digat_amd/_lib.py
--- a/digat_amd/_lib.py
+++ b/digat_amd/_lib.py
@@ -18,6 +18,7 @@
 PARAMS_SIDE_STREAM_OFF, PARAMS_SIDE_STREAM_ON = 512, 1024
 PARAMS_NO_LIVE_ROWS = 2048
 PARAMS_PROJ_F16F8C = 4096
+PARAMS_RAGGED_OFF, PARAMS_RAGGED_ROWMAJOR = 8192, 16384
 
 _f = C.c_void_p
 
@@ -171,6 +172,8 @@
     "digat_split_proj_weights": (C.c_int, [_f, _f, _f, C.c_int, _f, C.c_int, _f]),
     "digat_split_weights": (C.c_int, [_f, C.c_int, C.c_int, _f, C.c_int, _f]),
     "digat_linear_f32x3": (C.c_int, [_f, C.c_int64, _f, _f, _f, C.c_int64, C.c_int, C.c_int, C.c_int, _f, C.c_int, _f]),
+    "digat_linear_rows_f32x3": (C.c_int, [_f, C.c_int64] + [_f] * 6 + [C.c_int64] + [C.c_int] * 3 + [_f, C.c_int, _f, _f, _f, C.c_int64, _f]
+                                + [C.c_int] * 3 + [_f]),
     "digat_fold_workspace_bytes": (C.c_size_t, [C.c_int]),
     "digat_fold_attention": (C.c_int, [_f] * 5 + [C.c_int, _f, C.c_size_t, _f]),
     "digat_linear_bwd_input": (C.c_int, [_f, C.c_int64, _f, _f, C.c_int64, C.c_int, C.c_int, C.c_int, C.c_int, _f]),
diff --git a/digat_amd/csrc/digat_encoder.inc b/digat_amd/csrc/digat_encoder.inc
--- a/digat_amd/csrc/digat_encoder.inc
+++ b/digat_amd/csrc/digat_encoder.inc
@@ -143,6 +143,7 @@
     const digat_params* const p; const EncoderWs& w; const hipStream_t st;
     const int B, N, H, G, d, C, L, U, C1;
     const GemmFormats f;
+    const int ragged;
     float *const c_n, *const c_u; const float* const c_n_src;
     LiveLists pend{}, live{};
     const int* sparse_flag = nullptr;
@@ -151,7 +152,7 @@
     FoldedPass(const EncoderCall& call, const float* Xg0_, SideStream* side_)
         : c(call), pl(call.plan), Xg0(Xg0_), side(side_), p(call.p), w(call.ws), st(call.st), B(call.B), N(call.N), H(call.H), G(call.G),
           d(call.p->d), C(call.p->category_num), L(call.p->depth), U(call.H + call.p->category_num), C1(call.p->category_num + 1),
-          f(gemm_formats(call.p)), c_n(call.out_news), c_u(call.out_user), c_n_src(call.plan.c_n0_in_place ? call.c_n0 : call.out_news) {}
+          f(gemm_formats(call.p)), ragged(encoder_ragged(call.p->flags)), c_n(call.out_news), c_u(call.out_user), c_n_src(call.plan.c_n0_in_place ? call.c_n0 : call.out_news) {}
 
     int context_queries(int next_layer, hipStream_t sq) const {
         return launch_gemm(ctx_queries_args(p, next_layer == 0 ? c_n_src : c_n, B, next_layer, w.kq_t, w.kq_u, w.r_user[next_layer & 1]), sq);
@@ -174,6 +175,7 @@
         g.epi = EPI_RELU_RES; g.e0 = T; g.lde0 = d;
         g.wsplit = (const unsigned short*)p->featureAffine_wsplit;
         g.format = f.fmt; g.range_flag = f.range_flag;
+        g.ragged = ragged;
         if (live.bucket_idx && gemm_takes_row_list(g)) { g.rowidx = live.bucket_idx; g.nrows_dev = live.nbuckets; }
         e = launch_gemm(g, sq);
         if (e) return e;
diff --git a/digat_amd/csrc/digat_encoder_plan.h b/digat_amd/csrc/digat_encoder_plan.h
--- a/digat_amd/csrc/digat_encoder_plan.h
+++ b/digat_amd/csrc/digat_encoder_plan.h
@@ -101,3 +101,5 @@
     pl.side_wanted = folded && !(pl.side_mode == 0 || (pl.side_mode == 2 && B >= 2048));
     return pl;
 }
+
+static inline int encoder_ragged(int flags) { return (flags & DIGAT_PARAMS_RAGGED_OFF) ? 0 : ((flags & DIGAT_PARAMS_RAGGED_ROWMAJOR) ? 2 : 1); }
diff --git a/digat_amd/csrc/digat_gemm.inc b/digat_amd/csrc/digat_gemm.inc
--- a/digat_amd/csrc/digat_gemm.inc
+++ b/digat_amd/csrc/digat_gemm.inc
@@ -340,14 +340,15 @@
 #else
 #define GT_NOW() 0ull
 #endif
-template <int NSUB, bool F16, int MT, bool FULL>
+template <int NSUB, bool F16, int MT, bool FULL, bool RAG = false>
 __global__ void __launch_bounds__(256, MT == 1 ? 3 : 2) gemm_bf16x6s_kernel(const GemmArgs g) {
     static_assert(MT == 1 || MT == 2, "wave tiles of 16 or 32 rows");
+    static_assert(!RAG || (NSUB == 3 && MT == 2), "ragged tiles: 128 rows x up to three strips");
     constexpr int NT = 5;
     constexpr int WROWS = 16 * MT, TROWS = 4 * WROWS;
     constexpr int APW = 2 * MT;
     constexpr int RING = 3;
-    constexpr int ABUF = NSUB == 1 ? 2 : 1;
+    constexpr int ABUF = NSUB == 1 || RAG ? 2 : 1;
     constexpr int PL = F16 ? 2 : 3;
     constexpr int WS_SLOTS = PL * 320;
     constexpr int PIECES = WS_SLOTS / 64;
@@ -357,12 +358,29 @@
 
     const int Mv = g.nrows_dev ? __builtin_amdgcn_readfirstlane(*g.nrows_dev) : g.M;
     if (g.exec_rows && blockIdx.x == 0 && threadIdx.x == 0) atomicAdd(g.exec_rows, (unsigned long long)Mv);
-    const int total = ((Mv + TROWS - 1) / TROWS) * g.ntiles;
-    const int chunk = (total + 7) >> 3;
-    if ((int)(blockIdx.x >> 3) >= chunk) return;
-    const int tile = (int)(blockIdx.x & 7) * chunk + (int)(blockIdx.x >> 3);
-    if (tile >= total) return;
-    const int mtile = tile / g.ntiles, ntile = tile - mtile * g.ntiles;
+    int mtile, ntile;
+    if (!RAG || g.ragged == DIGAT_GEMM_RAGGED_ROWMAJOR) {
+        const int total = ((Mv + TROWS - 1) / TROWS) * g.ntiles;
+        const int chunk = (total + 7) >> 3;
+        if ((int)(blockIdx.x >> 3) >= chunk) return;
+        const int tile = (int)(blockIdx.x & 7) * chunk + (int)(blockIdx.x >> 3);
+        if (tile >= total) return;
+        mtile = tile / g.ntiles; ntile = tile - mtile * g.ntiles;
+    } else {
+        const int mlive = (Mv + TROWS - 1) / TROWS, nfw = g.ntiles - 1;
+        const int nfull = mlive * nfw, cf = (nfull + 7) >> 3, cs = (mlive + 7) >> 3;
+        const int xcd = (int)(blockIdx.x & 7), j = (int)(blockIdx.x >> 3);
+        if (j < cf) {
+            const int t = xcd * cf + j;
+            if (t >= nfull) return;
+            mtile = t / nfw; ntile = t - mtile * nfw;
+        } else {
+            const int t = xcd * cs + (j - cf);
+            if (j - cf >= cs || t >= mlive) return;
+            mtile = t; ntile = nfw;
+        }
+    }
+    const int ns = RAG ? __builtin_amdgcn_readfirstlane(g.strips - NSUB * ntile < NSUB ? g.strips - NSUB * ntile : NSUB) : NSUB;
 
     const int tid = threadIdx.x, lane = tid & 63, wm = tid >> 6;
     const int kg = lane >> 4, lr = lane & 15;
@@ -373,16 +391,14 @@
     unsigned long long gt_wait = 0, gt_bar = 0, gt_body = 0, gt_steps = 0, gt_last = 0;
 #endif
     const int KT = (g.K + 31) >> 5;
-    const int nsteps = KT * NSUB;
+    const int nsteps = KT * ns;
     const unsigned ldsB = (unsigned)(uintptr_t)(__attribute__((address_space(3))) unsigned char*)&Bs[0][0];
     const unsigned ldsA = (unsigned)(uintptr_t)(__attribute__((address_space(3))) unsigned char*)&As[0][0];
     const char* const wimg = reinterpret_cast<const char*>(g.wsplit);
     const unsigned wlane = (unsigned)lane * 16u;
     const int wu = __builtin_amdgcn_readfirstlane(wm);
 
-    auto issue_b = [&](int step) {
-        const int kt = step / NSUB, s = step - kt * NSUB;
-        const int buf = step % RING;
+    auto issue_b_at = [&](int kt, int s, int buf) {
         const char* src = wimg + ((long)(strip0 + s) * KT + kt) * (WS_SLOTS * 16);
 #pragma unroll
         for (int k = 0; k < IMG_I; ++k) {
@@ -390,6 +406,16 @@
             q = q < PIECES ? q : PIECES - 1;
             lds_dma16_s(src + q * 1024, wlane, ldsB + (unsigned)((buf * WS_SLOTS + q * 64) * 16));
         }
+    };
+    auto issue_b = [&](int step) {
+        const int kt = step / NSUB;
+        issue_b_at(kt, step - kt * NSUB, step % RING);
+    };
+    int nb_kt = 0, nb_s = 0, nb_buf = 0;
+    auto issue_b_next = [&]() {
+        issue_b_at(nb_kt, nb_s, nb_buf);
+        if (++nb_s == ns) { nb_s = 0; ++nb_kt; }
+        nb_buf = nb_buf == RING - 1 ? 0 : nb_buf + 1;
     };
     const long arow0 = g.rowidx ? 0 : (long)(m0 < Mv ? m0 : Mv - 1);
     const char* const abase = reinterpret_cast<const char*>(g.a0 + arow0 * g.lda0);
@@ -476,6 +502,11 @@
         for (int j = 0; j < ABUF; ++j) if (j < KT) issue_a(j, j);
 #pragma unroll
         for (int j = 0; j < RING - 1; ++j) if (j < nsteps) issue_b(j);
+    } else if constexpr (RAG) {
+        issue_a(0, 0);
+        if (ns == 1 && KT > 1) issue_a(1, 1);
+        issue_b_next();
+        if (nsteps > 1) issue_b_next();
     } else {
         issue_a(0, 0);
         issue_b(0);
@@ -486,97 +517,114 @@
 #pragma unroll
     for (int mt = 0; mt < MT; ++mt) split_mt(mt, 0, af);
 
-    for (int kt = 0; kt < KT; ++kt) {
-        const bool more = kt + 1 < KT;
-#pragma unroll
-        for (int s = 0; s < NSUB; ++s) {
-            const int step = kt * NSUB + s;
-            const int buf = step % RING;
+    auto k_loop = [&](auto one_strip) __attribute__((always_inline)) {
+        constexpr bool ONE = decltype(one_strip)::value;
+        constexpr int SMAX = ONE ? 1 : NSUB;
+        int step_r = 0, buf_r = 0;
+        for (int kt = 0; kt < KT; ++kt) {
+            const bool more = kt + 1 < KT;
+            const int sbuf = RAG ? ((more ? kt + 1 : kt) & 1) : 0;
+#pragma unroll
+            for (int s = 0; s < SMAX; ++s) {
+                if constexpr (RAG && !ONE) { if (s == 2 && ns == 2) break; }
+                const bool split_here = ONE ? s == 0 : s == 1;
+                const int step = RAG ? step_r : kt * NSUB + s;
+                const int buf = RAG ? buf_r : step % RING;
 #ifdef DIGAT_GEMM_TIMERS
-            const unsigned long long gt0 = GT_NOW();
-            if (step > 0) gt_body += gt0 - gt_last;
+                const unsigned long long gt0 = GT_NOW();
+                if (step > 0) gt_body += gt0 - gt_last;
 #endif
-            if constexpr (NSUB == 1) {
-                constexpr int L = (RING - 1 < ABUF - 1 ? RING - 1 : ABUF - 1) - 1;
-                constexpr int KEEP = (APW + IMG_I) * (L < 0 ? 0 : L) + ((ABUF - 1 < RING - 1) ? IMG_I : 0);
-                static_assert(KEEP <= 63, "vmcnt is six bits");
-                if (kt + (RING - 1 > ABUF ? RING - 1 : ABUF) < KT) wait_vmcnt_imm<KEEP>();
-                else asm volatile("s_waitcnt vmcnt(0)" ::: "memory");
-            } else if (step + 1 < nsteps) {
-                if constexpr (IMG_I == 4) asm volatile("s_waitcnt vmcnt(4)" ::: "memory");
-                else asm volatile("s_waitcnt vmcnt(3)" ::: "memory");
-            } else asm volatile("s_waitcnt vmcnt(0)" ::: "memory");
+                if constexpr (NSUB == 1) {
+                    constexpr int L = (RING - 1 < ABUF - 1 ? RING - 1 : ABUF - 1) - 1;
+                    constexpr int KEEP = (APW + IMG_I) * (L < 0 ? 0 : L) + ((ABUF - 1 < RING - 1) ? IMG_I : 0);
+                    static_assert(KEEP <= 63, "vmcnt is six bits");
+                    if (kt + (RING - 1 > ABUF ? RING - 1 : ABUF) < KT) wait_vmcnt_imm<KEEP>();
+                    else asm volatile("s_waitcnt vmcnt(0)" ::: "memory");
+                } else if (step + 1 < nsteps) {
+                    if constexpr (IMG_I == 4) asm volatile("s_waitcnt vmcnt(4)" ::: "memory");
+                    else asm volatile("s_waitcnt vmcnt(3)" ::: "memory");
+                } else asm volatile("s_waitcnt vmcnt(0)" ::: "memory");
 #ifdef DIGAT_GEMM_TIMERS
-            const unsigned long long gt1 = GT_NOW();
+                const unsigned long long gt1 = GT_NOW();
 #endif
-            __builtin_amdgcn_s_barrier();
+                __builtin_amdgcn_s_barrier();
 #ifdef DIGAT_GEMM_TIMERS
-            gt_last = GT_NOW();
-            gt_wait += gt1 - gt0; gt_bar += gt_last - gt1; ++gt_steps;
+                gt_last = GT_NOW();
+                gt_wait += gt1 - gt0; gt_bar += gt_last - gt1; ++gt_steps;
 #endif
-            if (NSUB == 1) {
-                if (kt + ABUF < KT) issue_a(kt + ABUF, kt % ABUF);
-                if (step + RING - 1 < nsteps) issue_b(step + RING - 1);
-            } else {
-                if (s == 0 && more) issue_a(kt + 1, 0);
-                if (step + 2 < nsteps) issue_b(step + 2);
-            }
-            const uint4* Bi = Bs[buf];
-            const int lslot = kg * 80 + lr;
-            bf16x8 bq[2][3];
-#pragma unroll
-            for (int p = 0; p < PL; ++p) bq[0][p] = __builtin_bit_cast(bf16x8, Bi[p * 320 + lslot]);
-#pragma unroll
-            for (int nt = 0; nt < NT; ++nt) {
-                if (nt + 1 < NT) {
-#pragma unroll
-                    for (int p = 0; p < PL; ++p) bq[(nt + 1) & 1][p] = __builtin_bit_cast(bf16x8, Bi[p * 320 + lslot + (nt + 1) * 16]);
-                }
-                const bf16x8 b1 = bq[nt & 1][0], b2 = bq[nt & 1][1], b3 = bq[nt & 1][PL - 1];
-                v4f c[MT];
-#pragma unroll
-                for (int mt = 0; mt < MT; ++mt) c[mt] = acc[s][mt][nt];
-                if (!F16 && (FULL || !lite[s])) {
-#pragma unroll
-                    for (int mt = 0; mt < MT; ++mt) c[mt] = mma(b1, af[2][mt], c[mt]);
-#pragma unroll
-                    for (int mt = 0; mt < MT; ++mt) c[mt] = mma(b2, af[1][mt], c[mt]);
-#pragma unroll
-                    for (int mt = 0; mt < MT; ++mt) c[mt] = mma(b3, af[0][mt], c[mt]);
-                }
-                if (FULL || lite[s] < 2) {
-#pragma unroll
-                    for (int mt = 0; mt < MT; ++mt) c[mt] = mma(b1, af[1][mt], c[mt]);
-#pragma unroll
-                    for (int mt = 0; mt < MT; ++mt) c[mt] = mma(b2, af[0][mt], c[mt]);
-                }
-#pragma unroll
-                for (int mt = 0; mt < MT; ++mt) c[mt] = mma(b1, af[0][mt], c[mt]);
-#pragma unroll
-                for (int mt = 0; mt < MT; ++mt) acc[s][mt][nt] = c[mt];
-                if (NSUB > 1) {
-                    if (s == 1 && nt == 0) split_mt(0, 0, afn);
-                    if constexpr (MT > 1) { if (s == 1 && nt == 2) split_mt(1, 0, afn); }
+                if (NSUB == 1) {
+                    if (kt + ABUF < KT) issue_a(kt + ABUF, kt % ABUF);
+                    if (step + RING - 1 < nsteps) issue_b(step + RING - 1);
+                } else if constexpr (RAG) {
+                    if constexpr (ONE) { if (kt + 2 < KT) issue_a(kt + 2, kt & 1); }
+                    else if (s == 0 && more) issue_a(kt + 1, (kt + 1) & 1);
+                    if (step + 2 < nsteps) issue_b_next();
                 } else {
-                    if (nt == 0) split_mt(0, (kt + 1) % ABUF, afn);
-                    if constexpr (MT > 1) { if (nt == 2) split_mt(1, (kt + 1) % ABUF, afn); }
-                }
-            }
-            if (NSUB == 1 || s == 1) {
-#pragma unroll
-                for (int i = 0; i < 56; ++i) {
-                    __builtin_amdgcn_sched_group_barrier(0x008, 1, 0);
-                    __builtin_amdgcn_sched_group_barrier(0x002, 2, 0);
-                }
-            }
-        }
-        if (more) {
-#pragma unroll
-            for (int p = 0; p < 3; ++p)
-#pragma unroll
-                for (int mt = 0; mt < MT; ++mt) af[p][mt] = afn[p][mt];
-        }
-    }
+                    if (s == 0 && more) issue_a(kt + 1, 0);
+                    if (step + 2 < nsteps) issue_b(step + 2);
+                }
+                const uint4* Bi = Bs[buf];
+                const int lslot = kg * 80 + lr;
+                bf16x8 bq[2][3];
+#pragma unroll
+                for (int p = 0; p < PL; ++p) bq[0][p] = __builtin_bit_cast(bf16x8, Bi[p * 320 + lslot]);
+#pragma unroll
+                for (int nt = 0; nt < NT; ++nt) {
+                    if (nt + 1 < NT) {
+#pragma unroll
+                        for (int p = 0; p < PL; ++p) bq[(nt + 1) & 1][p] = __builtin_bit_cast(bf16x8, Bi[p * 320 + lslot + (nt + 1) * 16]);
+                    }
+                    const bf16x8 b1 = bq[nt & 1][0], b2 = bq[nt & 1][1], b3 = bq[nt & 1][PL - 1];
+                    v4f c[MT];
+#pragma unroll
+                    for (int mt = 0; mt < MT; ++mt) c[mt] = acc[s][mt][nt];
+                    if (!F16 && (FULL || !lite[s])) {
+#pragma unroll
+                        for (int mt = 0; mt < MT; ++mt) c[mt] = mma(b1, af[2][mt], c[mt]);
+#pragma unroll
+                        for (int mt = 0; mt < MT; ++mt) c[mt] = mma(b2, af[1][mt], c[mt]);
+#pragma unroll
+                        for (int mt = 0; mt < MT; ++mt) c[mt] = mma(b3, af[0][mt], c[mt]);
+                    }
+                    if (FULL || lite[s] < 2) {
+#pragma unroll
+                        for (int mt = 0; mt < MT; ++mt) c[mt] = mma(b1, af[1][mt], c[mt]);
+#pragma unroll
+                        for (int mt = 0; mt < MT; ++mt) c[mt] = mma(b2, af[0][mt], c[mt]);
+                    }
+#pragma unroll
+                    for (int mt = 0; mt < MT; ++mt) c[mt] = mma(b1, af[0][mt], c[mt]);
+#pragma unroll
+                    for (int mt = 0; mt < MT; ++mt) acc[s][mt][nt] = c[mt];
+                    if (NSUB > 1) {
+                        if (split_here && nt == 0) split_mt(0, sbuf, afn);
+                        if constexpr (MT > 1) { if (split_here && nt == 2) split_mt(1, sbuf, afn); }
+                    } else {
+                        if (nt == 0) split_mt(0, (kt + 1) % ABUF, afn);
+                        if constexpr (MT > 1) { if (nt == 2) split_mt(1, (kt + 1) % ABUF, afn); }
+                    }
+                }
+                if (NSUB == 1 || split_here) {
+#pragma unroll
+                    for (int i = 0; i < 56; ++i) {
+                        __builtin_amdgcn_sched_group_barrier(0x008, 1, 0);
+                        __builtin_amdgcn_sched_group_barrier(0x002, 2, 0);
+                    }
+                }
+                if constexpr (RAG) { ++step_r; buf_r = buf_r == RING - 1 ? 0 : buf_r + 1; }
+            }
+            if (more) {
+#pragma unroll
+                for (int p = 0; p < 3; ++p)
+#pragma unroll
+                    for (int mt = 0; mt < MT; ++mt) af[p][mt] = afn[p][mt];
+            }
+        }
+    };
+    if constexpr (RAG) {
+        if (ns == 1) k_loop(std::true_type{});
+        else k_loop(std::false_type{});
+    } else k_loop(std::false_type{});
 
 #ifdef DIGAT_GEMM_TIMERS
     const unsigned long long gt_loop_end = GT_NOW();
@@ -600,6 +648,7 @@
     const bool has_e0 = g.epi == EPI_RELU_RES || g.epi == EPI_ADD_E0;
 #pragma unroll
     for (int s = 0; s < NSUB; ++s) {
+        if constexpr (RAG) { if (s >= ns) break; }
         const int ncol0 = (strip0 + s) * 80;
         const int seg = ncol0 / g.nseg;
         const int nbase = ncol0 - seg * g.nseg + kg * 4;
@@ -1324,6 +1373,17 @@
     }
     ProfScope prof(kind, listed ? 0.0 : 2.0 * g.M * (double)Ntot * g.K, st, listed ? 0.0 : (double)g.M * gemm_row_bytes(g));
     g.mtiles = p.mtiles; g.ntiles = p.ntiles;
+    g.ragged = p.ragged; g.strips = p.ragged ? Ntot / 80 : 0;
+    if (p.ragged) {
+        void (*ragged)(const GemmArgs) = nullptr;
+        if (p.kernel == GEMM_STRIP_3_F16_FULL) ragged = gemm_bf16x6s_kernel<3, true, 2, true, true>;
+        else if (p.kernel == GEMM_STRIP_3_F16) ragged = gemm_bf16x6s_kernel<3, true, 2, false, true>;
+        else if (p.kernel == GEMM_STRIP_3_BF16) ragged = gemm_bf16x6s_kernel<3, false, 2, false, true>;
+        else return DIGAT_ERR_ARG;
+        hipLaunchKernelGGL(ragged, dim3(p.grid), dim3(p.block), 0, st, g);
+        DIGAT_CHECK_LAUNCH();
+        return DIGAT_OK;
+    }
     switch (p.kernel) {
 #define DIGAT_GEMM_LAUNCH(id, ...) case GEMM_##id: hipLaunchKernelGGL((__VA_ARGS__), dim3(p.grid), dim3(p.block), 0, st, g); break;
         DIGAT_GEMM_KERNELS(DIGAT_GEMM_LAUNCH)
diff --git a/digat_amd/csrc/digat_gemm_plan.h b/digat_amd/csrc/digat_gemm_plan.h
--- a/digat_amd/csrc/digat_gemm_plan.h
+++ b/digat_amd/csrc/digat_gemm_plan.h
@@ -27,7 +27,10 @@
     unsigned* range_flag;
     const uint8_t* dmask; long lddm; float dscale;
     int dmask_cols;
+    int ragged;
+    int strips;
 };
+enum { DIGAT_GEMM_RAGGED = 1, DIGAT_GEMM_RAGGED_ROWMAJOR = 2 };
 
 #define DIGAT_GEMM_KERNELS(X)                                        \
     X(F16F8C_3, gemm_f16f8c_kernel<3>)                               \
@@ -77,6 +80,7 @@
     int mtiles, ntiles;
     unsigned grid, block;
     int image_format;
+    int ragged;
 };
 
 static inline bool gemm_kernel_takes_row_list(int kernel) {
@@ -84,7 +88,7 @@
 }
 
 static inline GemmPlan gemm_plan(const GemmArgs& g, int kind = DIGAT_KERNEL_LINEAR) {
-    GemmPlan p = {DIGAT_OK, GEMM_NONE, 0, 0, 0, 256, -1};
+    GemmPlan p = {DIGAT_OK, GEMM_NONE, 0, 0, 0, 256, -1, 0};
     const int Ntot = g.nseg * g.nsegs;
     const int Md = g.m_dispatch > 0 ? g.m_dispatch : g.M;
     const auto tiles = [&](int kernel, int mtiles, int ntiles, bool round8) {
@@ -141,12 +145,20 @@
         const int strips = Ntot / 80;
         const bool three = strips % 3 == 0;
         const int ntiles = three ? strips / 3 : strips;
-        if (((g.M + 127) / 128) * ntiles < 400 && (f16 || !g.rowidx)) {
+        const int Mfill = g.ragged ? Md : g.M;
+        if (((Mfill + 127) / 128) * ntiles < 400 && (f16 || !g.rowidx)) {
             const int k = f16 ? (three ? GEMM_STRIP_3_F16_64 : GEMM_STRIP_1_F16_64) : (three ? GEMM_STRIP_3_BF16_64 : GEMM_STRIP_1_BF16_64);
             return tiles(k, (g.M + 63) / 64, ntiles, true);
         }
         const int k = three ? (f16 ? (!g.x1_segs && !g.x3_segs ? GEMM_STRIP_3_F16_FULL : GEMM_STRIP_3_F16) : GEMM_STRIP_3_BF16)
                             : (f16 ? GEMM_STRIP_1_F16 : GEMM_STRIP_1_BF16);
+        if (g.ragged && !three && strips > 3) {
+            const int mt = (g.M + 127) / 128, nt = (strips + 2) / 3;
+            tiles(f16 ? (!g.x1_segs && !g.x3_segs ? GEMM_STRIP_3_F16_FULL : GEMM_STRIP_3_F16) : GEMM_STRIP_3_BF16, mt, nt, true);
+            p.grid = (unsigned)(8 * ((mt * (nt - 1) + 7) / 8 + (mt + 7) / 8));
+            p.ragged = g.ragged;
+            return p;
+        }
         return tiles(k, (g.M + 127) / 128, ntiles, true);
     }
     const int bm = cfg == 0 ? 128 : (cfg == 1 ? 64 : 32);
diff --git a/digat_amd/csrc/digat_kernels.hip b/digat_amd/csrc/digat_kernels.hip
--- a/digat_amd/csrc/digat_kernels.hip
+++ b/digat_amd/csrc/digat_kernels.hip
@@ -489,6 +489,29 @@
     return launch_gemm(g, (hipStream_t)stream, DIGAT_KERNEL_PROJ);
 }
 
+int digat_linear_rows_f32x3(const float* x, int64_t ldx, const float* w0, const float* w1, const float* b0, const float* b1,
+                            float* y0, float* y1, int64_t ldy, int M, int nseg, int K, void* wsplit, int format,
+                            const int* rowidx, const int* nrows_dev, const float* e0, int64_t lde0,
+                            const float* radd, int rows_per_b, int m_dispatch, int ragged, void* stream) {
+    if (!x || !w0 || !y0 || !wsplit || M < 0 || nseg <= 0 || K <= 0 || (w1 && !y1) || (radd && (!w1 || rows_per_b <= 0))) return DIGAT_ERR_ARG;
+    if (ragged < 0 || ragged > DIGAT_GEMM_RAGGED_ROWMAJOR || (rowidx && !nrows_dev)) return DIGAT_ERR_ARG;
+    if (K % 8 || ldx % 4 || nseg % 80) return DIGAT_ERR_SHAPE;
+    const int nsegs = w1 ? 2 : 1;
+    const int rcs = launch_split(w0, w1 ? w1 : w0, w0, nseg, nsegs, K, wsplit, (hipStream_t)stream, 0, format);
+    if (rcs) return rcs;
+    GemmArgs g = gemm_plain(x, ldx, w0, b0, y0, ldy, M, nseg, K, 0);
+    g.w[1] = w1; g.bias[1] = b1; g.y[1] = y1; g.nsegs = nsegs;
+    g.wsplit = (const unsigned short*)wsplit; g.format = format;
+    if (e0) { g.epi = EPI_RELU_RES; g.e0 = e0; g.lde0 = lde0; }
+    g.radd = radd; g.radd_seg = 1; g.rows_per_b = rows_per_b;
+    g.m_dispatch = m_dispatch; g.ragged = ragged;
+    if (rowidx) {
+        if (!gemm_takes_row_list(g)) return DIGAT_ERR_ARG;
+        g.rowidx = rowidx; g.nrows_dev = nrows_dev;
+    }
+    return launch_gemm(g, (hipStream_t)stream, DIGAT_KERNEL_PROJ);
+}
+
 struct NewsCtxWs { float *qv, *kq, *glob; };
 static NewsCtxWs news_ctx_carve(Arena& a, int B, int d) {
     const size_t bd = (size_t)B * d;
diff --git a/digat_amd/graphEncoders.py b/digat_amd/graphEncoders.py
--- a/digat_amd/graphEncoders.py
+++ b/digat_amd/graphEncoders.py
@@ -2,6 +2,7 @@
 
 import contextlib
 import math
+import os
 import threading
 
 import torch
@@ -80,6 +81,7 @@
         self.corpus_xattn_hint = {}
         self.side_stream = "auto"
         self.live_rows = True
+        self.ragged_tiles = os.environ.get("DIGAT_RAGGED_TILES", "long-first")
         self.fused_user_context = False
 
     def initialize(self):
@@ -283,7 +285,8 @@
                 | (_lib.PARAMS_PROJ_F16F8C if pm == "fp16-fp8c" else 0)
                 | (_lib.PARAMS_BD_TILED if self.pass_rows >= 2048 else 0)
                 | {"auto": 0, "off": _lib.PARAMS_SIDE_STREAM_OFF, "on": _lib.PARAMS_SIDE_STREAM_ON}[self._launch_option("side_stream")]
-                | (0 if self._launch_option("live_rows") else _lib.PARAMS_NO_LIVE_ROWS))
+                | (0 if self._launch_option("live_rows") else _lib.PARAMS_NO_LIVE_ROWS)
+                | {"long-first": 0, "row-major": _lib.PARAMS_RAGGED_ROWMAJOR, "off": _lib.PARAMS_RAGGED_OFF}[self.ragged_tiles])
 
     def _fold_sources(self):
         ca, ua = self.candidate_attention, self.userAttention
diff --git a/include/digat_hip.h b/include/digat_hip.h
--- a/include/digat_hip.h
+++ b/include/digat_hip.h
@@ -32,6 +32,10 @@
 int digat_split_weights(const float* W, int N, int K, void* wsplit, int format, void* stream);
 int digat_linear_f32x3(const float* x, int64_t ldx, const float* w, const float* b, float* y, int64_t ldy,
                        int M, int N, int K, void* wsplit, int format, void* stream);
+int digat_linear_rows_f32x3(const float* x, int64_t ldx, const float* w0, const float* w1, const float* b0, const float* b1,
+                            float* y0, float* y1, int64_t ldy, int M, int nseg, int K, void* wsplit, int format,
+                            const int* rowidx, const int* nrows_dev, const float* e0, int64_t lde0,
+                            const float* radd, int rows_per_b, int m_dispatch, int ragged, void* stream);
 
 size_t digat_xattn_workspace_bytes(int B, int n, int d);
 int digat_xattn_fwd(const float* X, const uint8_t* A, const float* ctx,
@@ -145,6 +149,7 @@
 
 enum { DIGAT_PARAMS_SIDE_STREAM_OFF = 512, DIGAT_PARAMS_SIDE_STREAM_ON = 1024, DIGAT_PARAMS_NO_LIVE_ROWS = 2048 };
 enum { DIGAT_PARAMS_PROJ_F16F8C = 4096 };
+enum { DIGAT_PARAMS_RAGGED_OFF = 8192, DIGAT_PARAMS_RAGGED_ROWMAJOR = 16384 };
 
 size_t digat_encoder_grouped_workspace_bytes(int B, int N, int H, int C, int d, int depth);
 int digat_encoder_fwd_grouped(const digat_params* params,
```

Measured after the change: 39090 impressions/s (median of 6 runs). +2.0%, better.
